# MPEGGroup/mpeg-pcc-tmc2

Hardware: AMD Instinct MI355X
Metric: encoder patch+image-gen frames/sec, longdress_vox10 32-frame GOF (higher is better)
Workload: dtype int32/f64

## Files before the change

include/tmc2hip.h:

```cpp
#ifndef TMC2HIP_H
#define TMC2HIP_H
#include <stddef.h>
#include <stdint.h>

#ifdef __cplusplus
extern "C" {
#endif

#define TMC2_OK 0
#define TMC2_E_NO_DEVICE -1
#define TMC2_E_HIP -2
#define TMC2_E_INVALID -3
#define TMC2_E_UNSUPPORTED -4
#define TMC2_E_STATE -5

typedef struct tmc2_ctx   tmc2_ctx;
typedef struct tmc2_frame tmc2_frame;

typedef struct tmc2_segmenter_params {
  int32_t nnNormalEstimation;
  int32_t normalOrientation;
  int32_t gridBasedRefineSegmentation;
  int32_t maxNNCountRefineSegmentation;
  int32_t iterationCountRefineSegmentation;
  int32_t voxelDimensionRefineSegmentation;
  int32_t searchRadiusRefineSegmentation;
  int32_t occupancyResolution;
  int32_t enablePatchSplitting;
  int32_t maxPatchSize;
  int32_t quantizerSizeX;
  int32_t quantizerSizeY;
  int32_t minPointCountPerCCPatchSegmentation;
  int32_t maxNNCountPatchSegmentation;
  int32_t surfaceThickness;
  int32_t mapCountMinus1;
  int32_t minLevel;
  int32_t maxAllowedDepth;
  int32_t geometryBitDepth2D;
  int32_t geometryBitDepth3D;
  double  maxAllowedDist2RawPointsDetection;
  double  maxAllowedDist2RawPointsSelection;
  double  lambdaRefineSegmentation;
  double  weightNormal[3];
} tmc2_segmenter_params;

typedef struct tmc2_patch {
  int32_t index, viewId;
  int32_t normalAxis, tangentAxis, bitangentAxis, projectionMode;
  int32_t u1, v1, d1;
  int32_t sizeU, sizeV, sizeD, sizeDPixel;
  int32_t sizeU0, sizeV0;
  int32_t size2DXInPixel, size2DYInPixel;
  int32_t d0Count, eomAndD1Count;
  int32_t u0, v0, patchOrientation;
  int64_t depthOffset;
  int64_t occOffset;
} tmc2_patch;

int         tmc2_ctx_create( int device, tmc2_ctx** out );
void        tmc2_ctx_destroy( tmc2_ctx* ctx );
const char* tmc2_last_error( void );
int         tmc2_ctx_synchronize( tmc2_ctx* ctx );
int         tmc2_host_alloc( size_t bytes, void** out );
void        tmc2_host_free( void* p );
int         tmc2_host_register( void* p, size_t bytes );
int         tmc2_host_unregister( void* p );
typedef struct tmc2_host_gate tmc2_host_gate;
int         tmc2_host_gate_create( int maxConcurrentHostSteps, tmc2_host_gate** out );
void        tmc2_host_gate_destroy( tmc2_host_gate* gate );
int         tmc2_ctx_set_host_gate( tmc2_ctx* ctx, tmc2_host_gate* gate );
void        tmc2_set_host_parallelism( int maxConcurrentHostSteps );
int         tmc2_ctx_set_option( tmc2_ctx* ctx, const char* key, const char* value );
const char* tmc2_ctx_get_option( tmc2_ctx* ctx, const char* key );
int         tmc2_ctx_reserve( tmc2_ctx* ctx, uint64_t maxPoints, int voxelDimRefine, int bits3d, int maxCanvasWidth, int maxCanvasHeight );
int         tmc2_ctx_pool_stats( tmc2_ctx* ctx, uint64_t* bytesHeld, uint64_t* mallocCalls, double* mallocMs, uint64_t* carvedBlocks );
int         tmc2_ctx_device_alloc( tmc2_ctx* ctx, size_t bytes, void** out );
int         tmc2_ctx_device_free( tmc2_ctx* ctx, void* p );
int         tmc2_ctx_upload( tmc2_ctx* ctx, void* deviceDst, const void* hostSrc, size_t bytes );
int         tmc2_ctx_download( tmc2_ctx* ctx, void* hostDst, const void* deviceSrc, size_t bytes );
void*       tmc2_ctx_stream( tmc2_ctx* ctx );
int         tmc2_ctx_device( tmc2_ctx* ctx );
int         tmc2_ctx_make_current( tmc2_ctx* ctx );
int         tmc2_ctx_stage_count( tmc2_ctx* ctx );
const char* tmc2_ctx_stage_name( tmc2_ctx* ctx, int i );
double      tmc2_ctx_stage_ms( tmc2_ctx* ctx, int i );
long        tmc2_ctx_stage_calls( tmc2_ctx* ctx, int i );
void        tmc2_ctx_stage_reset( tmc2_ctx* ctx );
void        tmc2_ctx_set_timing( tmc2_ctx* ctx, int enabled );

int  tmc2_frame_create( tmc2_ctx* ctx, const int16_t* xyz, const uint8_t* rgb, uint64_t n, tmc2_frame** out );
void tmc2_frame_destroy( tmc2_frame* f );
int  tmc2_kdtree_build( tmc2_frame* f );
void tmc2_set_kdtree_placement( int mode );
void tmc2_set_refine_overlap( int on );
int  tmc2_frame_get_kdtree_order( tmc2_frame* f, uint32_t* perm, int32_t* depth );
uint64_t tmc2_frame_point_count( const tmc2_frame* f );
int  tmc2_frame_reset( tmc2_frame* f );

int tmc2_kdtree_search( tmc2_frame* f, const int16_t* queries, uint64_t nq, int k, uint32_t* idx, uint32_t* dist2 );
int tmc2_kdtree_search_wide( tmc2_frame* f, const int16_t* queries, uint64_t nq, int k, uint32_t* idx );

int tmc2_normals_compute_normals( tmc2_frame* f, int k );
int tmc2_normals_orient( tmc2_frame* f );
int tmc2_normals_compute( tmc2_frame* f, int k, int orientation );
int tmc2_frame_get_normals( tmc2_frame* f, double* normals  );
int tmc2_frame_set_normals( tmc2_frame* f, const double* normals );
int tmc2_frame_get_adjacency( tmc2_frame* f, uint32_t* adj  );

int tmc2_weight_normal( tmc2_frame* f, int geometryBitDepth3D, double minWeightEPP, double weight[3] );

int tmc2_segmenter_initial_segmentation( tmc2_frame* f, const double weight[3] );
int tmc2_segmenter_refine_grid_based( tmc2_frame* f, int maxNNCount, double lambda, int iterationCount,
                                      int voxDim, int searchRadius );
int tmc2_segmenter_refine( tmc2_frame* f, int maxNNCount, double lambda, int iterationCount );
int tmc2_frame_get_partition( tmc2_frame* f, uint32_t* partition  );
int tmc2_frame_set_partition( tmc2_frame* f, const uint32_t* partition );
int tmc2_segmenter_segment_patches( tmc2_frame* f, const tmc2_segmenter_params* p );
int tmc2_segmenter_compute( tmc2_frame* f, const tmc2_segmenter_params* p );
int tmc2_segmenter_params_check( const tmc2_segmenter_params* p );
int tmc2_segmenter_compute_grid_based( tmc2_frame* f, const tmc2_segmenter_params* p, int voxelDimensionGridBasedSegmentation );
int tmc2_segmenter_compute_knn_refine( tmc2_frame* f, const tmc2_segmenter_params* p, int voxelDimensionGridBasedSegmentation );
int tmc2_segmenter_convert_points_to_voxels( tmc2_ctx* ctx, const int16_t* xyz, uint64_t n, int voxDim, int bits, int16_t* voxelXyz,
                                             uint64_t* voxelCount, uint32_t* voxelOfPoint );

int tmc2_frame_patch_count( tmc2_frame* f );
int tmc2_frame_patch_pool_sizes( tmc2_frame* f, int64_t* depthCount, int64_t* occCount );
int tmc2_frame_get_patches( tmc2_frame* f, tmc2_patch* patches, int16_t* depth0, int16_t* depth1, uint8_t* occupancy );

int tmc2_encoder_pack_flexible( tmc2_frame* f, int presetWidth, int numTilesHor, double tileHeightToWidthRatio,
                                int32_t* height );
int tmc2_encoder_pack_spatial_consistency( tmc2_frame* f, tmc2_frame* previous, int presetWidth, int numTilesHor,
                                           double tileHeightToWidthRatio, int32_t* height );
int tmc2_frame_get_packed_size( tmc2_frame* f, int32_t* width, int32_t* height );
int tmc2_frame_get_patch_matches( tmc2_frame* f, int32_t* matches );
int tmc2_encoder_global_patch_allocation( tmc2_frame** frames, int count, int minimumImageWidth, int minimumImageHeight,
                                          int32_t* widths, int32_t* heights );
int tmc2_frame_set_packing( tmc2_frame* f, const tmc2_patch* list, int count, const int32_t* matches, const uint8_t* occupancy,
                            int64_t occupancyBytes, int packedWidth, int packedHeight );
int tmc2_frame_get_patch_order( tmc2_frame* f, int32_t* order );
int tmc2_encoder_canvas_size( const int32_t* frameHeights, int frames, int tileWidth, int minimumImageWidth,
                              int minimumImageHeight, int32_t* width, int32_t* height );
int tmc2_encoder_generate_geometry_images( tmc2_frame* f, int width, int height, int occupancyPrecision );
int tmc2_frame_get_geometry_images( tmc2_frame* f, uint8_t* occupancy, uint8_t* occVideo, uint32_t* blockToPatch,
                                    uint16_t* geometryD0, uint16_t* geometryD1 );
int     tmc2_encoder_generate_attribute_images( tmc2_frame* f );
int     tmc2_transfer_colors( tmc2_ctx* ctx, const int16_t* srcXyz, const uint8_t* srcRgb, uint64_t n, const int16_t* tgtXyz,
                              uint64_t m, uint8_t* tgtRgb );
int64_t tmc2_frame_recon_count( tmc2_frame* f );
int     tmc2_frame_get_reconstruction( tmc2_frame* f, int16_t* xyz, uint8_t* rgb, uint32_t* pointToPixel );
int     tmc2_frame_get_attribute_images( tmc2_frame* f, uint8_t* attribute );
int     tmc2_frame_set_decoded_geometry( tmc2_frame* f, const uint8_t* occVideo, const uint16_t* geometry );

int tmc2_frame_device_images( tmc2_frame* f, void** occupancy, void** occVideo, void** blockToPatch, void** geometry );
int tmc2_frame_device_attribute( tmc2_frame* f, void** attribute );

int tmc2_color_convert_rgb444_to_yuv420( tmc2_ctx* ctx, const uint8_t* rgb, int width, int height, int downsamplingFilter,
                                         uint8_t* yuv420 );
int tmc2_color_convert_yuv420_to_yuv444( tmc2_ctx* ctx, const uint8_t* yuv420, int width, int height, int upsamplingFilter,
                                         uint16_t* yuv444 );
int tmc2_encoder_attribute_to_yuv420( tmc2_frame* f, int downsamplingFilter, uint8_t* yuv420 );
int tmc2_codec_set_decoded_attribute_yuv420( tmc2_frame* f, const uint8_t* yuv420, int upsamplingFilter );
int tmc2_frame_get_decoded_attribute( tmc2_frame* f, uint16_t* planes );

int tmc2_decoder_frame_create( tmc2_ctx* ctx, const tmc2_patch* patches, int count, int width, int height, int occupancyPrecision,
                               const uint8_t* occVideo, const uint16_t* geometry, tmc2_frame** out );
int tmc2_codec_generate_point_cloud( tmc2_frame* f );
int tmc2_codec_generate_point_cloud_pbf( tmc2_frame* f, int thresholdLossyOM, int passesCount, int filterSize, int log2Threshold );
int tmc2_frame_patch_border_filtering_size( tmc2_frame* f, int64_t* pixels );
int tmc2_frame_get_patch_border_filtering( tmc2_frame* f, uint8_t* occupancy, uint8_t* border );

int tmc2_codec_identify_boundary_points( tmc2_frame* f );
int tmc2_codec_color_point_cloud( tmc2_frame* f, const uint16_t* attribute );
int tmc2_codec_smooth_point_cloud_postprocess( tmc2_frame* f, int gridSize, double thresholdSmoothing );
int tmc2_codec_transfer_colors_16bit_bp( tmc2_frame* f );
int tmc2_codec_color_smoothing( tmc2_frame* f, int gridSize, double thresholdColorSmoothing, double thresholdColorDifference,
                                double thresholdColorVariation );
int tmc2_frame_set_geometry_bit_depth_3d( tmc2_frame* f, int geometryBitDepth3D );
int tmc2_color_smoothing( tmc2_ctx* ctx, const int16_t* xyz, uint16_t* colors16, const uint16_t* boundaryType, const uint32_t* patchIndex,
                          uint64_t M, int gridSize, int geometryBitDepth3D, double thresholdColorSmoothing,
                          double thresholdColorDifference, double thresholdColorVariation );
int tmc2_codec_convert_yuv16_to_rgb8( tmc2_frame* f );
int tmc2_frame_get_post_reconstruction( tmc2_frame* f, int16_t* xyz, uint16_t* colors16, uint8_t* rgb, uint16_t* boundaryType );

int tmc2_metrics_compute( tmc2_ctx* ctx, const int16_t* srcXyz, const uint8_t* srcRgb, uint64_t n, const int16_t* recXyz,
                          const uint8_t* recRgb, uint64_t m, const double* srcNormals, double resolution, double* out,
                          int64_t* counts );

int tmc2_metrics_compute_frame( tmc2_frame* frame, int which, int useNormals, double resolution, double* out, int64_t* counts );
int tmc2_metrics_compute_frame_source( tmc2_frame* frame, int which, const int16_t* srcXyz, const uint8_t* srcRgb, uint64_t n,
                                       const double* srcNormals, double resolution, double* out, int64_t* counts );

int tmc2_metrics_ordered_sums( tmc2_ctx* ctx, const double* termsA, uint64_t nA, const double* termsB, uint64_t nB, double* out );

int tmc2_metrics_display( const double* out, uint64_t sourcePoints, uint64_t reconstructPoints, const int64_t* counts,
                          uint64_t resolution, int withC2p, int precision, char* text, uint64_t capacity, uint64_t* needed );

int tmc2_ply_info( const char* path, int readNormals, uint64_t* pointCount, int* hasColors, int* hasNormals );
int tmc2_ply_read( const char* path, int16_t* xyz, uint8_t* rgb, double* normals, uint64_t capacity, int threads,
                   uint64_t* pointCount );
int tmc2_ply_write( const char* path, const int16_t* xyz, const uint8_t* rgb, const double* normals, uint64_t n, int asAscii );
int tmc2_point_set_checksum( const int16_t* xyz, const uint8_t* rgb, uint64_t n, int reorderPoints, uint8_t digest[16] );

int tmc2_checksum_file_write( const char* path, const uint8_t* digests, uint64_t frames );
int tmc2_checksum_file_read( const char* path, uint8_t* digests, uint64_t capacity, uint64_t* frames );

int tmc2_host_kdtree_build( const int16_t* xyz, uint64_t n, uint32_t* perm, uint64_t* nodeCount, int32_t* depth );
int tmc2_host_pack_flexible( tmc2_patch* patches, int count, const uint8_t* occupancy, int presetWidth, int numTilesHor,
                             double tileHeightToWidthRatio, int32_t* order, int32_t* height );
int tmc2_host_global_patch_allocation( int frames, int32_t* counts, tmc2_patch* patches, const uint8_t* occupancy,
                                       const int64_t* occupancyBase, int32_t* matches, int tileWidth, int tileHeight,
                                       int minimumImageWidth, int minimumImageHeight, uint8_t* occupancyOut,
                                       int64_t occupancyOutCapacity, int64_t* occupancyOutBase, int32_t* widths,
                                       int32_t* heights );
int tmc2_host_pack_spatial_consistency( tmc2_patch* patches, int count, const uint8_t* occupancy, const tmc2_patch* previous,
                                        int previousCount, int presetWidth, int numTilesHor, double tileHeightToWidthRatio,
                                        int32_t* order, int32_t* matches, int32_t* height );
int tmc2_host_place_segments( int frames, const int32_t* counts, tmc2_patch* patches, const uint8_t* occupancy,
                              const int64_t* occupancyBase, int mode, int minimumImageWidth, int minimumImageHeight, int numTilesHor,
                              double tileHeightToWidthRatio, int32_t* matches, uint8_t* occupancyOut, int64_t occupancyOutCapacity,
                              int64_t* occupancyOutBase, int32_t* widths, int32_t* heights );
int tmc2_host_orient_normals( const int16_t* xyz, uint64_t n, const uint32_t* knn, int k, double* normals );
int tmc2_host_color_smoothing( const int16_t* xyz, uint16_t* colors16, const uint16_t* boundaryType, const uint32_t* patchIndex,
                               uint64_t M, int gridSize, int geometryBitDepth3D, double thresholdColorSmoothing,
                               double thresholdColorDifference, double thresholdColorVariation );
int tmc2_host_patch_border_filtering( const tmc2_patch* patches, int count, int width, int height, int occupancyPrecision,
                                      const uint8_t* occVideo, const uint16_t* geometryD0, const uint32_t* blockToPatch,
                                      int thresholdLossyOM, int passesCount, int filterSize, int log2Threshold, uint8_t* occupancy,
                                      uint8_t* border );
int tmc2_host_convert_points_to_voxels( const int16_t* xyz, uint64_t n, int voxDim, int bits, int16_t* voxelXyz, uint64_t* voxelCount,
                                        uint32_t* voxelOfPoint );
int tmc2_host_refine_segmentation( const int16_t* xyz, uint64_t n, const double* normals, uint32_t* partition, int maxNNCount,
                                   double lambda, int iterationCount, uint32_t* adjacency  );

int tmc2_selftest_scan( tmc2_ctx* ctx, const uint32_t* d_in, uint32_t* d_out, uint64_t n, uint32_t* d_total, uint32_t* hostAnswer,
                        const uint32_t* d_carry, int carryWords, uint64_t epoch );
int tmc2_selftest_fill( tmc2_ctx* ctx, const uint64_t* regions, int count );
int tmc2_selftest_work_map( tmc2_ctx* ctx, uint64_t gridBlocks, int blockThreads, uint64_t n, uint64_t liveBlocks, uint32_t* d_hits,
                            uint32_t* d_logical );
int tmc2_selftest_components( tmc2_ctx* ctx, const uint32_t* d_knn, const uint8_t* d_partition, const uint8_t* d_raw,
                              const uint32_t* d_perm, uint64_t n, uint32_t* d_root, uint32_t* d_bad );
int tmc2_selftest_union_find( tmc2_ctx* ctx, int parity, uint32_t* d_word, uint64_t n, const uint32_t* d_edges, uint64_t m, int precheck,
                              int agent, uint32_t* d_root, uint32_t* d_rootParity, uint32_t* d_bad );
int tmc2_selftest_cand_sort( tmc2_ctx* ctx, uint32_t* d_lists, const uint32_t* d_offsets, uint64_t lists, uint32_t* d_ok );
int tmc2_selftest_std_sort( uint32_t* lists, const uint32_t* offsets, uint64_t count );
int tmc2_selftest_marked_cells( tmc2_ctx* ctx, const int16_t* d_xyz4, const uint8_t* d_boundaryType, uint64_t M, int gridSize, int bits,
                                int maxCoord, uint32_t* cells, uint32_t* d_bits, uint32_t* d_rank, const uint32_t* d_keys, uint64_t keys,
                                uint32_t* d_slots );

#ifdef __cplusplus
}
#endif
#endif
```

mpeg-pcc-tmc2_amd/csrc/attributes.hip:

```cpp
#include <algorithm>
#include <cmath>

#include "color_transfer.h"
#include "internal.h"
#include "patch_border_filter.h"

namespace tmc2 {
namespace {

__device__ __forceinline__ void toCanvasB( const PlaceDev& p, int u, int v, int& x, int& y ) {
  if ( p.orient == 0 ) {
    x = u + p.u0 * 16;
    y = v + p.v0 * 16;
  } else {
    x = v + p.u0 * 16;
    y = u + p.v0 * 16;
  }
}

__device__ __forceinline__ int normalCoord( const PlaceDev& p, int depth ) {
  return p.mode == 0 ? depth + p.d1 : max( 0, p.d1 - depth );
}

struct PbfMapsDev {
  const int64_t* offset;
  const uint8_t *occ, *flag;
  int            border;
  uint8_t*       btype;
};

template <bool EMIT, bool PBF = false>
__global__ __launch_bounds__( 256 ) void reconTileKernel( const PlaceDev* __restrict__ place,
                                                           const uint32_t* __restrict__ tilePatch,
                                                           const uint8_t* __restrict__ occVideo,
                                                           const uint32_t* __restrict__ blockToPatch,
                                                           const uint16_t* __restrict__ geo, int W, int H, int prec,
                                                           uint32_t* __restrict__ tileCount,
                                                           const uint32_t* __restrict__ tileOffset, Pt* __restrict__ recon,
                                                           uint32_t* __restrict__ pointToPixel, PbfMapsDev pbf = PbfMapsDev() ) {
  __shared__ uint32_t waveTotal[4];
  const uint32_t      tile  = blockIdx.x;
  const uint32_t      k     = tilePatch[tile];
  const PlaceDev      p     = place[k];
  const int           local = int( tile ) - p.tileBase;
  const int           ub = local % p.sizeU0, vb = local / p.sizeU0;
  const int           bx = p.orient == 0 ? ub + p.u0 : vb + p.u0, by = p.orient == 0 ? vb + p.v0 : ub + p.v0;
  const bool          owned = blockToPatch[size_t( by ) * ( W / 16 ) + bx] == k + 1;
  const int           u = ub * 16 + int( threadIdx.x & 15 ), v = vb * 16 + int( threadIdx.x >> 4 );
  int                 x, y;
  toCanvasB( p, u, v, x, y );
  uint32_t cnt = 0;
  int      c0 = 0, c1 = 0;
  bool    occupied = owned && x < W && y < H;
  uint8_t flag     = 0;
  if constexpr ( PBF ) {
    if ( occupied ) {
      const int64_t c = pbf.offset[k] + int64_t( v + pbf.border ) * ( p.sizeU0 * 16 + 2 * pbf.border ) + u + pbf.border;
      occupied        = pbf.occ[c] != 0;
      flag            = pbf.flag[c];
    }
  } else {
    occupied = occupied && occVideo[size_t( y / prec ) * ( W / prec ) + x / prec];
  }
  if ( occupied ) {
    c0  = normalCoord( p, geo[size_t( y ) * W + x] );
    c1  = normalCoord( p, geo[size_t( W ) * H + size_t( y ) * W + x] );
    cnt = c1 != c0 ? 2u : 1u;
  }
  const int lane = threadIdx.x & 63, wave = threadIdx.x >> 6;
  uint32_t  inc  = cnt;
#pragma unroll
  for ( int off = 1; off < 64; off <<= 1 ) {
    const uint32_t t = __shfl_up( inc, off, 64 );
    if ( lane >= off ) inc += t;
  }
  if ( lane == 63 ) waveTotal[wave] = inc;
  __syncthreads();
  if ( !EMIT ) {
    if ( threadIdx.x == 0 ) tileCount[tile] = waveTotal[0] + waveTotal[1] + waveTotal[2] + waveTotal[3];
    return;
  }
  if ( cnt == 0 ) return;
  uint32_t off = tileOffset[tile] + inc - cnt;
  for ( int w = 0; w < wave; ++w ) off += waveTotal[w];
  int c[3];
  c[p.axT] = u + p.u1;
  c[p.axB] = v + p.v1;
  c[p.axN] = c0;
  recon[off]        = Pt{int16_t( c[0] ), int16_t( c[1] ), int16_t( c[2] ), 0};
  pointToPixel[off] = packPixel( x, y, 0, cnt == 2 );
  if constexpr ( PBF ) {
    pbf.btype[off] = flag;
    if ( cnt == 2 ) pbf.btype[off + 1] = flag;
  }
  if ( cnt == 2 ) {
    c[p.axN]              = c1;
    recon[off + 1]        = Pt{int16_t( c[0] ), int16_t( c[1] ), int16_t( c[2] ), 0};
    pointToPixel[off + 1] = packPixel( x, y, 1, false );
  }
}

__global__ __launch_bounds__( 256 ) void forwardColorKernel( const uint32_t* __restrict__ idx8, const uint32_t* __restrict__ dist8,
                                                              const uint32_t* __restrict__ easy,
                                                              const uint8_t* __restrict__ srcRgb4, uint32_t m,
                                                              uint8_t* __restrict__ fwdRgb4 ) {
  const uint32_t t = blockIdx.x * blockDim.x + threadIdx.x;
  if ( t >= m ) return;
  if ( easy[t] != 0xFFFFFFFFu ) {
    reinterpret_cast<uchar4*>( fwdRgb4 )[t] = reinterpret_cast<const uchar4*>( srcRgb4 )[easy[t]];
    return;
  }
  const uint4* ir = reinterpret_cast<const uint4*>( idx8 + size_t( t ) * 8 );
  const uint4* dr = reinterpret_cast<const uint4*>( dist8 + size_t( t ) * 8 );
  const uint4  i0 = ir[0], i1 = ir[1], d0 = dr[0], d1 = dr[1];
  const uint32_t id[8] = {i0.x, i0.y, i0.z, i0.w, i1.x, i1.y, i1.z, i1.w};
  const uint32_t ds[8] = {d0.x, d0.y, d0.z, d0.w, d1.x, d1.y, d1.z, d1.w};
  reinterpret_cast<uchar4*>( fwdRgb4 )[t] = forwardColor( id, ds, reinterpret_cast<const uchar4*>( srcRgb4 ) );
}

template <bool FILL>
__global__ __launch_bounds__( 256 ) void backwardVoteKernel( const uint32_t* __restrict__ idx1, const uint32_t* __restrict__ dist1, uint32_t n,
                                                              uint32_t* __restrict__ count, const uint32_t* __restrict__ offset,
                                                              uint2* __restrict__ entries ) {
  const uint32_t s = blockIdx.x * blockDim.x + threadIdx.x;
  if ( s >= n ) return;
  const uint32_t t = idx1[s], slot = atomicAdd( &count[t], 1u );
  if ( FILL ) entries[offset[t] + slot] = make_uint2( dist1[s], s );
}

__global__ __launch_bounds__( 256 ) void combineColorKernel( const uint32_t* __restrict__ count, const uint32_t* __restrict__ offset,
                                                              uint2* __restrict__ entries, const uint8_t* __restrict__ srcRgb4,
                                                              const uint8_t* __restrict__ fwdRgb4, uint32_t m,
                                                              uint8_t* __restrict__ outRgb4, uint32_t* __restrict__ error ) {
  const uint32_t t = blockIdx.x * blockDim.x + threadIdx.x;
  if ( t >= m ) return;
  const int n = int( count[t] );
  if ( n == 0 ) {
    reinterpret_cast<uchar4*>( outRgb4 )[t] = reinterpret_cast<const uchar4*>( fwdRgb4 )[t];
    return;
  }
  uint2* e = entries + offset[t];
  if ( !orderCandidates( e, n ) ) *error = 1;
  const ColorSum c = backwardColor( e, e[0].x == 0 ? 1 : n, reinterpret_cast<const uchar4*>( srcRgb4 ), []( uint32_t source ) { return source; } );
  reinterpret_cast<uchar4*>( outRgb4 )[t] = combinedColor( reinterpret_cast<const uchar4*>( fwdRgb4 )[t], c );
}

__global__ __launch_bounds__( 256 ) void attributeScatterKernel( const uint8_t* __restrict__ rgb4,
                                                                  const uint32_t* __restrict__ pointToPixel, uint32_t m,
                                                                  int W, int H, uint8_t* __restrict__ attr ) {
  const uint32_t i = blockIdx.x * blockDim.x + threadIdx.x;
  if ( i >= m ) return;
  const uint32_t pp = pointToPixel[i];
  const size_t   px = size_t( pixelY( pp ) ) * W + pixelX( pp ), plane = size_t( W ) * H;
  const uchar4   c  = reinterpret_cast<const uchar4*>( rgb4 )[i];
  const bool     layer1 = pixelLayer( pp ), hasD1 = pixelHasD1( pp );
  if ( !layer1 ) {
    attr[px] = c.x, attr[plane + px] = c.y, attr[2 * plane + px] = c.z;
    if ( !hasD1 ) attr[3 * plane + px] = c.x, attr[4 * plane + px] = c.y, attr[5 * plane + px] = c.z;
  } else {
    attr[3 * plane + px] = c.x, attr[4 * plane + px] = c.y, attr[5 * plane + px] = c.z;
  }
}

__global__ __launch_bounds__( 256 ) void upsampleOccupancyKernel( const uint8_t* __restrict__ occVideo, int W, int H, int prec,
                                                                   uint8_t* __restrict__ occ ) {
  const size_t c = size_t( blockIdx.x ) * blockDim.x + threadIdx.x;
  if ( c >= size_t( W ) * H ) return;
  occ[c] = occVideo[size_t( ( c / W ) / prec ) * ( W / prec ) + ( c % W ) / prec];
}

__device__ __forceinline__ int mean4w( int p1, int w1, int p2, int w2, int p3, int w3, int p4, int w4 ) {
  return ( p1 * w1 + p2 * w2 + p3 * w3 + p4 * w4 ) / ( w1 + w2 + w3 + w4 );
}

__device__ __forceinline__ void pushPullMipPixel( int i, const uint8_t* img, const uint8_t* occ, int W, int H, uint8_t* mip,
                                                  uint8_t* mipOcc, int w, int h, int p0 = 0, int p1 = 6 ) {
  const int  x = i % w, y = i / w, X = 2 * x, Y = 2 * y;
  const bool i2 = X + 1 < W, i3 = Y + 1 < H;
  const int  w1 = occ[size_t( Y ) * W + X] ? 255 : 0;
  const int  w2 = ( i2 && occ[size_t( Y ) * W + X + 1] ) ? 255 : 0;
  const int  w3 = ( i3 && occ[size_t( Y + 1 ) * W + X] ) ? 255 : 0;
  const int  w4 = ( i2 && i3 && occ[size_t( Y + 1 ) * W + X + 1] ) ? 255 : 0;
  const bool any = ( w1 + w2 + w3 + w4 ) > 0;
  mipOcc[i]      = any ? 1 : 0;
  for ( int p = p0; p < p1; ++p ) {
    const uint8_t* s = img + size_t( p ) * W * H;
    uint8_t        v = 0;
    if ( any ) {
      const int v1 = s[size_t( Y ) * W + X], v2 = i2 ? s[size_t( Y ) * W + X + 1] : 0;
      const int v3 = i3 ? s[size_t( Y + 1 ) * W + X] : 0, v4 = ( i2 && i3 ) ? s[size_t( Y + 1 ) * W + X + 1] : 0;
      v            = uint8_t( mean4w( v1, w1, v2, w2, v3, w3, v4, w4 ) );
    }
    mip[size_t( p ) * w * h + i] = v;
  }
}
__global__ __launch_bounds__( 256 ) void pushPullMipKernel( const uint8_t* __restrict__ img, const uint8_t* __restrict__ occ, int W,
                                                             int H, uint8_t* __restrict__ mip, uint8_t* __restrict__ mipOcc, int w,
                                                             int h ) {
  const int i = blockIdx.x * blockDim.x + threadIdx.x;
  if ( i < w * h ) pushPullMipPixel( i, img, occ, W, H, mip, mipOcc, w, h );
}

__device__ __forceinline__ void pushPullFillPixel( int i, uint8_t* img, const uint8_t* occ, int W, int H, const uint8_t* mip, int w,
                                                   int h, int p0 = 0, int p1 = 6 ) {
  if ( occ[i] ) return;
  const int  X = i % W, Y = i / W, x = X >> 1, y = Y >> 1;
  const int  dx = ( X & 1 ) ? 1 : -1, dy = ( Y & 1 ) ? 1 : -1;
  const bool hx = dx < 0 ? x > 0 : x < w - 1, hy = dy < 0 ? y > 0 : y < h - 1;
  for ( int p = p0; p < p1; ++p ) {
    const uint8_t* m  = mip + size_t( p ) * w * h;
    const int      v  = m[size_t( y ) * w + x];
    const int      vx = hx ? m[size_t( y ) * w + x + dx] : 0;
    const int      vy = hy ? m[size_t( y + dy ) * w + x] : 0;
    const int      vd = ( hx && hy ) ? m[size_t( y + dy ) * w + x + dx] : 0;
    img[size_t( p ) * W * H + i] = uint8_t( mean4w( v, 144, vx, hx ? 48 : 0, vy, hy ? 48 : 0, vd, ( hx && hy ) ? 16 : 0 ) );
  }
}
__global__ __launch_bounds__( 256 ) void pushPullFillKernel( uint8_t* __restrict__ img, const uint8_t* __restrict__ occ, int W, int H,
                                                              const uint8_t* __restrict__ mip, int w, int h ) {
  const int i = blockIdx.x * blockDim.x + threadIdx.x;
  if ( i < W * H ) pushPullFillPixel( i, img, occ, W, H, mip, w, h );
}

__device__ __forceinline__ void pushPullBlurPixel( int i, const uint8_t* src, uint8_t* dst, const uint8_t* occ, int W, int H, int p0 = 0,
                                                   int p1 = 6 ) {
  if ( occ[i] ) return;
  const int x = i % W, y = i / W;
  const int x1 = x > 0 ? x - 1 : x, y1 = y > 0 ? y - 1 : y, x2 = x < W - 1 ? x + 1 : x, y2 = y < H - 1 ? y + 1 : y;
  for ( int p = p0; p < p1; ++p ) {
    const uint8_t* s   = src + size_t( p ) * W * H;
    const int      sum = s[size_t( y1 ) * W + x1] + s[size_t( y1 ) * W + x2] + s[size_t( y2 ) * W + x1] + s[size_t( y2 ) * W + x2] +
                    s[size_t( y ) * W + x1] + s[size_t( y ) * W + x2] + s[size_t( y1 ) * W + x] + s[size_t( y2 ) * W + x];
    dst[size_t( p ) * W * H + i] = uint8_t( ( sum + 4 ) >> 3 );
  }
}
__global__ __launch_bounds__( 256 ) void pushPullBlurKernel( const uint8_t* __restrict__ src, uint8_t* __restrict__ dst,
                                                              const uint8_t* __restrict__ occ, int W, int H ) {
  const int i = blockIdx.x * blockDim.x + threadIdx.x;
  if ( i < W * H ) pushPullBlurPixel( i, src, dst, occ, W, H );
}

constexpr int kPushPullTile = 96, kPushPullSpan = 128, kPushPullMaxIters = ( kPushPullSpan - kPushPullTile ) / 2;
__global__ __launch_bounds__( 1024 ) void pushPullFillBlurKernel( uint8_t* __restrict__ img, const uint8_t* __restrict__ occ, int W,
                                                                   int H, const uint8_t* __restrict__ mip, int w, int h, int iters,
                                                                   int tilesX ) {
  __shared__ uint8_t sOcc[kPushPullSpan * kPushPullSpan];
  __shared__ uint8_t sBuf[2][kPushPullSpan * kPushPullSpan];
  const int      X0 = ( blockIdx.x % tilesX ) * kPushPullTile, Y0 = ( blockIdx.x / tilesX ) * kPushPullTile;
  const int      RX0 = max( X0 - iters, 0 ), RY0 = max( Y0 - iters, 0 );
  const int      RW = min( X0 + kPushPullTile + iters, W ) - RX0, RH = min( Y0 + kPushPullTile + iters, H ) - RY0;
  uint8_t*       plane = img + size_t( blockIdx.y ) * W * H;
  const uint8_t* m     = mip + size_t( blockIdx.y ) * w * h;
  for ( int i = threadIdx.x; i < kPushPullSpan * RH; i += 1024 ) {
    const int rx = i & ( kPushPullSpan - 1 ), ry = i >> 7;
    if ( rx >= RW ) continue;
    const int     X = RX0 + rx, Y = RY0 + ry;
    const size_t  g = size_t( Y ) * W + X;
    const uint8_t o = occ[g];
    uint8_t       v;
    if ( o ) {
      v = plane[g];
    } else {
      const int  x = X >> 1, y = Y >> 1, dx = ( X & 1 ) ? 1 : -1, dy = ( Y & 1 ) ? 1 : -1;
      const bool hx = dx < 0 ? x > 0 : x < w - 1, hy = dy < 0 ? y > 0 : y < h - 1;
      const int  c  = m[size_t( y ) * w + x];
      const int  vx = hx ? m[size_t( y ) * w + x + dx] : 0;
      const int  vy = hy ? m[size_t( y + dy ) * w + x] : 0;
      const int  vd = ( hx && hy ) ? m[size_t( y + dy ) * w + x + dx] : 0;
      v             = uint8_t( mean4w( c, 144, vx, hx ? 48 : 0, vy, hy ? 48 : 0, vd, ( hx && hy ) ? 16 : 0 ) );
    }
    sOcc[i]    = o;
    sBuf[0][i] = v;
    sBuf[1][i] = v;
  }
  __syncthreads();
  int cur = 0;
  for ( int it = 0; it < iters; ++it ) {
    const uint8_t* src = sBuf[cur];
    uint8_t*       dst = sBuf[cur ^ 1];
    for ( int i = threadIdx.x; i < kPushPullSpan * RH; i += 1024 ) {
      const int rx = i & ( kPushPullSpan - 1 ), ry = i >> 7;
      if ( rx >= RW || sOcc[i] ) continue;
      const int l = rx > 0 ? -1 : 0, r = rx < RW - 1 ? 1 : 0;
      const int u = ry > 0 ? -kPushPullSpan : 0, d = ry < RH - 1 ? kPushPullSpan : 0;
      const int sum = src[i + u + l] + src[i + u + r] + src[i + d + l] + src[i + d + r] + src[i + l] + src[i + r] + src[i + u] +
                      src[i + d];
      dst[i] = uint8_t( ( sum + 4 ) >> 3 );
    }
    __syncthreads();
    cur ^= 1;
  }
  const uint8_t* res = sBuf[cur];
  for ( int i = threadIdx.x; i < kPushPullSpan * RH; i += 1024 ) {
    const int rx = i & ( kPushPullSpan - 1 ), ry = i >> 7;
    const int X = RX0 + rx, Y = RY0 + ry;
    if ( rx >= RW || sOcc[i] || X < X0 || X >= X0 + kPushPullTile || Y < Y0 || Y >= Y0 + kPushPullTile ) continue;
    plane[size_t( Y ) * W + X] = res[i];
  }
}

constexpr int kPushPullSmall  = 160 * 160;
constexpr int kPushPullLevels = 16;
struct PushPullLevels {
  int      count;
  int      first;
  int      w[kPushPullLevels], h[kPushPullLevels];
  uint8_t *img[kPushPullLevels], *tmp[kPushPullLevels], *occ[kPushPullLevels];
};
__global__ __launch_bounds__( 1024 ) void pushPullCoarseLevelsKernel( PushPullLevels L ) {
  const int p0 = int( blockIdx.x ), p1 = p0 + 1;
  for ( int l = L.first + 1; l < L.count; ++l ) {
    const int cnt = L.w[l] * L.h[l];
    for ( int i = threadIdx.x; i < cnt; i += blockDim.x )
      pushPullMipPixel( i, L.img[l - 1], L.occ[l - 1], L.w[l - 1], L.h[l - 1], L.img[l], L.occ[l], L.w[l], L.h[l], p0, p1 );
    __syncthreads();
  }
  int iters = 4;
  for ( int l = L.count - 1; l > L.first; --l ) {
    const int fw = L.w[l - 1], fh = L.h[l - 1], cnt = fw * fh;
    uint8_t * img = L.img[l - 1], *tmp = L.tmp[l - 1];
    const uint8_t* occ = L.occ[l - 1];
    for ( int i = threadIdx.x; i < cnt; i += blockDim.x ) pushPullFillPixel( i, img, occ, fw, fh, L.img[l], L.w[l], L.h[l], p0, p1 );
    __syncthreads();
    for ( int i = threadIdx.x; i < cnt; i += blockDim.x ) tmp[size_t( p0 ) * cnt + i] = img[size_t( p0 ) * cnt + i];
    __syncthreads();
    uint8_t *src = img, *dst = tmp;
    for ( int it = 0; it < iters; ++it ) {
      for ( int i = threadIdx.x; i < cnt; i += blockDim.x ) pushPullBlurPixel( i, src, dst, occ, fw, fh, p0, p1 );
      __syncthreads();
      uint8_t* t = src;
      src        = dst;
      dst        = t;
    }
    if ( src != img ) {
      L.img[l - 1] = src;
      L.tmp[l - 1] = img;
    }
    iters = min( iters + 1, 16 );
  }
}

__global__ __launch_bounds__( 256 ) void attributeGroupDilateKernel( const uint8_t* __restrict__ occ, int W, int H,
                                                                      uint8_t* __restrict__ attr ) {
  const size_t c = size_t( blockIdx.x ) * blockDim.x + threadIdx.x, plane = size_t( W ) * H;
  if ( c >= plane || occ[c] ) return;
#pragma unroll
  for ( int k = 0; k < 3; ++k ) {
    const uint32_t a = attr[k * plane + c], b = attr[( 3 + k ) * plane + c];
    const uint8_t  v = uint8_t( ( a + b + 1 ) >> 1 );
    attr[k * plane + c] = attr[( 3 + k ) * plane + c] = v;
  }
}

}

int transferColorsDevice( tmc2_ctx* ctx, const TreeDev& srcTree, const Pt* d_srcPts, const uint8_t* d_srcRgb4, uint32_t n,
                          const TreeDev& tgtTree, const Pt* d_tgtPts, uint32_t M, uint8_t* d_outRgb4, uint32_t* d_error ) {
  hipStream_t      s = ctx->stream;
  const dim3       blk( 256 );
  DevBuf<uint32_t> d_idx8, d_dist8, d_idx1, d_dist1, d_count, d_offset, d_cursor;
  DevBuf<uint2>    d_entries;
  DevBuf<uint8_t>  d_fwd;
  TMC2_TRY( d_idx8.alloc( size_t( M ) * 8 ) );
  TMC2_TRY( d_dist8.alloc( size_t( M ) * 8 ) );
  TMC2_TRY( d_idx1.alloc( n ) );
  TMC2_TRY( d_dist1.alloc( n ) );
  TMC2_TRY( d_count.alloc( M ) );
  TMC2_TRY( d_offset.alloc( M ) );
  TMC2_TRY( d_cursor.alloc( M ) );
  TMC2_TRY( d_entries.alloc( n ) );
  TMC2_TRY( d_fwd.alloc( size_t( M ) * 4 ) );
  DevBuf<uint32_t> d_easy8;
  TMC2_TRY( d_easy8.alloc( M ) );
  TMC2_TRY( launchKnnSplit( ctx, srcTree, d_tgtPts, M, 8, d_easy8.p, d_idx8.p, d_dist8.p, "knn8_recon_in_source" ) );
  TMC2_TRY( launchKnnSplit( ctx, tgtTree, d_srcPts, n, 1, d_idx1.p, d_idx1.p, d_dist1.p, "knn1_source_in_recon" ) );
  StageScope stage( ctx, "transfer_colors" );
  TMC2_TRY( fillRegions( ctx, {{d_count.p, size_t( M ) * 4, 0}, {d_cursor.p, size_t( M ) * 4, 0}, {d_error, 4, 0}} ) );
  const dim3 grdM( ( M + 255 ) / 256 ), grdN( ( n + 255 ) / 256 );
  hipLaunchKernelGGL( forwardColorKernel, grdM, blk, 0, s, d_idx8.p, d_dist8.p, d_easy8.p, d_srcRgb4, M, d_fwd.p );
  hipLaunchKernelGGL( backwardVoteKernel<false>, grdN, blk, 0, s, d_idx1.p, d_dist1.p, n, d_count.p, d_offset.p, d_entries.p );
  TMC2_TRY( exclusiveScanU32( ctx, d_count.p, d_offset.p, M, nullptr ) );
  hipLaunchKernelGGL( backwardVoteKernel<true>, grdN, blk, 0, s, d_idx1.p, d_dist1.p, n, d_cursor.p, d_offset.p, d_entries.p );
  hipLaunchKernelGGL( combineColorKernel, grdM, blk, 0, s, d_count.p, d_offset.p, d_entries.p, d_srcRgb4, d_fwd.p, M,
                      d_outRgb4, d_error );
  TMC2_HIP( hipGetLastError() );
  return TMC2_OK;
}

int reconstructPointCloud( tmc2_frame* f, const PbfParams* pbfParams ) {
  if ( !f->haveGeometryImages ) {
    setError( "generatePointCloud: geometry images missing" );
    return TMC2_E_STATE;
  }
  if ( pbfParams ) {
    if ( const char* what = pbfRefusal( f->occPrecision, *pbfParams, long( f->patches.size() ) ) ) {
      setError( "generatePointCloud (patch border filtering): unsupported %s", what );
      return TMC2_E_UNSUPPORTED;
    }
  }
  const bool keepAttributeImages = f->haveAttributeImages && ( pbfParams || f->havePbf );
  f->canvasesChanged();
  f->haveAttributeImages = keepAttributeImages;
  if ( pbfParams ) TMC2_TRY( patchBorderFilterDevice( f, *pbfParams ) );
  PbfMapsDev pbf;
  if ( pbfParams ) pbf = PbfMapsDev{f->d_pbfOffset.p, f->pbfOcc, f->pbfFlag, f->pbfBorderWidth, nullptr};
  tmc2_ctx*    ctx = f->ctx;
  hipStream_t  s   = ctx->stream;
  const int    W = f->canvasW, H = f->canvasH, prec = f->occPrecision;
  const dim3   blk( 256 );
  const uint32_t tiles = f->tileCount;
  StageScope       stage( ctx, "reconstruct" );
  DevBuf<uint32_t> d_tileCount, d_tileOffset, d_small;
  TMC2_TRY( d_tileCount.alloc( std::max( tiles, 1u ) ) );
  TMC2_TRY( d_tileOffset.alloc( std::max( tiles, 1u ) ) );
  TMC2_TRY( d_small.alloc( 8 ) );
  uint32_t M = 0;
  if ( tiles ) {
    if ( pbfParams )
      hipLaunchKernelGGL( ( reconTileKernel<false, true> ), dim3( tiles ), blk, 0, s, f->d_place.p, f->d_tilePatch.p, f->d_occVideo.p,
                          f->d_blockToPatch.p, f->d_geo.p, W, H, prec, d_tileCount.p, (const uint32_t*)nullptr, (Pt*)nullptr,
                          (uint32_t*)nullptr, pbf );
    else
      hipLaunchKernelGGL( reconTileKernel<false>, dim3( tiles ), blk, 0, s, f->d_place.p, f->d_tilePatch.p, f->d_occVideo.p,
                          f->d_blockToPatch.p, f->d_geo.p, W, H, prec, d_tileCount.p, (const uint32_t*)nullptr, (Pt*)nullptr,
                          (uint32_t*)nullptr, PbfMapsDev() );
    volatile uint32_t* answer = ctx->answerLine( tmc2_ctx::kAnswerRecon );
    TMC2_TRY( exclusiveScanU32( ctx, d_tileCount.p, d_tileOffset.p, tiles, d_small.p, ScanAnswer{answer, nullptr, 0} ) );
    TMC2_HIP( hipStreamSynchronize( s ) );
    M = answer[0];
  }
  if ( M == 0 && pbfParams ) {
    stage.end();
    f->reconCount         = 0;
    f->haveReconstruction = true;
    f->haveBoundaryTypes  = true;
    return TMC2_OK;
  }
  if ( M == 0 ) {
    setError( "generatePointCloud: empty reconstruction" );
    return TMC2_E_STATE;
  }
  TMC2_TRY( f->d_recon.alloc( M ) );
  TMC2_TRY( f->d_pointToPixel.alloc( M ) );
  if ( pbfParams ) {
    TMC2_TRY( f->d_boundaryType.alloc( M ) );
    TMC2_TRY( f->d_pbfBoundary.alloc( M ) );
    pbf.btype = f->d_boundaryType.p;
    hipLaunchKernelGGL( ( reconTileKernel<true, true> ), dim3( tiles ), blk, 0, s, f->d_place.p, f->d_tilePatch.p, f->d_occVideo.p,
                        f->d_blockToPatch.p, f->d_geo.p, W, H, prec, d_tileCount.p, d_tileOffset.p, f->d_recon.p, f->d_pointToPixel.p,
                        pbf );
    TMC2_HIP( hipMemcpyAsync( f->d_pbfBoundary.p, f->d_boundaryType.p, M, hipMemcpyDeviceToDevice, s ) );
  } else {
    hipLaunchKernelGGL( reconTileKernel<true>, dim3( tiles ), blk, 0, s, f->d_place.p, f->d_tilePatch.p, f->d_occVideo.p,
                        f->d_blockToPatch.p, f->d_geo.p, W, H, prec, d_tileCount.p, d_tileOffset.p, f->d_recon.p,
                        f->d_pointToPixel.p, PbfMapsDev() );
  }
  stage.end();
  f->reconCount = M;
  TMC2_TRY( buildKdTreePlaced( ctx, f->d_recon.p, M, nullptr, "kdtree_build_recon", f->reconTree ) );
  f->haveReconstruction = true;
  f->haveBoundaryTypes  = pbfParams != nullptr;
  return TMC2_OK;
}

int generateAttributeImages( tmc2_frame* f ) {
  if ( !f->haveGeometryImages ) {
    setError( "generateAttributeImages: geometry images missing" );
    return TMC2_E_STATE;
  }
  if ( f->d_rgb.count == 0 ) {
    setError( "generateAttributeImages: the frame has no colours" );
    return TMC2_E_STATE;
  }
  TMC2_TRY( f->ensureTree() );
  TMC2_TRY( reconstructPointCloud( f ) );
  tmc2_ctx*    ctx = f->ctx;
  hipStream_t  s   = ctx->stream;
  const int    W = f->canvasW, H = f->canvasH, prec = f->occPrecision;
  const size_t area = size_t( W ) * H;
  const dim3   blk( 256 );
  const uint32_t n = uint32_t( f->n ), M = uint32_t( f->reconCount );
  DevBuf<uint32_t> d_small;
  TMC2_TRY( d_small.alloc( 8 ) );
  TMC2_TRY( f->d_reconRgb.alloc( size_t( M ) * 4 ) );
  const dim3 grdM( ( M + 255 ) / 256 );
  volatile uint32_t* h_err = ctx->answerLine( tmc2_ctx::kAnswerAttrError );
  TMC2_TRY( transferColorsDevice( ctx, f->tree.view( QueryBox::Tight ), f->d_pts.p, f->d_rgb.p, n, f->reconTree.view( QueryBox::Tight ),
                                  f->d_recon.p, M, f->d_reconRgb.p, const_cast<uint32_t*>( h_err ) ) );
  StageScope      stage( ctx, "attribute_images" );
  DevBuf<uint8_t> d_occ;
  TMC2_TRY( d_occ.alloc( area ) );
  TMC2_TRY( f->d_attr.alloc( 6 * area ) );
  TMC2_HIP( hipMemsetAsync( f->d_attr.p, 0, 6 * area, s ) );
  hipLaunchKernelGGL( upsampleOccupancyKernel, dim3( uint32_t( ( area + 255 ) / 256 ) ), blk, 0, s, f->d_occVideo.p, W, H, prec,
                      d_occ.p );
  hipLaunchKernelGGL( attributeScatterKernel, grdM, blk, 0, s, f->d_reconRgb.p, f->d_pointToPixel.p, M, W, H, f->d_attr.p );
  struct Level {
    int      w, h;
    uint8_t *img, *tmp, *occ;
  };
  std::vector<Level> lv;
  lv.push_back( Level{W, H, f->d_attr.p, nullptr, d_occ.p} );
  size_t pyramidBytes = 6 * area;
  {
    int w = W, h = H;
    for ( ;; ) {
      w = ( w + 1 ) >> 1;
      h = ( h + 1 ) >> 1;
      lv.push_back( Level{w, h, nullptr, nullptr, nullptr} );
      pyramidBytes += size_t( w ) * h * ( 6 + 6 + 1 );
      if ( w <= 4 || h <= 4 ) break;
    }
  }
  DevBuf<uint8_t> d_pyr;
  TMC2_TRY( d_pyr.alloc( pyramidBytes + 64 * lv.size() ) );
  {
    uint8_t* p = d_pyr.p;
    lv[0].tmp  = p;
    p += 6 * area;
    for ( size_t l = 1; l < lv.size(); ++l ) {
      const size_t a = size_t( lv[l].w ) * lv[l].h;
      lv[l].img = p, p += 6 * a;
      lv[l].tmp = p, p += 6 * a;
      lv[l].occ = p, p += ( a + 15 ) & ~size_t( 15 );
    }
  }
  size_t firstSmall = lv.size();
  if ( lv.size() <= size_t( kPushPullLevels ) )
    for ( size_t l = 1; l < lv.size(); ++l )
      if ( lv[l].w * lv[l].h <= kPushPullSmall ) {
        firstSmall = l;
        break;
      }
  for ( size_t l = 1; l < lv.size() && l <= firstSmall; ++l ) {
    const int cnt = lv[l].w * lv[l].h;
    hipLaunchKernelGGL( pushPullMipKernel, dim3( ( cnt + 255 ) / 256 ), blk, 0, s, lv[l - 1].img, lv[l - 1].occ, lv[l - 1].w,
                        lv[l - 1].h, lv[l].img, lv[l].occ, lv[l].w, lv[l].h );
  }
  int iters = 4;
  if ( firstSmall + 1 < lv.size() ) {
    PushPullLevels L;
    L.count = int( lv.size() ), L.first = int( firstSmall );
    for ( size_t l = 0; l < lv.size(); ++l ) L.w[l] = lv[l].w, L.h[l] = lv[l].h, L.img[l] = lv[l].img, L.tmp[l] = lv[l].tmp, L.occ[l] = lv[l].occ;
    hipLaunchKernelGGL( pushPullCoarseLevelsKernel, dim3( 6 ), dim3( 1024 ), 0, s, L );
    for ( size_t l = lv.size() - 1; l > firstSmall; --l ) {
      if ( iters & 1 ) std::swap( lv[l - 1].img, lv[l - 1].tmp );
      iters = std::min( iters + 1, 16 );
    }
  }
  for ( size_t l = std::min( firstSmall, lv.size() - 1 ); l >= 1; --l ) {
    Level&    fine = lv[l - 1];
    const int cnt  = fine.w * fine.h;
    const dim3 grd( ( cnt + 255 ) / 256 );
    if ( iters <= kPushPullMaxIters ) {
      const int tilesX = ( fine.w + kPushPullTile - 1 ) / kPushPullTile, tilesY = ( fine.h + kPushPullTile - 1 ) / kPushPullTile;
      hipLaunchKernelGGL( pushPullFillBlurKernel, dim3( tilesX * tilesY, 6 ), dim3( 1024 ), 0, s, fine.img, fine.occ, fine.w, fine.h,
                          lv[l].img, lv[l].w, lv[l].h, iters, tilesX );
      iters = std::min( iters + 1, 16 );
      continue;
    }
    hipLaunchKernelGGL( pushPullFillKernel, grd, blk, 0, s, fine.img, fine.occ, fine.w, fine.h, lv[l].img, lv[l].w, lv[l].h );
    TMC2_HIP( hipMemcpyAsync( fine.tmp, fine.img, size_t( 6 ) * cnt, hipMemcpyDeviceToDevice, s ) );
    uint8_t *src = fine.img, *dst = fine.tmp;
    for ( int it = 0; it < iters; ++it ) {
      hipLaunchKernelGGL( pushPullBlurKernel, grd, blk, 0, s, src, dst, fine.occ, fine.w, fine.h );
      std::swap( src, dst );
    }
    if ( src != fine.img ) {
      if ( l - 1 == 0 )
        TMC2_HIP( hipMemcpyAsync( fine.img, src, size_t( 6 ) * cnt, hipMemcpyDeviceToDevice, s ) );
      else
        std::swap( fine.img, fine.tmp );
    }
    iters = std::min( iters + 1, 16 );
  }
  hipLaunchKernelGGL( attributeGroupDilateKernel, dim3( uint32_t( ( area + 255 ) / 256 ) ), blk, 0, s, d_occ.p, W, H, f->d_attr.p );
  stage.end();
  TMC2_HIP( hipStreamSynchronize( s ) );
  TMC2_HIP( hipGetLastError() );
  const uint32_t err = *h_err;
  if ( err ) {
    setError( "transferColors: a backward candidate list hit std::sort's depth limit (heapsort fallback of libstdc++ "
              "introsort is not reproduced)" );
    return TMC2_E_UNSUPPORTED;
  }
  f->haveAttributeImages = true;
  return TMC2_OK;
}

}

extern "C" {

int tmc2_transfer_colors( tmc2_ctx* ctx, const int16_t* srcXyz, const uint8_t* srcRgb, uint64_t n, const int16_t* tgtXyz,
                          uint64_t m, uint8_t* tgtRgb ) {
  using namespace tmc2;
  if ( !ctx || !srcXyz || !srcRgb || !tgtXyz || !tgtRgb || n < 8 || m < 1 ) {
    setError( "transfer_colors: invalid argument (the source needs at least 8 points)" );
    return TMC2_E_INVALID;
  }
  ApiScope    scope( ctx );
  hipStream_t s = ctx->stream;
  struct Side {
    DevBuf<Pt> pts;
    DeviceTree tree;
  } S, T;
  auto upload = [&]( Side& sd, const int16_t* xyz, uint64_t cnt ) -> int {
    std::vector<Pt> pts( cnt );
    for ( uint64_t i = 0; i < cnt; ++i ) pts[i] = Pt{xyz[3 * i], xyz[3 * i + 1], xyz[3 * i + 2], 0};
    TMC2_TRY( sd.pts.alloc( cnt ) );
    TMC2_HIP( hipMemcpyAsync( sd.pts.p, pts.data(), cnt * sizeof( Pt ), hipMemcpyHostToDevice, s ) );
    TMC2_HIP( hipStreamSynchronize( s ) );
    return buildKdTreeDevice( ctx, sd.pts.p, cnt, sd.tree );
  };
  TMC2_TRY( upload( S, srcXyz, n ) );
  TMC2_TRY( upload( T, tgtXyz, m ) );
  std::vector<uint8_t> c4( 4 * n );
  for ( uint64_t i = 0; i < n; ++i ) c4[4 * i] = srcRgb[3 * i], c4[4 * i + 1] = srcRgb[3 * i + 1], c4[4 * i + 2] = srcRgb[3 * i + 2], c4[4 * i + 3] = 0;
  DevBuf<uint8_t>  d_rgb, d_out;
  DevBuf<uint32_t> d_err;
  TMC2_TRY( d_rgb.alloc( 4 * n ) );
  TMC2_TRY( d_out.alloc( 4 * m ) );
  TMC2_TRY( d_err.alloc( 1 ) );
  TMC2_HIP( hipMemcpyAsync( d_rgb.p, c4.data(), 4 * n, hipMemcpyHostToDevice, s ) );
  TMC2_TRY( transferColorsDevice( ctx, S.tree.view( QueryBox::Any ), S.pts.p, d_rgb.p, uint32_t( n ), T.tree.view( QueryBox::Any ), T.pts.p,
                                  uint32_t( m ), d_out.p, d_err.p ) );
  std::vector<uint8_t> o4( 4 * m );
  uint32_t             err = 0;
  TMC2_HIP( hipMemcpyAsync( o4.data(), d_out.p, 4 * m, hipMemcpyDeviceToHost, s ) );
  TMC2_HIP( hipMemcpyAsync( &err, d_err.p, 4, hipMemcpyDeviceToHost, s ) );
  TMC2_HIP( hipStreamSynchronize( s ) );
  if ( err ) {
    setError( "transferColors: a backward candidate list hit std::sort's depth limit (not reproduced)" );
    return TMC2_E_UNSUPPORTED;
  }
  for ( uint64_t i = 0; i < m; ++i ) tgtRgb[3 * i] = o4[4 * i], tgtRgb[3 * i + 1] = o4[4 * i + 1], tgtRgb[3 * i + 2] = o4[4 * i + 2];
  return TMC2_OK;
}

int tmc2_codec_generate_point_cloud( tmc2_frame* f ) {
  if ( !f ) return TMC2_E_INVALID;
  tmc2::ApiScope scope( f->ctx );
  return tmc2::reconstructPointCloud( f );
}

int tmc2_encoder_generate_attribute_images( tmc2_frame* f ) {
  if ( !f ) return TMC2_E_INVALID;
  tmc2::ApiScope scope( f->ctx );
  return tmc2::generateAttributeImages( f );
}

int64_t tmc2_frame_recon_count( tmc2_frame* f ) { return ( f && f->haveReconstruction ) ? int64_t( f->reconCount ) : 0; }

int tmc2_frame_get_reconstruction( tmc2_frame* f, int16_t* xyz, uint8_t* rgb, uint32_t* pointToPixel ) {
  if ( !f || !f->haveReconstruction ) {
    tmc2::setError( "get_reconstruction: not generated" );
    return TMC2_E_STATE;
  }
  if ( rgb && ( !f->haveAttributeImages || f->havePbf ) ) {
    tmc2::setError( "get_reconstruction: no transferred colours (tmc2_encoder_generate_attribute_images produces them)" );
    return TMC2_E_STATE;
  }
  tmc2::ApiScope scope( f->ctx );
  hipStream_t    s = f->ctx->stream;
  const size_t   M = f->reconCount;
  if ( M == 0 ) return TMC2_OK;
  std::vector<tmc2::Pt>  pts( M );
  std::vector<uint8_t>   c4( rgb ? 4 * M : 0 );
  std::vector<uint32_t>  pp( M );
  TMC2_HIP( hipMemcpyAsync( pts.data(), f->d_recon.p, M * sizeof( tmc2::Pt ), hipMemcpyDeviceToHost, s ) );
  if ( rgb ) TMC2_HIP( hipMemcpyAsync( c4.data(), f->d_reconRgb.p, 4 * M, hipMemcpyDeviceToHost, s ) );
  TMC2_HIP( hipMemcpyAsync( pp.data(), f->d_pointToPixel.p, 4 * M, hipMemcpyDeviceToHost, s ) );
  TMC2_HIP( hipStreamSynchronize( s ) );
  for ( size_t i = 0; i < M; ++i ) {
    if ( xyz ) xyz[3 * i] = pts[i].x, xyz[3 * i + 1] = pts[i].y, xyz[3 * i + 2] = pts[i].z;
    if ( rgb ) rgb[3 * i] = c4[4 * i], rgb[3 * i + 1] = c4[4 * i + 1], rgb[3 * i + 2] = c4[4 * i + 2];
    if ( pointToPixel )
      pointToPixel[3 * i] = tmc2::pixelX( pp[i] ), pointToPixel[3 * i + 1] = tmc2::pixelY( pp[i] ), pointToPixel[3 * i + 2] = tmc2::pixelLayer( pp[i] );
  }
  return TMC2_OK;
}

int tmc2_frame_device_attribute( tmc2_frame* f, void** attribute ) {
  if ( !f || !attribute || !f->haveAttributeImages ) return TMC2_E_STATE;
  *attribute = f->d_attr.p;
  return TMC2_OK;
}

int tmc2_frame_get_attribute_images( tmc2_frame* f, uint8_t* attribute ) {
  if ( !f || !attribute || !f->haveAttributeImages ) {
    tmc2::setError( "get_attribute_images: not generated" );
    return TMC2_E_STATE;
  }
  tmc2::ApiScope scope( f->ctx );
  TMC2_HIP( hipMemcpyAsync( attribute, f->d_attr.p, size_t( 6 ) * f->canvasW * f->canvasH, hipMemcpyDeviceToHost, f->ctx->stream ) );
  TMC2_HIP( hipStreamSynchronize( f->ctx->stream ) );
  return TMC2_OK;
}
}
```

mpeg-pcc-tmc2_amd/csrc/images.hip:

```cpp
#include <memory>

#include "internal.h"

namespace tmc2 {
namespace {

__device__ __forceinline__ void toCanvas( const PlaceDev& p, int u, int v, int& x, int& y ) {
  if ( p.orient == 0 ) {
    x = u + p.u0 * 16;
    y = v + p.v0 * 16;
  } else {
    x = v + p.u0 * 16;
    y = u + p.v0 * 16;
  }
}

__global__ __launch_bounds__( 256 ) void rasterTileKernel( const PlaceDev* __restrict__ place,
                                                            const uint32_t* __restrict__ tilePatch,
                                                            const int16_t* __restrict__ depth0,
                                                            const int16_t* __restrict__ depth1, int W, int H,
                                                            uint8_t* __restrict__ occMap, uint16_t* __restrict__ geo0,
                                                            uint16_t* __restrict__ geo1, uint32_t* __restrict__ error ) {
  const uint32_t tile  = blockIdx.x;
  const PlaceDev p     = place[tilePatch[tile]];
  const int      local = int( tile ) - p.tileBase;
  const int      u = ( local % p.sizeU0 ) * 16 + int( threadIdx.x & 15 ), v = ( local / p.sizeU0 ) * 16 + int( threadIdx.x >> 4 );
  if ( u >= p.sizeU || v >= p.sizeV ) return;
  const size_t  q = size_t( p.depthOff ) + size_t( v ) * p.sizeU + u;
  const int16_t d = depth0[q];
  if ( d == 32767 ) return;
  int x, y;
  toCanvas( p, u, v, x, y );
  if ( x >= W || y >= H ) {
    *error = 1;
    return;
  }
  const size_t c = size_t( y ) * W + x;
  occMap[c]      = 1;
  geo0[c]        = uint16_t( d );
  geo1[c]        = uint16_t( depth1[q] );
}

__global__ __launch_bounds__( 256 ) void occVideoKernel( const uint8_t* __restrict__ occMap, int W, int Wv, int Hv, int p,
                                                          uint8_t* __restrict__ occVideo ) {
  const int i = blockIdx.x * blockDim.x + threadIdx.x;
  if ( i >= Wv * Hv ) return;
  const int xv = i % Wv, yv = i / Wv;
  uint32_t  any = 0;
  for ( int j = 0; j < p; ++j )
    for ( int k = 0; k < p; ++k ) any |= occMap[size_t( yv * p + j ) * W + xv * p + k];
  occVideo[i] = any ? 1 : 0;
}

__global__ __launch_bounds__( 256 ) void blockToPatchKernel( const PlaceDev* __restrict__ place, int P,
                                                              const uint8_t* __restrict__ occVideo, int Wb, int Hb,
                                                              int Wv, int p, uint32_t* __restrict__ blockToPatch ) {
  const int b = blockIdx.x * blockDim.x + threadIdx.x;
  if ( b >= Wb * Hb ) return;
  const int bx = b % Wb, by = b / Wb;
  const int cells = 16 / p;
  bool      any = false;
  for ( int j = 0; j < cells && !any; ++j )
    for ( int i = 0; i < cells; ++i ) any |= occVideo[size_t( by * cells + j ) * Wv + bx * cells + i] != 0;
  uint32_t owner = 0;
  if ( any ) {
    for ( int k = 0; k < P; ++k ) {
      const PlaceDev q = place[k];
      const int      w = q.orient == 0 ? q.sizeU0 : q.sizeV0, h = q.orient == 0 ? q.sizeV0 : q.sizeU0;
      if ( bx >= q.u0 && bx < q.u0 + w && by >= q.v0 && by < q.v0 + h ) owner = uint32_t( k + 1 );
    }
  }
  blockToPatch[b] = owner;
}

__global__ __launch_bounds__( 256 ) void dilateBlockKernel( const uint8_t* __restrict__ occMap, int W, int H,
                                                             uint16_t* __restrict__ geo ,
                                                             uint8_t* __restrict__ emptyBlock ) {
  __shared__ uint32_t lvl[18][18];
  __shared__ uint32_t val[18][18];
  __shared__ int      counters[2];
  const int Wb = W / 16;
  const int bx = blockIdx.x % Wb, by = blockIdx.x / Wb;
  const int i = threadIdx.x & 15, j = threadIdx.x >> 4;
  uint16_t* img = geo + size_t( blockIdx.y ) * W * H;
  const size_t c = size_t( by * 16 + j ) * W + bx * 16 + i;
  for ( int t = threadIdx.x; t < 18 * 18; t += 256 ) ( &lvl[0][0] )[t] = 0xFFFFFFFFu;
  if ( threadIdx.x == 0 ) counters[0] = 0;
  __syncthreads();
  uint32_t myLevel = occMap[c] ? 1u : 0u;
  uint32_t myVal   = img[c];
  lvl[j + 1][i + 1] = myLevel;
  val[j + 1][i + 1] = myVal;
  if ( myLevel ) atomicAdd( &counters[0], 1 );
  __syncthreads();
  int filled = counters[0];
  if ( filled == 0 ) {
    if ( threadIdx.x == 0 && blockIdx.y == 0 ) emptyBlock[blockIdx.x] = 1;
    return;
  }
  if ( threadIdx.x == 0 && blockIdx.y == 0 ) emptyBlock[blockIdx.x] = 0;
  for ( uint32_t it = 1; filled < 256; ++it ) {
    uint32_t sum = 0, cnt = 0;
    if ( myLevel == 0 ) {
      if ( lvl[j][i + 1] == it ) { sum += val[j][i + 1]; ++cnt; }
      if ( lvl[j + 1][i] == it ) { sum += val[j + 1][i]; ++cnt; }
      if ( lvl[j + 1][i + 2] == it ) { sum += val[j + 1][i + 2]; ++cnt; }
      if ( lvl[j + 2][i + 1] == it ) { sum += val[j + 2][i + 1]; ++cnt; }
    }
    __syncthreads();
    if ( threadIdx.x == 0 ) counters[1] = 0;
    __syncthreads();
    if ( cnt ) {
      myLevel           = it + 1;
      myVal             = ( sum + cnt / 2 ) / cnt;
      lvl[j + 1][i + 1] = myLevel;
      val[j + 1][i + 1] = myVal;
      atomicAdd( &counters[1], 1 );
    }
    __syncthreads();
    filled += counters[1];
    __syncthreads();
  }
  img[c] = uint16_t( myVal );
}

__global__ void carryFirstColumnKernel( const uint8_t* __restrict__ emptyBlock, int W, int H, uint16_t* __restrict__ geo,
                                        uint8_t* __restrict__ resolved ) {
  const int x = threadIdx.x;
  uint16_t* img = geo + size_t( blockIdx.x ) * W * H;
  const int Wb = W / 16, Hb = H / 16;
  uint16_t  carry = 0;
  for ( int by = 0; by < Hb; ++by ) {
    if ( emptyBlock[size_t( by ) * Wb] ) {
      if ( by > 0 )
        for ( int j = 0; j < 16; ++j ) img[size_t( by * 16 + j ) * W + x] = carry;
      if ( by == 0 ) carry = img[size_t( 15 ) * W + x];
    } else {
      carry = img[size_t( by * 16 + 15 ) * W + x];
    }
  }
  (void)resolved;
}

__global__ __launch_bounds__( 64 ) void carryRowsKernel( const uint8_t* __restrict__ emptyBlock, int W, int H,
                                                          uint16_t* __restrict__ geo ) {
  const int y = blockIdx.x * blockDim.x + threadIdx.x;
  if ( y >= H ) return;
  uint16_t* row = geo + size_t( blockIdx.y ) * W * H + size_t( y ) * W;
  const int Wb  = W / 16;
  const uint8_t* e = emptyBlock + size_t( y / 16 ) * Wb;
  uint16_t carry = row[15];
  for ( int bx = 1; bx < Wb; ++bx ) {
    if ( e[bx] ) {
#pragma unroll
      for ( int i = 0; i < 16; ++i ) row[bx * 16 + i] = carry;
    } else {
      carry = row[bx * 16 + 15];
    }
  }
}

__global__ __launch_bounds__( 256 ) void groupDilateKernel( const uint8_t* __restrict__ occVideo, int W, int H, int Wv,
                                                             int p, uint16_t* __restrict__ geo ) {
  const size_t c = size_t( blockIdx.x ) * blockDim.x + threadIdx.x;
  if ( c >= size_t( W ) * H ) return;
  const int x = int( c % W ), y = int( c / W );
  if ( occVideo[size_t( y / p ) * Wv + x / p ] ) return;
  const uint32_t a = geo[c], b = geo[size_t( W ) * H + c];
  const uint16_t avg = uint16_t( ( a + b + 1 ) >> 1 );
  geo[c]                   = avg;
  geo[size_t( W ) * H + c] = avg;
}

}

int uploadPlacement( tmc2_frame* f ) {
  const int P = int( f->patches.size() );
  size_t    tiles = 0;
  for ( int k = 0; k < P; ++k ) {
    const tmc2_patch& t = f->patches[size_t( f->packOrder[size_t( k )] )];
    if ( t.patchOrientation != 0 && t.patchOrientation != 1 ) {
      setError( "patch orientation %d unsupported", t.patchOrientation );
      return TMC2_E_UNSUPPORTED;
    }
    if ( t.sizeU0 < 0 || t.sizeV0 < 0 || t.u0 < 0 || t.v0 < 0 ) {
      setError( "patch %d: negative block size or position", k );
      return TMC2_E_INVALID;
    }
    tiles += size_t( t.sizeU0 ) * size_t( t.sizeV0 );
  }
  const size_t placeBytes = ( size_t( P ) * sizeof( PlaceDev ) + 15 ) & ~size_t( 15 );
  uint8_t*     staging    = f->ctx->hostTables.get<uint8_t>( std::max<size_t>( placeBytes + tiles * 4, size_t( 1 ) << 20 ) );
  if ( !staging ) {
    setError( "uploadPlacement: hipHostMalloc failed" );
    return TMC2_E_HIP;
  }
  PlaceDev* place     = reinterpret_cast<PlaceDev*>( staging );
  uint32_t* tilePatch = reinterpret_cast<uint32_t*>( staging + placeBytes );
  size_t    at        = 0;
  for ( int k = 0; k < P; ++k ) {
    const tmc2_patch& t = f->patches[size_t( f->packOrder[size_t( k )] )];
    PlaceDev&         d = place[size_t( k )];
    d.u0 = t.u0, d.v0 = t.v0, d.orient = t.patchOrientation;
    d.sizeU = t.sizeU, d.sizeV = t.sizeV, d.sizeU0 = t.sizeU0, d.sizeV0 = t.sizeV0;
    d.tileBase = int32_t( at );
    d.depthOff = t.depthOffset;
    d.u1 = t.u1, d.v1 = t.v1, d.d1 = t.d1;
    d.axN = t.normalAxis, d.axT = t.tangentAxis, d.axB = t.bitangentAxis, d.mode = t.projectionMode;
    d.pad = 0;
    for ( size_t b = size_t( t.sizeU0 ) * size_t( t.sizeV0 ); b > 0; --b ) tilePatch[at++] = uint32_t( k );
  }
  hipStream_t s = f->ctx->stream;
  TMC2_TRY( f->d_place.alloc( size_t( std::max( P, 1 ) ) ) );
  TMC2_TRY( f->d_tilePatch.alloc( std::max<size_t>( tiles, 1 ) ) );
  if ( P ) {
    TMC2_HIP( hipMemcpyAsync( f->d_place.p, place, size_t( P ) * sizeof( PlaceDev ), hipMemcpyHostToDevice, s ) );
    if ( tiles ) TMC2_HIP( hipMemcpyAsync( f->d_tilePatch.p, tilePatch, tiles * 4, hipMemcpyHostToDevice, s ) );
  }
  f->tileCount = uint32_t( tiles );
  return TMC2_OK;
}

int createDecoderFrame( tmc2_ctx* ctx, const tmc2_patch* patches, int count, int W, int H, int occPrecision, const uint8_t* occVideo,
                        const uint16_t* geometry, tmc2_frame** out ) {
  if ( W <= 0 || H <= 0 || W % 16 || H % 16 || W > kMaxCanvasDim || H > kMaxCanvasDim || occPrecision < 1 || 16 % occPrecision ) {
    setError( "decoder_frame_create: unsupported geometry %dx%d (at most %d a side), precision %d", W, H, kMaxCanvasDim, occPrecision );
    return TMC2_E_UNSUPPORTED;
  }
  std::unique_ptr<tmc2_frame> f( new tmc2_frame() );
  f->ticket.bind( ctx );
  f->ctx = ctx;
  f->n   = 0;
  f->patches.assign( patches, patches + count );
  f->packOrder.resize( size_t( count ) );
  for ( int k = 0; k < count; ++k ) {
    f->packOrder[size_t( k )] = k;
    const tmc2_patch& t = f->patches[size_t( k )];
    const int axes = ( 1 << t.normalAxis ) | ( 1 << t.tangentAxis ) | ( 1 << t.bitangentAxis );
    if ( t.normalAxis < 0 || t.normalAxis > 2 || t.tangentAxis < 0 || t.tangentAxis > 2 || t.bitangentAxis < 0 ||
         t.bitangentAxis > 2 || axes != 7 || t.projectionMode < 0 || t.projectionMode > 1 || t.patchOrientation < 0 ||
         t.patchOrientation > 1 || t.sizeU0 <= 0 || t.sizeV0 <= 0 ) {
      setError( "decoder_frame_create: patch %d: axes (%d, %d, %d) / projection mode %d / orientation %d / block size %dx%d invalid",
                k, t.normalAxis, t.tangentAxis, t.bitangentAxis, t.projectionMode, t.patchOrientation, t.sizeU0, t.sizeV0 );
      return TMC2_E_INVALID;
    }
    const int64_t bw = t.patchOrientation == 0 ? t.sizeU0 : t.sizeV0, bh = t.patchOrientation == 0 ? t.sizeV0 : t.sizeU0;
    if ( t.u0 < 0 || t.v0 < 0 || ( int64_t( t.u0 ) + bw ) * 16 > W || ( int64_t( t.v0 ) + bh ) * 16 > H ) {
      setError( "decoder_frame_create: patch %d lies outside the %dx%d canvas", k, W, H );
      return TMC2_E_INVALID;
    }
  }
  f->packMatch.assign( size_t( count ), -1 );
  f->havePatches = f->havePacking = true;
  hipStream_t  s    = ctx->stream;
  const size_t area = size_t( W ) * H;
  const int    Wv = W / occPrecision, Hv = H / occPrecision, Wb = W / 16, Hb = H / 16;
  TMC2_TRY( f->d_occVideo.alloc( size_t( Wv ) * Hv ) );
  TMC2_TRY( f->d_blockToPatch.alloc( size_t( Wb ) * Hb ) );
  TMC2_TRY( f->d_geo.alloc( 2 * area ) );
  TMC2_TRY( f->d_occMap.alloc( area ) );
  TMC2_TRY( uploadPlacement( f.get() ) );
  TMC2_HIP( hipMemcpyAsync( f->d_occVideo.p, occVideo, size_t( Wv ) * Hv, hipMemcpyHostToDevice, s ) );
  TMC2_HIP( hipMemcpyAsync( f->d_geo.p, geometry, 2 * area * sizeof( uint16_t ), hipMemcpyHostToDevice, s ) );
  TMC2_HIP( hipMemsetAsync( f->d_occMap.p, 0, area, s ) );
  {
    StageScope stage( ctx, "block_to_patch" );
    hipLaunchKernelGGL( blockToPatchKernel, dim3( ( Wb * Hb + 255 ) / 256 ), dim3( 256 ), 0, s, f->d_place.p, count, f->d_occVideo.p, Wb,
                        Hb, Wv, occPrecision, f->d_blockToPatch.p );
  }
  TMC2_HIP( hipStreamSynchronize( s ) );
  TMC2_HIP( hipGetLastError() );
  f->canvasW = W, f->canvasH = H, f->occPrecision = occPrecision;
  f->haveGeometryImages = true;
  *out                  = f.release();
  return TMC2_OK;
}

int generateGeometryImages( tmc2_frame* f, int W, int H, int occRes, int occPrecision ) {
  if ( !f->havePacking ) {
    setError( "generateGeometryImages: frame not packed" );
    return TMC2_E_STATE;
  }
  if ( occRes != 16 || W <= 0 || H <= 0 || W % 16 || H % 16 || W > kMaxCanvasDim || H > kMaxCanvasDim || occPrecision < 1 ||
       16 % occPrecision ) {
    setError( "generateGeometryImages: unsupported geometry %dx%d (at most %d a side), occupancyResolution %d, precision %d", W, H,
              kMaxCanvasDim, occRes, occPrecision );
    return TMC2_E_UNSUPPORTED;
  }
  f->packingChanged();
  tmc2_ctx*   ctx = f->ctx;
  hipStream_t s   = ctx->stream;
  const int   P   = int( f->patches.size() );
  const size_t area = size_t( W ) * H;
  const int    Wv = W / occPrecision, Hv = H / occPrecision, Wb = W / 16, Hb = H / 16;
  volatile uint32_t* h_err = ctx->answerLine( tmc2_ctx::kAnswerGeoError );
  *h_err                   = 0;
  DevBuf<uint8_t>  d_empty;
  TMC2_TRY( d_empty.alloc( size_t( Wb ) * Hb ) );
  TMC2_TRY( f->d_occMap.alloc( area ) );
  TMC2_TRY( f->d_occVideo.alloc( size_t( Wv ) * Hv ) );
  TMC2_TRY( f->d_blockToPatch.alloc( size_t( Wb ) * Hb ) );
  TMC2_TRY( f->d_geo.alloc( 2 * area ) );
  TMC2_TRY( uploadPlacement( f ) );
  DevBuf<PlaceDev>& d_place     = f->d_place;
  DevBuf<uint32_t>& d_tilePatch = f->d_tilePatch;
  StageScope        stage( ctx, "geometry_images" );
  TMC2_TRY( fillRegions( ctx, {{f->d_occMap.p, area, 0}, {f->d_geo.p, 2 * area * sizeof( uint16_t ), 0}} ) );
  const dim3 blk( 256 );
  if ( f->tileCount )
    hipLaunchKernelGGL( rasterTileKernel, dim3( f->tileCount ), blk, 0, s, d_place.p, d_tilePatch.p,
                        f->d_depth0.p, f->d_depth1.p, W, H, f->d_occMap.p, f->d_geo.p, f->d_geo.p + area, const_cast<uint32_t*>( h_err ) );
  hipLaunchKernelGGL( occVideoKernel, dim3( ( Wv * Hv + 255 ) / 256 ), blk, 0, s, f->d_occMap.p, W, Wv, Hv, occPrecision,
                      f->d_occVideo.p );
  hipLaunchKernelGGL( blockToPatchKernel, dim3( ( Wb * Hb + 255 ) / 256 ), blk, 0, s, d_place.p, P, f->d_occVideo.p, Wb,
                      Hb, Wv, occPrecision, f->d_blockToPatch.p );
  hipLaunchKernelGGL( dilateBlockKernel, dim3( Wb * Hb, 2 ), blk, 0, s, f->d_occMap.p, W, H, f->d_geo.p, d_empty.p );
  hipLaunchKernelGGL( carryFirstColumnKernel, dim3( 2 ), dim3( 16 ), 0, s, d_empty.p, W, H, f->d_geo.p, (uint8_t*)nullptr );
  hipLaunchKernelGGL( carryRowsKernel, dim3( ( H + 63 ) / 64, 2 ), dim3( 64 ), 0, s, d_empty.p, W, H, f->d_geo.p );
  hipLaunchKernelGGL( groupDilateKernel, dim3( uint32_t( ( area + 255 ) / 256 ) ), blk, 0, s, f->d_occVideo.p, W, H, Wv,
                      occPrecision, f->d_geo.p );
  stage.end();
  TMC2_HIP( hipStreamSynchronize( s ) );
  TMC2_HIP( hipGetLastError() );
  const uint32_t err = *h_err;
  if ( err ) {
    setError( "generateGeometryImages: a patch falls outside the %dx%d canvas (the reference exits with code 180)", W, H );
    return TMC2_E_INVALID;
  }
  f->canvasW            = W;
  f->canvasH            = H;
  f->occPrecision       = occPrecision;
  f->haveGeometryImages = true;
  return TMC2_OK;
}

}

extern "C" {

int tmc2_encoder_generate_geometry_images( tmc2_frame* f, int width, int height, int occupancyPrecision ) {
  if ( !f ) return TMC2_E_INVALID;
  tmc2::ApiScope scope( f->ctx );
  return tmc2::generateGeometryImages( f, width, height, 16, occupancyPrecision );
}

int tmc2_decoder_frame_create( tmc2_ctx* ctx, const tmc2_patch* patches, int count, int width, int height, int occupancyPrecision,
                               const uint8_t* occVideo, const uint16_t* geometry, tmc2_frame** out ) {
  if ( !ctx || !out || count < 0 || ( count && !patches ) || !occVideo || !geometry ) return TMC2_E_INVALID;
  *out = nullptr;
  tmc2::ApiScope scope( ctx );
  return tmc2::createDecoderFrame( ctx, patches, count, width, height, occupancyPrecision, occVideo, geometry, out );
}

int tmc2_frame_set_decoded_geometry( tmc2_frame* f, const uint8_t* occVideo, const uint16_t* geometry ) {
  if ( !f || !f->haveGeometryImages ) {
    tmc2::setError( "set_decoded_geometry: canvases not generated" );
    return TMC2_E_STATE;
  }
  tmc2::ApiScope scope( f->ctx );
  hipStream_t    s    = f->ctx->stream;
  const size_t   area = size_t( f->canvasW ) * f->canvasH;
  if ( occVideo )
    TMC2_HIP( hipMemcpyAsync( f->d_occVideo.p, occVideo, area / ( size_t( f->occPrecision ) * f->occPrecision ),
                              hipMemcpyHostToDevice, s ) );
  if ( geometry ) TMC2_HIP( hipMemcpyAsync( f->d_geo.p, geometry, 2 * area * sizeof( uint16_t ), hipMemcpyHostToDevice, s ) );
  if ( occVideo ) {
    const int Wb = f->canvasW / 16, Hb = f->canvasH / 16;
    hipLaunchKernelGGL( tmc2::blockToPatchKernel, dim3( ( Wb * Hb + 255 ) / 256 ), dim3( 256 ), 0, s, f->d_place.p,
                        int( f->patches.size() ), f->d_occVideo.p, Wb, Hb, f->canvasW / f->occPrecision, f->occPrecision,
                        f->d_blockToPatch.p );
  }
  f->canvasesChanged();
  TMC2_HIP( hipStreamSynchronize( s ) );
  TMC2_HIP( hipGetLastError() );
  return TMC2_OK;
}

int tmc2_frame_device_images( tmc2_frame* f, void** occupancy, void** occVideo, void** blockToPatch, void** geometry ) {
  if ( !f || !f->haveGeometryImages ) {
    tmc2::setError( "device_images: not generated" );
    return TMC2_E_STATE;
  }
  if ( occupancy ) *occupancy = f->d_occMap.p;
  if ( occVideo ) *occVideo = f->d_occVideo.p;
  if ( blockToPatch ) *blockToPatch = f->d_blockToPatch.p;
  if ( geometry ) *geometry = f->d_geo.p;
  return TMC2_OK;
}

int tmc2_frame_get_geometry_images( tmc2_frame* f, uint8_t* occupancy, uint8_t* occVideo, uint32_t* blockToPatch,
                                    uint16_t* geometryD0, uint16_t* geometryD1 ) {
  if ( !f || !f->haveGeometryImages ) {
    tmc2::setError( "get_geometry_images: not generated" );
    return TMC2_E_STATE;
  }
  tmc2::ApiScope scope( f->ctx );
  hipStream_t  s    = f->ctx->stream;
  const size_t area = size_t( f->canvasW ) * f->canvasH;
  const size_t av   = area / ( size_t( f->occPrecision ) * f->occPrecision );
  if ( occupancy ) TMC2_HIP( hipMemcpyAsync( occupancy, f->d_occMap.p, area, hipMemcpyDeviceToHost, s ) );
  if ( occVideo ) TMC2_HIP( hipMemcpyAsync( occVideo, f->d_occVideo.p, av, hipMemcpyDeviceToHost, s ) );
  if ( blockToPatch ) TMC2_HIP( hipMemcpyAsync( blockToPatch, f->d_blockToPatch.p, area / 256 * 4, hipMemcpyDeviceToHost, s ) );
  if ( geometryD0 ) TMC2_HIP( hipMemcpyAsync( geometryD0, f->d_geo.p, area * 2, hipMemcpyDeviceToHost, s ) );
  if ( geometryD1 ) TMC2_HIP( hipMemcpyAsync( geometryD1, f->d_geo.p + area, area * 2, hipMemcpyDeviceToHost, s ) );
  TMC2_HIP( hipStreamSynchronize( s ) );
  return TMC2_OK;
}
}
```

mpeg-pcc-tmc2_amd/tmc2_amd/lib.py:

```python
import ctypes as C
import os as _os

_os.environ.setdefault("GPU_MAX_HW_QUEUES", "16")
import os
import re
import threading
import numpy as np

_HERE = os.path.dirname(os.path.abspath(__file__))
_LIB = None


def library_path():
    return os.path.normpath(os.path.join(_HERE, "..", "libtmc2hip.so"))


class Tmc2Error(RuntimeError):
    pass


class SegmenterParams(C.Structure):
    _fields_ = [(n, C.c_int32) for n in (
        "nnNormalEstimation", "normalOrientation", "gridBasedRefineSegmentation", "maxNNCountRefineSegmentation",
        "iterationCountRefineSegmentation", "voxelDimensionRefineSegmentation", "searchRadiusRefineSegmentation",
        "occupancyResolution", "enablePatchSplitting", "maxPatchSize", "quantizerSizeX", "quantizerSizeY",
        "minPointCountPerCCPatchSegmentation", "maxNNCountPatchSegmentation", "surfaceThickness", "mapCountMinus1",
        "minLevel", "maxAllowedDepth", "geometryBitDepth2D", "geometryBitDepth3D")] + [
        ("maxAllowedDist2RawPointsDetection", C.c_double), ("maxAllowedDist2RawPointsSelection", C.c_double),
        ("lambdaRefineSegmentation", C.c_double), ("weightNormal", C.c_double * 3)]


class Patch(C.Structure):
    _fields_ = [(n, C.c_int32) for n in (
        "index", "viewId", "normalAxis", "tangentAxis", "bitangentAxis", "projectionMode", "u1", "v1", "d1", "sizeU",
        "sizeV", "sizeD", "sizeDPixel", "sizeU0", "sizeV0", "size2DXInPixel", "size2DYInPixel", "d0Count",
        "eomAndD1Count", "u0", "v0", "patchOrientation")] + [("depthOffset", C.c_int64), ("occOffset", C.c_int64)]


PATCH_DTYPE = np.dtype(Patch._fields_)


def ctc_params(iterations=10, bits3d=11, weight=(1.0, 1.0, 1.0), vox_dim=4):
    p = SegmenterParams()
    p.nnNormalEstimation = 16
    p.normalOrientation = 1
    p.gridBasedRefineSegmentation = 1
    p.maxNNCountRefineSegmentation = 1024
    p.iterationCountRefineSegmentation = iterations
    p.voxelDimensionRefineSegmentation = vox_dim
    p.searchRadiusRefineSegmentation = 192
    p.occupancyResolution = 16
    p.enablePatchSplitting = 1
    p.maxPatchSize = 1024
    p.quantizerSizeX = 16
    p.quantizerSizeY = 16
    p.minPointCountPerCCPatchSegmentation = 16
    p.maxNNCountPatchSegmentation = 16
    p.surfaceThickness = 4
    p.mapCountMinus1 = 1
    p.minLevel = 64
    p.maxAllowedDepth = 255
    p.geometryBitDepth2D = 8
    p.geometryBitDepth3D = bits3d
    p.maxAllowedDist2RawPointsDetection = 9.0
    p.maxAllowedDist2RawPointsSelection = 1.0
    p.lambdaRefineSegmentation = 3.0
    p.weightNormal[0], p.weightNormal[1], p.weightNormal[2] = weight
    return p


def fast_params(iterations=5, bits3d=11, weight=(1.0, 1.0, 1.0)):
    p = ctc_params(iterations, bits3d, weight, vox_dim=2)
    p.maxNNCountRefineSegmentation = 384
    p.searchRadiusRefineSegmentation = 128
    return p


def knn_refine_params(iterations=100, bits3d=11, weight=(1.0, 1.0, 1.0)):
    p = ctc_params(iterations, bits3d, weight)
    p.gridBasedRefineSegmentation = 0
    p.maxNNCountRefineSegmentation = 256
    return p


_GUARD = 4096
_guard_on = os.environ.get("TMC2_GUARD", "0") == "1"
_guard_tls = threading.local()


def set_guard(on):
    global _guard_on
    _guard_on = bool(on)


def _ptr(a):
    if not _guard_on or a.nbytes == 0:
        return a.ctypes.data_as(C.c_void_p)
    if not a.flags["C_CONTIGUOUS"]:
        raise Tmc2Error("guard mode: array handed to the C-ABI is not contiguous")
    g = np.full(a.nbytes + 2 * _GUARD, 0xA5, np.uint8)
    g[_GUARD:_GUARD + a.nbytes] = a.reshape(-1).view(np.uint8)
    if not hasattr(_guard_tls, "pending"):
        _guard_tls.pending = []
    _guard_tls.pending.append((a, g))
    return C.c_void_p(g.ctypes.data + _GUARD)


def _guard_finish():
    pending, _guard_tls.pending = getattr(_guard_tls, "pending", []), []
    for a, g in pending:
        n = a.nbytes
        lo, hi = g[:_GUARD], g[_GUARD + n:]
        if (lo != 0xA5).any() or (hi != 0xA5).any():
            before, after = int((lo != 0xA5).sum()), int((hi != 0xA5).sum())
            first = int(np.argmax(hi != 0xA5)) if after else -1
            raise Tmc2Error("guard mode: the library wrote outside a caller's buffer (%s %s, %d bytes): %d bytes changed before it, "
                            "%d after it (first at +%d)" % (a.dtype, a.shape, n, before, after, first))
        if a.flags["WRITEABLE"]:
            a.reshape(-1).view(np.uint8)[:] = g[_GUARD:_GUARD + n]


_SCALARS = {"void": None, "int": C.c_int, "int32_t": C.c_int32, "int64_t": C.c_int64, "uint64_t": C.c_uint64, "size_t": C.c_size_t,
            "long": C.c_long, "double": C.c_double}


def _ctype(c_type):
    if c_type == "const char*":
        return C.c_char_p
    return C.c_void_p if c_type[-1] in "*]" else _SCALARS[c_type]


def declare(handle, rows):
    for row in rows:
        ret, name, params = re.fullmatch(r"(.+?) (tmc2_\w+)\((.*)\)", row).groups()
        fn = getattr(handle, name)
        fn.restype = _ctype(ret)
        fn.argtypes = [] if params == "void" else [_ctype(t) for t in params.split(", ")]
    return handle


def load_library():
    global _LIB
    if _LIB is not None:
        return _LIB
    path = library_path()
    if not os.path.exists(path):
        raise Tmc2Error("libtmc2hip.so not built: run `python __graft_entry__.py build` (hipcc, gfx950)")
    _LIB = declare(C.CDLL(path), TMC2HIP)
    return _LIB


def _check(rc):
    if _guard_on:
        _guard_finish()
    if rc != 0:
        raise Tmc2Error("tmc2hip error %d: %s" % (rc, load_library().tmc2_last_error().decode()))


class HostGate:

    def __init__(self, limit):
        self.L = load_library()
        self.h = C.c_void_p()
        _check(self.L.tmc2_host_gate_create(int(limit), C.byref(self.h)))

    def close(self):
        if self.h:
            self.L.tmc2_host_gate_destroy(self.h)
            self.h = C.c_void_p()

    def __del__(self):
        try:
            self.close()
        except Exception:
            pass


class Context:
    def __init__(self, device=0):
        self.L = load_library()
        self.h = C.c_void_p()
        _check(self.L.tmc2_ctx_create(int(device), C.byref(self.h)))

    def close(self):
        if self.h:
            self.L.tmc2_ctx_destroy(self.h)
            self.h = C.c_void_p()

    def __del__(self):
        try:
            self.close()
        except Exception:
            pass

    def synchronize(self):
        _check(self.L.tmc2_ctx_synchronize(self.h))

    def set_option(self, key, value):
        _check(self.L.tmc2_ctx_set_option(self.h, key.encode(), None if value is None else str(value).encode()))

    def get_option(self, key):
        v = self.L.tmc2_ctx_get_option(self.h, key.encode())
        return None if v is None else v.decode()

    def set_host_gate(self, gate):
        _check(self.L.tmc2_ctx_set_host_gate(self.h, None if gate is None else gate.h))

    def reserve(self, max_points, vox_dim, bits3d, max_w, max_h):
        _check(self.L.tmc2_ctx_reserve(self.h, int(max_points), int(vox_dim), int(bits3d), int(max_w), int(max_h)))

    def device_alloc(self, nbytes):
        p = C.c_void_p()
        _check(self.L.tmc2_ctx_device_alloc(self.h, int(nbytes), C.byref(p)))
        return p

    def device_free(self, p):
        _check(self.L.tmc2_ctx_device_free(self.h, p))

    def upload(self, device_ptr, array):
        a = np.ascontiguousarray(array)
        _check(self.L.tmc2_ctx_upload(self.h, device_ptr, _ptr(a), a.nbytes))

    def download(self, array, device_ptr):
        _check(self.L.tmc2_ctx_download(self.h, _ptr(array), device_ptr, array.nbytes))
        return array


    def selftest_scan(self, d_in, d_out, n, d_total=None, host_answer=None, d_carry=None, carry_words=0, epoch=0):
        _check(self.L.tmc2_selftest_scan(self.h, d_in, d_out, int(n), d_total, host_answer, d_carry, int(carry_words), int(epoch)))

    def selftest_fill(self, regions):
        r = np.ascontiguousarray([[int(getattr(p, "value", p) or 0), int(b), int(v)] for p, b, v in regions], dtype=np.uint64).reshape(-1, 3)
        _check(self.L.tmc2_selftest_fill(self.h, _ptr(r) if len(r) else None, len(r)))

    def selftest_work_map(self, grid_blocks, block_threads, n, live_blocks, d_hits, d_logical):
        _check(self.L.tmc2_selftest_work_map(self.h, int(grid_blocks), int(block_threads), int(n), int(live_blocks), d_hits, d_logical))

    def selftest_components(self, d_knn, d_partition, d_raw, d_perm, n, d_root, d_bad):
        _check(self.L.tmc2_selftest_components(self.h, d_knn, d_partition, d_raw, d_perm, int(n), d_root, d_bad))

    def selftest_union_find(self, parity, d_word, n, d_edges, m, precheck, agent, d_root, d_root_parity, d_bad):
        _check(self.L.tmc2_selftest_union_find(self.h, int(parity), d_word, int(n), d_edges, int(m), int(precheck), int(agent), d_root,
                                               d_root_parity, d_bad))

    def selftest_cand_sort(self, d_lists, d_offsets, lists, d_ok):
        _check(self.L.tmc2_selftest_cand_sort(self.h, d_lists, d_offsets, int(lists), d_ok))

    def selftest_marked_cells(self, d_xyz4, d_boundary_type, m, grid_size, bits=0, max_coord=0, d_bits=None, d_rank=None, d_keys=None,
                              keys=0, d_slots=None):
        cells = C.c_uint32(0)
        _check(self.L.tmc2_selftest_marked_cells(self.h, d_xyz4, d_boundary_type, int(m), int(grid_size), int(bits), int(max_coord),
                                                 C.byref(cells), d_bits, d_rank, d_keys, int(keys), d_slots))
        return cells.value

    def stream(self):
        return self.L.tmc2_ctx_stream(self.h)

    def device(self):
        return int(self.L.tmc2_ctx_device(self.h))

    def make_current(self):
        _check(self.L.tmc2_ctx_make_current(self.h))

    def pool_stats(self):
        held, calls, carved, ms = C.c_uint64(), C.c_uint64(), C.c_uint64(), C.c_double()
        _check(self.L.tmc2_ctx_pool_stats(self.h, C.byref(held), C.byref(calls), C.byref(ms), C.byref(carved)))
        return {"bytes_held": held.value, "hipmalloc_calls": calls.value, "hipmalloc_ms": ms.value, "carved_blocks": carved.value}

    def stage_ms(self):
        return {self.L.tmc2_ctx_stage_name(self.h, i).decode(): self.L.tmc2_ctx_stage_ms(self.h, i)
                for i in range(self.L.tmc2_ctx_stage_count(self.h))}

    def stage_calls(self):
        return {self.L.tmc2_ctx_stage_name(self.h, i).decode(): self.L.tmc2_ctx_stage_calls(self.h, i)
                for i in range(self.L.tmc2_ctx_stage_count(self.h))}

    def stage_reset(self):
        self.L.tmc2_ctx_stage_reset(self.h)

    def set_timing(self, enabled):
        self.L.tmc2_ctx_set_timing(self.h, 1 if enabled else 0)

    def frame(self, xyz, rgb=None):
        return Frame(self, xyz, rgb)

    def transfer_colors(self, src_xyz, src_rgb, tgt_xyz):
        a = np.ascontiguousarray(src_xyz, np.int16)
        b = np.ascontiguousarray(src_rgb, np.uint8)
        c = np.ascontiguousarray(tgt_xyz, np.int16)
        if a.shape != b.shape:
            raise Tmc2Error("transfer_colors: %d source points, %d source colours" % (len(a), len(b)))
        out = np.zeros((len(c), 3), np.uint8)
        _check(self.L.tmc2_transfer_colors(self.h, _ptr(a), _ptr(b), len(a), _ptr(c), len(c), _ptr(out)))
        return out

    def convert_points_to_voxels(self, xyz, vox_dim, bits3d):
        a = np.ascontiguousarray(xyz, np.int16).reshape(-1, 3)
        vox, rank, count = np.zeros((len(a), 3), np.int16), np.zeros(len(a), np.uint32), C.c_uint64()
        _check(self.L.tmc2_segmenter_convert_points_to_voxels(self.h, _ptr(a), len(a), int(vox_dim), int(bits3d), _ptr(vox), C.byref(count),
                                                              _ptr(rank)))
        return vox[:count.value].copy(), rank

    def color_smoothing(self, xyz, colors16, boundary, patch_index, grid_size, bits3d, thr_smoothing=10.0, thr_difference=10.0,
                        thr_variation=6.0):
        a = _color_smoothing_arrays(xyz, colors16, boundary, patch_index)
        _check(self.L.tmc2_color_smoothing(self.h, _ptr(a[0]), _ptr(a[1]), _ptr(a[2]), _ptr(a[3]), len(a[0]), int(grid_size),
                                          int(bits3d), thr_smoothing, thr_difference, thr_variation))
        return a[1]

    def decoder_frame(self, patches, width, height, occ_precision, occ_video, geometry):
        pt = np.ascontiguousarray(patches, dtype=PATCH_DTYPE)
        ov = np.ascontiguousarray(occ_video, dtype=np.uint8)
        geo = np.ascontiguousarray(geometry, dtype=np.uint16)
        if ov.shape != (height // occ_precision, width // occ_precision) or geo.shape != (2, height, width):
            raise ValueError("decoded canvases do not match %dx%d at precision %d" % (width, height, occ_precision))
        fr = Frame.__new__(Frame)
        fr.L, fr.ctx, fr.h = self.L, self, C.c_void_p()
        fr._xyz, fr._rgb, fr.n = None, None, 0
        _check(self.L.tmc2_decoder_frame_create(self.h, _ptr(pt), len(pt), int(width), int(height), int(occ_precision), _ptr(ov),
                                               _ptr(geo), C.byref(fr.h)))
        fr._canvas = (int(width), int(height), int(occ_precision))
        return fr

    def color_convert_rgb444_to_yuv420(self, rgb, downsampling_filter=4):
        rgb = np.ascontiguousarray(rgb, dtype=np.uint8)
        _, H, W = rgb.shape
        out = np.zeros(W * H * 3 // 2, np.uint8)
        _check(self.L.tmc2_color_convert_rgb444_to_yuv420(self.h, _ptr(rgb), int(W), int(H), int(downsampling_filter), _ptr(out)))
        a = W * H
        return out[:a].reshape(H, W), out[a:a + a // 4].reshape(H // 2, W // 2), out[a + a // 4:].reshape(H // 2, W // 2)

    def color_convert_yuv420_to_yuv444(self, y, u, v, upsampling_filter=0):
        H, W = y.shape
        src = np.concatenate([np.ascontiguousarray(a, dtype=np.uint8).reshape(-1) for a in (y, u, v)])
        out = np.zeros((3, H, W), np.uint16)
        _check(self.L.tmc2_color_convert_yuv420_to_yuv444(self.h, _ptr(src), int(W), int(H), int(upsampling_filter), _ptr(out)))
        return out

    def metrics_compute(self, src_xyz, src_rgb, rec_xyz, rec_rgb, normals=None, resolution=1023.0):
        a = np.ascontiguousarray(src_xyz, np.int16)
        b = np.ascontiguousarray(src_rgb, np.uint8)
        c = np.ascontiguousarray(rec_xyz, np.int16)
        d = np.ascontiguousarray(rec_rgb, np.uint8)
        nm = None if normals is None else np.ascontiguousarray(normals, np.float64)
        out = np.zeros((3, 8), np.float64)
        counts = np.zeros(2, np.int64)
        _check(self.L.tmc2_metrics_compute(self.h, _ptr(a), _ptr(b), len(a), _ptr(c), _ptr(d), len(c),
                                           None if nm is None else _ptr(nm), resolution, _ptr(out), _ptr(counts)))
        return out, counts

    def metrics_ordered_sums(self, terms_a, terms_b):
        a = np.ascontiguousarray(terms_a, np.float64).reshape(-1, 5)
        b = np.ascontiguousarray(terms_b, np.float64).reshape(-1, 5)
        out = np.zeros(10, np.float64)
        _check(self.L.tmc2_metrics_ordered_sums(self.h, _ptr(a) if len(a) else None, len(a), _ptr(b) if len(b) else None, len(b), _ptr(out)))
        return out


class Frame:

    def __init__(self, ctx, xyz, rgb=None):
        self.ctx, self.L = ctx, ctx.L
        xyz = np.ascontiguousarray(xyz, dtype=np.int16)
        assert xyz.ndim == 2 and xyz.shape[1] == 3
        self.n = len(xyz)
        self._xyz = xyz
        self._rgb = None if rgb is None else np.ascontiguousarray(rgb, dtype=np.uint8)
        self.h = C.c_void_p()
        _check(self.L.tmc2_frame_create(ctx.h, _ptr(xyz), None if rgb is None else _ptr(self._rgb), self.n, C.byref(self.h)))

    def close(self):
        if self.h:
            self.L.tmc2_frame_destroy(self.h)
            self.h = C.c_void_p()

    def __del__(self):
        try:
            self.close()
        except Exception:
            pass

    def reset(self):
        _check(self.L.tmc2_frame_reset(self.h))

    def metrics_compute(self, which=0, use_normals=True, resolution=1023.0):
        out = np.zeros((3, 8), np.float64)
        counts = np.zeros(2, np.int64)
        _check(self.L.tmc2_metrics_compute_frame(self.h, which, 1 if use_normals else 0, resolution, _ptr(out), _ptr(counts)))
        return out, counts

    def metrics_compute_source(self, src_xyz, src_rgb, normals=None, which=1, resolution=1023.0):
        a = np.ascontiguousarray(src_xyz, np.int16)
        b = np.ascontiguousarray(src_rgb, np.uint8)
        nm = None if normals is None else np.ascontiguousarray(normals, np.float64)
        out = np.zeros((3, 8), np.float64)
        counts = np.zeros(2, np.int64)
        _check(self.L.tmc2_metrics_compute_frame_source(self.h, which, _ptr(a), _ptr(b), len(a),
                                                        None if nm is None else _ptr(nm), resolution, _ptr(out), _ptr(counts)))
        return out, counts

    def kdtree_build(self):
        _check(self.L.tmc2_kdtree_build(self.h))

    def kdtree_order(self):
        perm = np.empty(self.n, np.uint32)
        depth = C.c_int32()
        _check(self.L.tmc2_frame_get_kdtree_order(self.h, _ptr(perm), C.byref(depth)))
        return perm, depth.value

    def device_images(self):
        W, H, p = self._canvas
        ptrs = [C.c_void_p() for _ in range(4)]
        _check(self.L.tmc2_frame_device_images(self.h, *[C.byref(x) for x in ptrs]))
        out = dict(occupancy=(ptrs[0].value, (H, W), "|u1"), occ_video=(ptrs[1].value, (H // p, W // p), "|u1"),
                   block_to_patch=(ptrs[2].value, (H // 16, W // 16), "<u4"), geometry=(ptrs[3].value, (2, H, W), "<u2"))
        a = C.c_void_p()
        if self.L.tmc2_frame_device_attribute(self.h, C.byref(a)) == 0:
            out["attribute"] = (a.value, (2, 3, H, W), "|u1")
        return out

    def kdtree_search(self, queries, k, with_dist=False):
        q = np.ascontiguousarray(queries, dtype=np.int16)
        idx = np.empty((len(q), k), np.uint32)
        d = np.empty((len(q), k), np.uint32) if with_dist else None
        _check(self.L.tmc2_kdtree_search(self.h, _ptr(q), len(q), int(k), _ptr(idx), None if d is None else _ptr(d)))
        return (idx, d) if with_dist else idx

    def kdtree_search_wide(self, k, queries=None):
        q = None if queries is None else np.ascontiguousarray(queries, dtype=np.int16).reshape(-1, 3)
        nq = self.n if q is None else len(q)
        idx = np.empty((nq, max(int(k), 0) if int(k) <= 1024 else 0), np.uint32)
        _check(self.L.tmc2_kdtree_search_wide(self.h, None if q is None else _ptr(q), nq, int(k), _ptr(idx)))
        return idx

    def normals_compute_normals(self, k=16):
        _check(self.L.tmc2_normals_compute_normals(self.h, int(k)))

    def normals_orient(self):
        _check(self.L.tmc2_normals_orient(self.h))

    def normals_compute(self, k=16, orientation=1):
        _check(self.L.tmc2_normals_compute(self.h, int(k), int(orientation)))

    def get_normals(self):
        out = np.empty((self.n, 3), np.float64)
        _check(self.L.tmc2_frame_get_normals(self.h, _ptr(out)))
        return out

    def set_normals(self, normals):
        a = np.ascontiguousarray(normals, dtype=np.float64)
        _check(self.L.tmc2_frame_set_normals(self.h, _ptr(a)))

    def get_adjacency(self, k=16):
        out = np.empty((self.n, k), np.uint32)
        _check(self.L.tmc2_frame_get_adjacency(self.h, _ptr(out)))
        return out

    def weight_normal(self, bits3d=11, min_weight_epp=0.6):
        w = (C.c_double * 3)()
        _check(self.L.tmc2_weight_normal(self.h, int(bits3d), min_weight_epp, w))
        return np.array([w[0], w[1], w[2]])

    def segmenter_initial_segmentation(self, weight):
        w = (C.c_double * 3)(*[float(x) for x in weight])
        _check(self.L.tmc2_segmenter_initial_segmentation(self.h, w))

    def segmenter_refine_grid_based(self, max_nn=1024, lam=3.0, iterations=10, vox_dim=4, radius=192):
        _check(self.L.tmc2_segmenter_refine_grid_based(self.h, int(max_nn), lam, int(iterations), int(vox_dim), int(radius)))

    def segmenter_refine(self, max_nn=256, lam=3.0, iterations=100):
        _check(self.L.tmc2_segmenter_refine(self.h, int(max_nn), lam, int(iterations)))

    def get_partition(self):
        out = np.empty(self.n, np.uint32)
        _check(self.L.tmc2_frame_get_partition(self.h, _ptr(out)))
        return out

    def set_partition(self, partition):
        a = np.ascontiguousarray(partition, dtype=np.uint32)
        _check(self.L.tmc2_frame_set_partition(self.h, _ptr(a)))

    def segmenter_segment_patches(self, params):
        _check(self.L.tmc2_segmenter_segment_patches(self.h, C.byref(params)))

    def segmenter_compute(self, params, grid_based=None):
        if not params.gridBasedRefineSegmentation:
            _check(self.L.tmc2_segmenter_compute_knn_refine(self.h, C.byref(params), 0 if grid_based is None else int(grid_based)))
        elif grid_based is None:
            _check(self.L.tmc2_segmenter_compute(self.h, C.byref(params)))
        else:
            _check(self.L.tmc2_segmenter_compute_grid_based(self.h, C.byref(params), int(grid_based)))

    def get_patches(self):
        cnt = self.L.tmc2_frame_patch_count(self.h)
        dc, oc = C.c_int64(), C.c_int64()
        _check(self.L.tmc2_frame_patch_pool_sizes(self.h, C.byref(dc), C.byref(oc)))
        patches = np.zeros(cnt, PATCH_DTYPE)
        d0 = np.zeros(dc.value, np.int16)
        d1 = np.zeros(dc.value, np.int16)
        occ = np.zeros(oc.value, np.uint8)
        _check(self.L.tmc2_frame_get_patches(self.h, _ptr(patches), _ptr(d0), _ptr(d1), _ptr(occ)))
        return patches, d0, d1, occ


    def get_patch_records(self):
        cnt = self.L.tmc2_frame_patch_count(self.h)
        dc, oc = C.c_int64(), C.c_int64()
        _check(self.L.tmc2_frame_patch_pool_sizes(self.h, C.byref(dc), C.byref(oc)))
        patches, occ = np.zeros(cnt, PATCH_DTYPE), np.zeros(oc.value, np.uint8)
        _check(self.L.tmc2_frame_get_patches(self.h, _ptr(patches), None, None, _ptr(occ)))
        return patches, occ

    def set_packing(self, patch_list, matches, occupancy, packed_width, packed_height):
        p = np.ascontiguousarray(patch_list, dtype=PATCH_DTYPE)
        occ = np.ascontiguousarray(occupancy, dtype=np.uint8)
        m = None if matches is None else np.ascontiguousarray(matches, dtype=np.int32)
        _check(self.L.tmc2_frame_set_packing(self.h, _ptr(p), len(p), None if m is None else _ptr(m), _ptr(occ), len(occ),
                                             int(packed_width), int(packed_height)))

    def encoder_pack_flexible(self, preset_width=1280, tiles_hor=2, ratio=1.0):
        h = C.c_int32()
        _check(self.L.tmc2_encoder_pack_flexible(self.h, int(preset_width), int(tiles_hor), ratio, C.byref(h)))
        return h.value

    def encoder_pack_spatial_consistency(self, previous, preset_width=1280, tiles_hor=2, ratio=1.0):
        h = C.c_int32()
        _check(self.L.tmc2_encoder_pack_spatial_consistency(self.h, previous.h, int(preset_width), int(tiles_hor), ratio, C.byref(h)))
        return h.value

    def get_packed_size(self):
        w, h = C.c_int32(), C.c_int32()
        _check(self.L.tmc2_frame_get_packed_size(self.h, C.byref(w), C.byref(h)))
        return w.value, h.value

    def get_patch_matches(self):
        m = np.zeros(self.L.tmc2_frame_patch_count(self.h), np.int32)
        _check(self.L.tmc2_frame_get_patch_matches(self.h, _ptr(m)))
        return m

    def get_patch_order(self):
        order = np.zeros(self.L.tmc2_frame_patch_count(self.h), np.int32)
        _check(self.L.tmc2_frame_get_patch_order(self.h, _ptr(order)))
        return order

    def encoder_generate_geometry_images(self, width, height, occ_precision=4):
        _check(self.L.tmc2_encoder_generate_geometry_images(self.h, int(width), int(height), int(occ_precision)))
        self._canvas = (int(width), int(height), int(occ_precision))

    def get_geometry_images(self, out=None):
        W, H, p = self._canvas
        if out is None:
            out = dict(occupancy=np.zeros((H, W), np.uint8), occ_video=np.zeros((H // p, W // p), np.uint8),
                       block_to_patch=np.zeros((H // 16, W // 16), np.uint32), geo0=np.zeros((H, W), np.uint16),
                       geo1=np.zeros((H, W), np.uint16))
        _check(self.L.tmc2_frame_get_geometry_images(self.h, _ptr(out["occupancy"]), _ptr(out["occ_video"]),
                                                     _ptr(out["block_to_patch"]), _ptr(out["geo0"]), _ptr(out["geo1"])))
        return out


    def encoder_generate_attribute_images(self):
        self._pbf = False
        _check(self.L.tmc2_encoder_generate_attribute_images(self.h))

    def recon_count(self):
        return self.L.tmc2_frame_recon_count(self.h)

    def get_reconstruction(self, colors=True):
        M = self.L.tmc2_frame_recon_count(self.h)
        xyz, rgb, p2p = np.zeros((M, 3), np.int16), (np.zeros((M, 3), np.uint8) if colors else None), np.zeros((M, 3), np.uint32)
        _check(self.L.tmc2_frame_get_reconstruction(self.h, _ptr(xyz), None if rgb is None else _ptr(rgb), _ptr(p2p)))
        return xyz, rgb, p2p

    def codec_generate_point_cloud(self, pbf=None):
        self._pbf = pbf is not None
        if pbf is None:
            _check(self.L.tmc2_codec_generate_point_cloud(self.h))
            return
        passes, filter_size, log2_threshold, threshold_om = (tuple(pbf) + (0,))[:4]
        _check(self.L.tmc2_codec_generate_point_cloud_pbf(self.h, int(threshold_om), int(passes), int(filter_size), int(log2_threshold)))

    def get_patch_border_filtering(self):
        n = C.c_int64()
        _check(self.L.tmc2_frame_patch_border_filtering_size(self.h, C.byref(n)))
        occ, border = np.zeros(n.value, np.uint8), np.zeros(n.value, np.uint8)
        _check(self.L.tmc2_frame_get_patch_border_filtering(self.h, _ptr(occ), _ptr(border)))
        return occ, border

    def codec_identify_boundary_points(self):
        _check(self.L.tmc2_codec_identify_boundary_points(self.h))

    def encoder_attribute_to_yuv420(self, downsampling_filter=4, out=None):
        W, H, _ = self._canvas
        if out is None:
            out = np.zeros((2, W * H * 3 // 2), np.uint8)
        _check(self.L.tmc2_encoder_attribute_to_yuv420(self.h, int(downsampling_filter), _ptr(out)))
        return out

    def codec_set_decoded_attribute_yuv420(self, yuv420, upsampling_filter=0):
        W, H, _ = self._canvas
        src = np.ascontiguousarray(yuv420, dtype=np.uint8)
        if src.size != 2 * (W * H * 3 // 2):
            raise ValueError("decoded I420 frames must hold 2 x %d bytes" % (W * H * 3 // 2))
        _check(self.L.tmc2_codec_set_decoded_attribute_yuv420(self.h, _ptr(src), int(upsampling_filter)))

    def get_decoded_attribute(self):
        W, H, _ = self._canvas
        out = np.zeros((2, 3, H, W), np.uint16)
        _check(self.L.tmc2_frame_get_decoded_attribute(self.h, _ptr(out)))
        return out

    def codec_color_point_cloud(self, attribute16=None):
        if attribute16 is None:
            _check(self.L.tmc2_codec_color_point_cloud(self.h, None))
            return
        W, H, _ = self._canvas
        att = np.ascontiguousarray(attribute16, dtype=np.uint16)
        if att.shape != (2, 3, H, W):
            raise ValueError("decoded attribute frames must be uint16 [2][3][%d][%d]" % (H, W))
        _check(self.L.tmc2_codec_color_point_cloud(self.h, _ptr(att)))

    def codec_smooth_point_cloud_postprocess(self, grid_size=8, threshold=64.0):
        _check(self.L.tmc2_codec_smooth_point_cloud_postprocess(self.h, int(grid_size), threshold))

    def codec_transfer_colors_16bit_bp(self):
        _check(self.L.tmc2_codec_transfer_colors_16bit_bp(self.h))

    def codec_convert_yuv16_to_rgb8(self):
        _check(self.L.tmc2_codec_convert_yuv16_to_rgb8(self.h))

    def set_geometry_bit_depth_3d(self, bits3d):
        _check(self.L.tmc2_frame_set_geometry_bit_depth_3d(self.h, int(bits3d)))

    def codec_color_smoothing(self, grid_size, thr_smoothing=10.0, thr_difference=10.0, thr_variation=6.0):
        _check(self.L.tmc2_codec_color_smoothing(self.h, int(grid_size), thr_smoothing, thr_difference, thr_variation))

    def codec_post_reconstruct(self, attribute16=None, grid_size=8, threshold=64.0, color_smoothing=None, pbf=None):
        if pbf is not None:
            self.codec_generate_point_cloud(pbf)
        else:
            if getattr(self, "_pbf", False):
                self.codec_generate_point_cloud()
            self.codec_identify_boundary_points()
        self.codec_color_point_cloud(attribute16)
        self.codec_smooth_point_cloud_postprocess(grid_size, threshold)
        if pbf is None:
            self.codec_transfer_colors_16bit_bp()
        if color_smoothing is not None:
            self.codec_color_smoothing(*color_smoothing)
        self.codec_convert_yuv16_to_rgb8()

    def get_post_reconstruction(self, xyz=True, colors16=True, rgb=True, boundary=True):
        M = self.L.tmc2_frame_recon_count(self.h)
        out = dict(xyz=np.zeros((M, 3), np.int16) if xyz else None, colors16=np.zeros((M, 3), np.uint16) if colors16 else None,
                   rgb=np.zeros((M, 3), np.uint8) if rgb else None, boundary=np.zeros(M, np.uint16) if boundary else None)
        _check(self.L.tmc2_frame_get_post_reconstruction(self.h, *[None if out[k] is None else _ptr(out[k])
                                                                    for k in ("xyz", "colors16", "rgb", "boundary")]))
        return {k: v for k, v in out.items() if v is not None}

    def get_attribute_images(self, out=None):
        W, H, _ = self._canvas
        if out is None:
            out = np.zeros((2, 3, H, W), np.uint8)
        _check(self.L.tmc2_frame_get_attribute_images(self.h, _ptr(out)))
        return out

    def set_decoded_geometry(self, occ_video=None, geometry=None):
        ov = None if occ_video is None else np.ascontiguousarray(occ_video, dtype=np.uint8)
        g = None if geometry is None else np.ascontiguousarray(geometry, dtype=np.uint16)
        _check(self.L.tmc2_frame_set_decoded_geometry(self.h, None if ov is None else _ptr(ov), None if g is None else _ptr(g)))


class _Pinned:

    def __init__(self, nbytes):
        self.L, self.p, self.nbytes = load_library(), C.c_void_p(), int(nbytes)
        _check(self.L.tmc2_host_alloc(self.nbytes, C.byref(self.p)))
        self.__array_interface__ = dict(shape=(self.nbytes,), typestr="|u1", data=(self.p.value, False), version=3)

    def __del__(self):
        try:
            if self.p:
                self.L.tmc2_host_free(self.p)
                self.p = C.c_void_p()
        except Exception:
            pass


class SharedHostArray:

    def __init__(self, name, nbytes, create, register=True):
        import mmap
        self.path, self.nbytes, self.created, self.registered = os.path.join("/dev/shm", name), int(nbytes), bool(create), False
        fd = os.open(self.path, (os.O_CREAT | os.O_RDWR) if create else os.O_RDWR, 0o600)
        try:
            if create:
                os.ftruncate(fd, self.nbytes)
            self.map = mmap.mmap(fd, self.nbytes)
        finally:
            os.close(fd)
        self.array = np.frombuffer(self.map, dtype=np.uint8)
        if register:
            _check(load_library().tmc2_host_register(C.c_void_p(self.array.ctypes.data), self.nbytes))
            self.registered = True

    def close(self):
        if self.registered:
            rc = load_library().tmc2_host_unregister(C.c_void_p(self.array.ctypes.data))
            self.registered = False
            if rc != 0:
                raise Tmc2Error("tmc2_host_unregister(%s) failed: %d" % (self.path, rc))
        if self.created:
            try:
                os.unlink(self.path)
            except OSError:
                pass
            self.created = False


def host_array(shape, dtype=np.uint8):
    dtype = np.dtype(dtype)
    n = int(np.prod(shape)) * dtype.itemsize
    return np.asarray(_Pinned(max(n, 1)))[:n].view(dtype).reshape(shape)


def encoder_canvas_size(heights, tile_width=1280, min_w=1280, min_h=1280):
    L = load_library()
    hs = np.ascontiguousarray(heights, dtype=np.int32)
    W, H = C.c_int32(), C.c_int32()
    _check(L.tmc2_encoder_canvas_size(_ptr(hs), len(hs), int(tile_width), int(min_w), int(min_h), C.byref(W), C.byref(H)))
    return W.value, H.value


def host_kdtree_build(xyz):
    L = load_library()
    xyz = np.ascontiguousarray(xyz, dtype=np.int16)
    perm = np.empty(len(xyz), np.uint32)
    nodes, depth = C.c_uint64(), C.c_int32()
    _check(L.tmc2_host_kdtree_build(_ptr(xyz), len(xyz), _ptr(perm), C.byref(nodes), C.byref(depth)))
    return perm, nodes.value, depth.value


def host_pack_flexible(patches, occupancy, preset_width=1280, tiles_hor=2, ratio=1.0):
    L = load_library()
    p = np.array(patches, dtype=PATCH_DTYPE, order="C", copy=True)
    occ = np.ascontiguousarray(occupancy, dtype=np.uint8)
    order, h = np.zeros(len(p), np.int32), C.c_int32()
    _check(L.tmc2_host_pack_flexible(_ptr(p), len(p), _ptr(occ), int(preset_width), int(tiles_hor), ratio, _ptr(order),
                                     C.byref(h)))
    return p, order, h.value


def host_pack_spatial_consistency(patches, occupancy, previous_list, preset_width=1280, tiles_hor=2, ratio=1.0):
    L = load_library()
    p = np.array(patches, dtype=PATCH_DTYPE, order="C", copy=True)
    prev = np.ascontiguousarray(previous_list, dtype=PATCH_DTYPE)
    occ = np.ascontiguousarray(occupancy, dtype=np.uint8)
    order, match, h = np.zeros(len(p), np.int32), np.zeros(len(p), np.int32), C.c_int32()
    _check(L.tmc2_host_pack_spatial_consistency(_ptr(p), len(p), _ptr(occ), _ptr(prev), len(prev), int(preset_width),
                                                int(tiles_hor), ratio, _ptr(order), _ptr(match), C.byref(h)))
    return p, order, match, h.value


def encoder_global_patch_allocation(frames, min_w=1280, min_h=1280):
    L = load_library()
    n = len(frames)
    handles = (C.c_void_p * n)(*[fr.h for fr in frames])
    w, h = np.zeros(n, np.int32), np.zeros(n, np.int32)
    _check(L.tmc2_encoder_global_patch_allocation(handles, n, int(min_w), int(min_h), _ptr(w), _ptr(h)))
    return w, h


def host_global_patch_allocation(lists, pools, matches, tile_w, tile_h, min_w=1280, min_h=1280):
    L = load_library()
    n = len(lists)
    counts = np.array([len(x) for x in lists], np.int32)
    patches = np.ascontiguousarray(np.concatenate([np.asarray(x, dtype=PATCH_DTYPE) for x in lists]), dtype=PATCH_DTYPE)
    m = np.ascontiguousarray(np.concatenate([np.asarray(x, dtype=np.int32) for x in matches]), dtype=np.int32)
    pools = [np.ascontiguousarray(x, dtype=np.uint8) for x in pools]
    base = np.zeros(n, np.int64)
    base[1:] = np.cumsum([len(x) for x in pools])[:-1]
    occ = np.ascontiguousarray(np.concatenate(pools)) if n else np.zeros(0, np.uint8)
    cap = int(len(patches) * max(1, int(patches["sizeU0"].max(initial=1))) * max(1, int(patches["sizeV0"].max(initial=1))))
    out, out_base = np.zeros(max(cap, 1), np.uint8), np.zeros(n + 1, np.int64)
    w, h = np.zeros(n, np.int32), np.zeros(n, np.int32)
    _check(L.tmc2_host_global_patch_allocation(n, _ptr(counts), _ptr(patches), _ptr(occ), _ptr(base), _ptr(m), int(tile_w),
                                               int(tile_h), int(min_w), int(min_h), _ptr(out), cap, _ptr(out_base),
                                               _ptr(w), _ptr(h)))
    res, at = [], 0
    for f in range(n):
        c = int(counts[f])
        res.append((patches[at:at + c].copy(), out[out_base[f]:out_base[f + 1] if f + 1 < n else out_base[n]].copy(),
                    m[at:at + c].copy(), int(w[f]), int(h[f])))
        at += c
    return res


def host_pack_gof_records(records, mode, min_w=1280, min_h=1280, tiles_hor=2, ratio=1.0):
    L = load_library()
    n = len(records)
    if n == 0:
        return []
    counts = np.array([len(r) for r, _ in records], np.int32)
    patches = np.ascontiguousarray(np.concatenate([np.asarray(r, dtype=PATCH_DTYPE) for r, _ in records]), dtype=PATCH_DTYPE)
    pools = [np.ascontiguousarray(o, dtype=np.uint8) for _, o in records]
    base = np.zeros(n, np.int64)
    base[1:] = np.cumsum([len(x) for x in pools])[:-1]
    occ = np.ascontiguousarray(np.concatenate(pools))
    cap = int(len(patches) * max(1, int(patches["sizeU0"].max(initial=1))) * max(1, int(patches["sizeV0"].max(initial=1)))) if mode == 2 else len(occ)
    out, out_base = np.zeros(max(cap, 1), np.uint8), np.zeros(n + 1, np.int64)
    m = np.zeros(max(len(patches), 1), np.int32)
    w, h = np.zeros(n, np.int32), np.zeros(n, np.int32)
    _check(L.tmc2_host_place_segments(n, _ptr(counts), _ptr(patches), _ptr(occ), _ptr(base), int(mode), int(min_w), int(min_h),
                                      int(tiles_hor), ratio, _ptr(m), _ptr(out), cap, _ptr(out_base), _ptr(w), _ptr(h)))
    res, at = [], 0
    for f in range(n):
        c = int(counts[f])
        res.append((patches[at:at + c].copy(), out[out_base[f]:out_base[f + 1]].copy(), m[at:at + c].copy(), int(w[f]), int(h[f])))
        at += c
    return res


def segmenter_params_check(params):
    _check(load_library().tmc2_segmenter_params_check(C.byref(params)))


def metrics_display(out, source_points, reconstruct_points, counts, resolution=1023, with_c2p=True, precision=9):
    L = load_library()
    q = np.ascontiguousarray(out, dtype=np.float64)
    c = np.ascontiguousarray(counts, dtype=np.int64)
    need = C.c_uint64()
    _check(L.tmc2_metrics_display(_ptr(q), int(source_points), int(reconstruct_points), _ptr(c), int(resolution), int(bool(with_c2p)),
                                  int(precision), None, 0, C.byref(need)))
    buf = C.create_string_buffer(need.value)
    _check(L.tmc2_metrics_display(_ptr(q), int(source_points), int(reconstruct_points), _ptr(c), int(resolution), int(bool(with_c2p)),
                                  int(precision), buf, need.value, None))
    return buf.value.decode()


def checksum_file_write(path, digests):
    L = load_library()
    d = np.frombuffer(b"".join(digests), np.uint8).copy() if len(digests) else np.zeros(0, np.uint8)
    _check(L.tmc2_checksum_file_write(str(path).encode(), _ptr(d) if len(d) else None, len(digests)))


def checksum_file_read(path):
    L = load_library()
    n = C.c_uint64()
    _check(L.tmc2_checksum_file_read(str(path).encode(), None, 0, C.byref(n)))
    d = np.zeros(16 * max(1, n.value), np.uint8)
    _check(L.tmc2_checksum_file_read(str(path).encode(), _ptr(d), n.value, C.byref(n)))
    return [d[16 * f:16 * f + 16].tobytes() for f in range(n.value)]


def ply_info(path, read_normals=False):
    L = load_library()
    n, c, m = C.c_uint64(), C.c_int(), C.c_int()
    _check(L.tmc2_ply_info(str(path).encode(), int(bool(read_normals)), C.byref(n), C.byref(c), C.byref(m)))
    return n.value, bool(c.value), bool(m.value)


def ply_read(path, read_normals=False, threads=0, out=None):
    L = load_library()
    n, has_rgb, has_nrm = ply_info(path, read_normals)
    if out is not None:
        xyz, rgb = out
        if len(xyz) < n or (rgb is not None and len(rgb) < n):
            raise ValueError("buffers too small for %d points" % n)
    else:
        xyz, rgb = np.zeros((n, 3), np.int16), (np.zeros((n, 3), np.uint8) if has_rgb else None)
    nrm = np.zeros((n, 3), np.float64) if has_nrm else None
    cnt = C.c_uint64()
    _check(L.tmc2_ply_read(str(path).encode(), _ptr(xyz), None if rgb is None or not has_rgb else _ptr(rgb),
                           None if nrm is None else _ptr(nrm), len(xyz), int(threads), C.byref(cnt)))
    return xyz[:n], (rgb[:n] if rgb is not None and has_rgb else None), nrm


def ply_write(path, xyz, rgb=None, normals=None, ascii=True):
    L = load_library()
    xyz = np.ascontiguousarray(xyz, dtype=np.int16)
    rgb = None if rgb is None else np.ascontiguousarray(rgb, dtype=np.uint8)
    nrm = None if normals is None else np.ascontiguousarray(normals, dtype=np.float64)
    _check(L.tmc2_ply_write(str(path).encode(), _ptr(xyz), None if rgb is None else _ptr(rgb), None if nrm is None else _ptr(nrm),
                            len(xyz), int(bool(ascii))))


def point_set_checksum(xyz, rgb=None, reorder=False):
    L = load_library()
    xyz = np.ascontiguousarray(xyz, dtype=np.int16)
    rgb = None if rgb is None else np.ascontiguousarray(rgb, dtype=np.uint8)
    d = np.zeros(16, np.uint8)
    _check(L.tmc2_point_set_checksum(_ptr(xyz), None if rgb is None else _ptr(rgb), len(xyz), int(bool(reorder)), _ptr(d)))
    return d.tobytes()


def host_orient_normals(xyz, knn, normals):
    L = load_library()
    xyz = np.ascontiguousarray(xyz, dtype=np.int16)
    knn = np.ascontiguousarray(knn, dtype=np.uint32)
    out = np.array(normals, dtype=np.float64, order="C", copy=True)
    _check(L.tmc2_host_orient_normals(_ptr(xyz), len(xyz), _ptr(knn), int(knn.shape[1]), _ptr(out)))
    return out


def _color_smoothing_arrays(xyz, colors16, boundary, patch_index):
    xyz = np.ascontiguousarray(xyz, dtype=np.int16)
    out = np.array(colors16, dtype=np.uint16, order="C", copy=True)
    bt = np.ascontiguousarray(boundary, dtype=np.uint16)
    patch = np.ascontiguousarray(patch_index, dtype=np.uint32)
    if xyz.shape != (len(xyz), 3) or out.shape != xyz.shape or bt.shape != (len(xyz),) or patch.shape != (len(xyz),):
        raise Tmc2Error("color_smoothing: xyz [M][3], colors16 [M][3], boundary [M] and patch_index [M] of one M expected")
    return xyz, out, bt, patch


def host_color_smoothing(xyz, colors16, boundary, patch_index, grid_size, bits3d, thr_smoothing=10.0, thr_difference=10.0,
                         thr_variation=6.0):
    L = load_library()
    a = _color_smoothing_arrays(xyz, colors16, boundary, patch_index)
    _check(L.tmc2_host_color_smoothing(_ptr(a[0]), _ptr(a[1]), _ptr(a[2]), _ptr(a[3]), len(a[0]), int(grid_size), int(bits3d),
                                       thr_smoothing, thr_difference, thr_variation))
    return a[1]


def host_patch_border_filtering(patches, width, height, occ_precision, occ_video, geometry_d0, block_to_patch, passes, filter_size,
                                log2_threshold, threshold_om=0):
    L = load_library()
    pt = np.ascontiguousarray(patches, dtype=PATCH_DTYPE)
    ov = np.ascontiguousarray(occ_video, dtype=np.uint8)
    geo = np.ascontiguousarray(geometry_d0, dtype=np.uint16)
    b2p = np.ascontiguousarray(block_to_patch, dtype=np.uint32)
    if width <= 0 or height <= 0 or occ_precision <= 0 or ov.size != (height // occ_precision) * (width // occ_precision) or \
            geo.size != height * width or b2p.size != (height // 16) * (width // 16):
        raise Tmc2Error("host_patch_border_filtering: canvases do not match %dx%d at precision %d" % (width, height, occ_precision))
    n = int(sum(int(t["sizeU0"]) * int(t["sizeV0"]) * 256 for t in pt if t["sizeU0"] > 0 and t["sizeV0"] > 0))
    occ, border = np.zeros(n, np.uint8), np.zeros(n, np.uint8)
    _check(L.tmc2_host_patch_border_filtering(_ptr(pt), len(pt), int(width), int(height), int(occ_precision), _ptr(ov), _ptr(geo), _ptr(b2p),
                                              int(threshold_om), int(passes), int(filter_size), int(log2_threshold), _ptr(occ), _ptr(border)))
    return occ, border


def host_convert_points_to_voxels(xyz, vox_dim, bits3d):
    a = np.ascontiguousarray(xyz, np.int16).reshape(-1, 3)
    vox, rank, count = np.zeros((len(a), 3), np.int16), np.zeros(len(a), np.uint32), C.c_uint64()
    _check(load_library().tmc2_host_convert_points_to_voxels(_ptr(a), len(a), int(vox_dim), int(bits3d), _ptr(vox), C.byref(count), _ptr(rank)))
    return vox[:count.value].copy(), rank


def host_refine_segmentation(xyz, normals, partition, max_nn=256, lam=3.0, iterations=100, with_adjacency=False):
    a = np.ascontiguousarray(xyz, np.int16).reshape(-1, 3)
    nrm = np.ascontiguousarray(normals, np.float64).reshape(-1, 3)
    out = np.array(partition, dtype=np.uint32, order="C", copy=True).reshape(-1)
    if len(nrm) != len(a) or len(out) != len(a):
        raise Tmc2Error("host_refine_segmentation: xyz [n][3], normals [n][3] and partition [n] of one n expected")
    adj = np.zeros((len(a), max(int(max_nn), 0) if int(max_nn) <= 1024 else 0), np.uint32) if with_adjacency else None
    _check(load_library().tmc2_host_refine_segmentation(_ptr(a), len(a), _ptr(nrm), _ptr(out), int(max_nn), lam, int(iterations),
                                                        None if adj is None else _ptr(adj)))
    return (out, adj) if with_adjacency else out


def selftest_std_sort(pairs, offsets):
    out = np.ascontiguousarray(pairs, dtype=np.uint32).copy()
    off = np.ascontiguousarray(offsets, dtype=np.uint32)
    if out.ndim != 2 or out.shape[1] != 2 or len(off) < 1 or int(off[-1]) != len(out) or (np.diff(off.astype(np.int64)) < 0).any():
        raise Tmc2Error("selftest_std_sort: pairs [total][2] and rising offsets that end at total expected")
    _check(load_library().tmc2_selftest_std_sort(_ptr(out), _ptr(off), len(off) - 1))
    return out


TMC2HIP = """
int tmc2_ctx_create(int, tmc2_ctx**)
void tmc2_ctx_destroy(tmc2_ctx*)
const char* tmc2_last_error(void)
int tmc2_ctx_synchronize(tmc2_ctx*)
int tmc2_host_alloc(size_t, void**)
void tmc2_host_free(void*)
int tmc2_host_register(void*, size_t)
int tmc2_host_unregister(void*)
int tmc2_host_gate_create(int, tmc2_host_gate**)
void tmc2_host_gate_destroy(tmc2_host_gate*)
int tmc2_ctx_set_host_gate(tmc2_ctx*, tmc2_host_gate*)
void tmc2_set_host_parallelism(int)
int tmc2_ctx_set_option(tmc2_ctx*, const char*, const char*)
const char* tmc2_ctx_get_option(tmc2_ctx*, const char*)
int tmc2_ctx_reserve(tmc2_ctx*, uint64_t, int, int, int, int)
int tmc2_ctx_pool_stats(tmc2_ctx*, uint64_t*, uint64_t*, double*, uint64_t*)
int tmc2_ctx_device_alloc(tmc2_ctx*, size_t, void**)
int tmc2_ctx_device_free(tmc2_ctx*, void*)
int tmc2_ctx_upload(tmc2_ctx*, void*, const void*, size_t)
int tmc2_ctx_download(tmc2_ctx*, void*, const void*, size_t)
void* tmc2_ctx_stream(tmc2_ctx*)
int tmc2_ctx_device(tmc2_ctx*)
int tmc2_ctx_make_current(tmc2_ctx*)
int tmc2_ctx_stage_count(tmc2_ctx*)
const char* tmc2_ctx_stage_name(tmc2_ctx*, int)
double tmc2_ctx_stage_ms(tmc2_ctx*, int)
long tmc2_ctx_stage_calls(tmc2_ctx*, int)
void tmc2_ctx_stage_reset(tmc2_ctx*)
void tmc2_ctx_set_timing(tmc2_ctx*, int)
int tmc2_frame_create(tmc2_ctx*, const int16_t*, const uint8_t*, uint64_t, tmc2_frame**)
void tmc2_frame_destroy(tmc2_frame*)
int tmc2_kdtree_build(tmc2_frame*)
void tmc2_set_kdtree_placement(int)
void tmc2_set_refine_overlap(int)
int tmc2_frame_get_kdtree_order(tmc2_frame*, uint32_t*, int32_t*)
uint64_t tmc2_frame_point_count(const tmc2_frame*)
int tmc2_frame_reset(tmc2_frame*)
int tmc2_kdtree_search(tmc2_frame*, const int16_t*, uint64_t, int, uint32_t*, uint32_t*)
int tmc2_kdtree_search_wide(tmc2_frame*, const int16_t*, uint64_t, int, uint32_t*)
int tmc2_normals_compute_normals(tmc2_frame*, int)
int tmc2_normals_orient(tmc2_frame*)
int tmc2_normals_compute(tmc2_frame*, int, int)
int tmc2_frame_get_normals(tmc2_frame*, double*)
int tmc2_frame_set_normals(tmc2_frame*, const double*)
int tmc2_frame_get_adjacency(tmc2_frame*, uint32_t*)
int tmc2_weight_normal(tmc2_frame*, int, double, double[3])
int tmc2_segmenter_initial_segmentation(tmc2_frame*, const double[3])
int tmc2_segmenter_refine_grid_based(tmc2_frame*, int, double, int, int, int)
int tmc2_segmenter_refine(tmc2_frame*, int, double, int)
int tmc2_frame_get_partition(tmc2_frame*, uint32_t*)
int tmc2_frame_set_partition(tmc2_frame*, const uint32_t*)
int tmc2_segmenter_segment_patches(tmc2_frame*, const tmc2_segmenter_params*)
int tmc2_segmenter_compute(tmc2_frame*, const tmc2_segmenter_params*)
int tmc2_segmenter_params_check(const tmc2_segmenter_params*)
int tmc2_segmenter_compute_grid_based(tmc2_frame*, const tmc2_segmenter_params*, int)
int tmc2_segmenter_compute_knn_refine(tmc2_frame*, const tmc2_segmenter_params*, int)
int tmc2_segmenter_convert_points_to_voxels(tmc2_ctx*, const int16_t*, uint64_t, int, int, int16_t*, uint64_t*, uint32_t*)
int tmc2_frame_patch_count(tmc2_frame*)
int tmc2_frame_patch_pool_sizes(tmc2_frame*, int64_t*, int64_t*)
int tmc2_frame_get_patches(tmc2_frame*, tmc2_patch*, int16_t*, int16_t*, uint8_t*)
int tmc2_encoder_pack_flexible(tmc2_frame*, int, int, double, int32_t*)
int tmc2_encoder_pack_spatial_consistency(tmc2_frame*, tmc2_frame*, int, int, double, int32_t*)
int tmc2_frame_get_packed_size(tmc2_frame*, int32_t*, int32_t*)
int tmc2_frame_get_patch_matches(tmc2_frame*, int32_t*)
int tmc2_encoder_global_patch_allocation(tmc2_frame**, int, int, int, int32_t*, int32_t*)
int tmc2_frame_set_packing(tmc2_frame*, const tmc2_patch*, int, const int32_t*, const uint8_t*, int64_t, int, int)
int tmc2_frame_get_patch_order(tmc2_frame*, int32_t*)
int tmc2_encoder_canvas_size(const int32_t*, int, int, int, int, int32_t*, int32_t*)
int tmc2_encoder_generate_geometry_images(tmc2_frame*, int, int, int)
int tmc2_frame_get_geometry_images(tmc2_frame*, uint8_t*, uint8_t*, uint32_t*, uint16_t*, uint16_t*)
int tmc2_encoder_generate_attribute_images(tmc2_frame*)
int tmc2_transfer_colors(tmc2_ctx*, const int16_t*, const uint8_t*, uint64_t, const int16_t*, uint64_t, uint8_t*)
int64_t tmc2_frame_recon_count(tmc2_frame*)
int tmc2_frame_get_reconstruction(tmc2_frame*, int16_t*, uint8_t*, uint32_t*)
int tmc2_frame_get_attribute_images(tmc2_frame*, uint8_t*)
int tmc2_frame_set_decoded_geometry(tmc2_frame*, const uint8_t*, const uint16_t*)
int tmc2_frame_device_images(tmc2_frame*, void**, void**, void**, void**)
int tmc2_frame_device_attribute(tmc2_frame*, void**)
int tmc2_color_convert_rgb444_to_yuv420(tmc2_ctx*, const uint8_t*, int, int, int, uint8_t*)
int tmc2_color_convert_yuv420_to_yuv444(tmc2_ctx*, const uint8_t*, int, int, int, uint16_t*)
int tmc2_encoder_attribute_to_yuv420(tmc2_frame*, int, uint8_t*)
int tmc2_codec_set_decoded_attribute_yuv420(tmc2_frame*, const uint8_t*, int)
int tmc2_frame_get_decoded_attribute(tmc2_frame*, uint16_t*)
int tmc2_decoder_frame_create(tmc2_ctx*, const tmc2_patch*, int, int, int, int, const uint8_t*, const uint16_t*, tmc2_frame**)
int tmc2_codec_generate_point_cloud(tmc2_frame*)
int tmc2_codec_generate_point_cloud_pbf(tmc2_frame*, int, int, int, int)
int tmc2_frame_patch_border_filtering_size(tmc2_frame*, int64_t*)
int tmc2_frame_get_patch_border_filtering(tmc2_frame*, uint8_t*, uint8_t*)
int tmc2_codec_identify_boundary_points(tmc2_frame*)
int tmc2_codec_color_point_cloud(tmc2_frame*, const uint16_t*)
int tmc2_codec_smooth_point_cloud_postprocess(tmc2_frame*, int, double)
int tmc2_codec_transfer_colors_16bit_bp(tmc2_frame*)
int tmc2_codec_color_smoothing(tmc2_frame*, int, double, double, double)
int tmc2_frame_set_geometry_bit_depth_3d(tmc2_frame*, int)
int tmc2_color_smoothing(tmc2_ctx*, const int16_t*, uint16_t*, const uint16_t*, const uint32_t*, uint64_t, int, int, double, double, double)
int tmc2_codec_convert_yuv16_to_rgb8(tmc2_frame*)
int tmc2_frame_get_post_reconstruction(tmc2_frame*, int16_t*, uint16_t*, uint8_t*, uint16_t*)
int tmc2_metrics_compute(tmc2_ctx*, const int16_t*, const uint8_t*, uint64_t, const int16_t*, const uint8_t*, uint64_t, const double*, double, double*, int64_t*)
int tmc2_metrics_compute_frame(tmc2_frame*, int, int, double, double*, int64_t*)
int tmc2_metrics_compute_frame_source(tmc2_frame*, int, const int16_t*, const uint8_t*, uint64_t, const double*, double, double*, int64_t*)
int tmc2_metrics_ordered_sums(tmc2_ctx*, const double*, uint64_t, const double*, uint64_t, double*)
int tmc2_metrics_display(const double*, uint64_t, uint64_t, const int64_t*, uint64_t, int, int, char*, uint64_t, uint64_t*)
int tmc2_ply_info(const char*, int, uint64_t*, int*, int*)
int tmc2_ply_read(const char*, int16_t*, uint8_t*, double*, uint64_t, int, uint64_t*)
int tmc2_ply_write(const char*, const int16_t*, const uint8_t*, const double*, uint64_t, int)
int tmc2_point_set_checksum(const int16_t*, const uint8_t*, uint64_t, int, uint8_t[16])
int tmc2_checksum_file_write(const char*, const uint8_t*, uint64_t)
int tmc2_checksum_file_read(const char*, uint8_t*, uint64_t, uint64_t*)
int tmc2_host_kdtree_build(const int16_t*, uint64_t, uint32_t*, uint64_t*, int32_t*)
int tmc2_host_pack_flexible(tmc2_patch*, int, const uint8_t*, int, int, double, int32_t*, int32_t*)
int tmc2_host_global_patch_allocation(int, int32_t*, tmc2_patch*, const uint8_t*, const int64_t*, int32_t*, int, int, int, int, uint8_t*, int64_t, int64_t*, int32_t*, int32_t*)
int tmc2_host_pack_spatial_consistency(tmc2_patch*, int, const uint8_t*, const tmc2_patch*, int, int, int, double, int32_t*, int32_t*, int32_t*)
int tmc2_host_place_segments(int, const int32_t*, tmc2_patch*, const uint8_t*, const int64_t*, int, int, int, int, double, int32_t*, uint8_t*, int64_t, int64_t*, int32_t*, int32_t*)
int tmc2_host_orient_normals(const int16_t*, uint64_t, const uint32_t*, int, double*)
int tmc2_host_color_smoothing(const int16_t*, uint16_t*, const uint16_t*, const uint32_t*, uint64_t, int, int, double, double, double)
int tmc2_host_patch_border_filtering(const tmc2_patch*, int, int, int, int, const uint8_t*, const uint16_t*, const uint32_t*, int, int, int, int, uint8_t*, uint8_t*)
int tmc2_host_convert_points_to_voxels(const int16_t*, uint64_t, int, int, int16_t*, uint64_t*, uint32_t*)
int tmc2_host_refine_segmentation(const int16_t*, uint64_t, const double*, uint32_t*, int, double, int, uint32_t*)
int tmc2_selftest_scan(tmc2_ctx*, const uint32_t*, uint32_t*, uint64_t, uint32_t*, uint32_t*, const uint32_t*, int, uint64_t)
int tmc2_selftest_fill(tmc2_ctx*, const uint64_t*, int)
int tmc2_selftest_work_map(tmc2_ctx*, uint64_t, int, uint64_t, uint64_t, uint32_t*, uint32_t*)
int tmc2_selftest_components(tmc2_ctx*, const uint32_t*, const uint8_t*, const uint8_t*, const uint32_t*, uint64_t, uint32_t*, uint32_t*)
int tmc2_selftest_union_find(tmc2_ctx*, int, uint32_t*, uint64_t, const uint32_t*, uint64_t, int, int, uint32_t*, uint32_t*, uint32_t*)
int tmc2_selftest_cand_sort(tmc2_ctx*, uint32_t*, const uint32_t*, uint64_t, uint32_t*)
int tmc2_selftest_std_sort(uint32_t*, const uint32_t*, uint64_t)
int tmc2_selftest_marked_cells(tmc2_ctx*, const int16_t*, const uint8_t*, uint64_t, int, int, int, uint32_t*, uint32_t*, uint32_t*, const uint32_t*, uint64_t, uint32_t*)
""".strip().split("\n")
```

Baseline: 197.8.

## Vectorise push-pull padding and group dilation with packed byte words and pitched levels

Rewrites the attribute push-pull padding to work on 32-bit words of four pixels. It uses pitched per-level buffers, SWAR occupancy masks and reciprocal-multiply averaging in the mip kernel. The tiled fill+blur kernel now runs with 256 threads, keeps a per-word free-pixel mask in shared memory, and exits early for tiles with no empty pixels. Group dilation of the geometry images now processes four 16-bit pixels per thread using a packed average. It also adds a standalone attribute_images API, at the cost of more intricate bit tricks and edge handling.

```diff
diff --git a/include/tmc2hip.h b/include/tmc2hip.h
--- a/include/tmc2hip.h
+++ b/include/tmc2hip.h
@@ -146,6 +146,8 @@
 int     tmc2_encoder_generate_attribute_images( tmc2_frame* f );
 int     tmc2_transfer_colors( tmc2_ctx* ctx, const int16_t* srcXyz, const uint8_t* srcRgb, uint64_t n, const int16_t* tgtXyz,
                               uint64_t m, uint8_t* tgtRgb );
+int     tmc2_attribute_images( tmc2_ctx* ctx, const uint8_t* rgb, const uint32_t* pointToPixel, uint64_t M, const uint8_t* occVideo,
+                               int W, int H, int occPrecision, uint8_t* out );
 int64_t tmc2_frame_recon_count( tmc2_frame* f );
 int     tmc2_frame_get_reconstruction( tmc2_frame* f, int16_t* xyz, uint8_t* rgb, uint32_t* pointToPixel );
 int     tmc2_frame_get_attribute_images( tmc2_frame* f, uint8_t* attribute );
diff --git a/mpeg-pcc-tmc2_amd/csrc/attributes.hip b/mpeg-pcc-tmc2_amd/csrc/attributes.hip
--- a/mpeg-pcc-tmc2_amd/csrc/attributes.hip
+++ b/mpeg-pcc-tmc2_amd/csrc/attributes.hip
@@ -1,5 +1,7 @@
 #include <algorithm>
 #include <cmath>
+#include <cstdlib>
+#include <vector>
 
 #include "color_transfer.h"
 #include "internal.h"
@@ -163,192 +165,284 @@
 }
 
 __global__ __launch_bounds__( 256 ) void upsampleOccupancyKernel( const uint8_t* __restrict__ occVideo, int W, int H, int prec,
-                                                                   uint8_t* __restrict__ occ ) {
+                                                                   uint32_t* __restrict__ occ ) {
   const size_t c = size_t( blockIdx.x ) * blockDim.x + threadIdx.x;
-  if ( c >= size_t( W ) * H ) return;
-  occ[c] = occVideo[size_t( ( c / W ) / prec ) * ( W / prec ) + ( c % W ) / prec];
-}
+  const int    Ww = W >> 2;
+  if ( c >= size_t( Ww ) * H ) return;
+  const int      x   = int( c % Ww ) * 4, y = int( c / Ww );
+  const uint8_t* row = occVideo + size_t( y / prec ) * ( W / prec );
+  uint32_t       o   = 0;
+#pragma unroll
+  for ( int k = 0; k < 4; ++k ) o |= uint32_t( row[( x + k ) / prec] ) << ( 8 * k );
+  occ[c] = o;
+}
+
+struct PushPullLevel {
+  int      w, h, pitch;
+  uint8_t *img, *tmp, *occ;
+};
+__host__ __device__ __forceinline__ size_t planeBytes( const PushPullLevel& l ) { return size_t( l.pitch ) * l.h; }
+
+__device__ __forceinline__ uint32_t nonzeroBytes( uint32_t o ) {
+  const uint32_t t = ( ( ( o & 0x7F7F7F7Fu ) + 0x7F7F7F7Fu ) | o ) & 0x80808080u;
+  return ( t >> 7 ) * 0xFFu;
+}
+__device__ __forceinline__ uint32_t lowBytes( int n ) { return n >= 4 ? 0xFFFFFFFFu : ( 1u << ( 8 * n ) ) - 1u; }
+__device__ __forceinline__ uint32_t pairSums( uint32_t v ) { return ( v & 0x00FF00FFu ) + ( ( v >> 8 ) & 0x00FF00FFu ); }
 
 __device__ __forceinline__ int mean4w( int p1, int w1, int p2, int w2, int p3, int w3, int p4, int w4 ) {
   return ( p1 * w1 + p2 * w2 + p3 * w3 + p4 * w4 ) / ( w1 + w2 + w3 + w4 );
 }
 
-__device__ __forceinline__ void pushPullMipPixel( int i, const uint8_t* img, const uint8_t* occ, int W, int H, uint8_t* mip,
-                                                  uint8_t* mipOcc, int w, int h, int p0 = 0, int p1 = 6 ) {
+__device__ __forceinline__ void pushPullMipPixel( int i, const uint8_t* img, const uint8_t* occ, int W, int H, int P, uint8_t* mip,
+                                                  uint8_t* mipOcc, int w, int p ) {
   const int  x = i % w, y = i / w, X = 2 * x, Y = 2 * y;
   const bool i2 = X + 1 < W, i3 = Y + 1 < H;
-  const int  w1 = occ[size_t( Y ) * W + X] ? 255 : 0;
-  const int  w2 = ( i2 && occ[size_t( Y ) * W + X + 1] ) ? 255 : 0;
-  const int  w3 = ( i3 && occ[size_t( Y + 1 ) * W + X] ) ? 255 : 0;
-  const int  w4 = ( i2 && i3 && occ[size_t( Y + 1 ) * W + X + 1] ) ? 255 : 0;
+  const int  w1 = occ[Y * P + X] ? 255 : 0;
+  const int  w2 = ( i2 && occ[Y * P + X + 1] ) ? 255 : 0;
+  const int  w3 = ( i3 && occ[( Y + 1 ) * P + X] ) ? 255 : 0;
+  const int  w4 = ( i2 && i3 && occ[( Y + 1 ) * P + X + 1] ) ? 255 : 0;
   const bool any = ( w1 + w2 + w3 + w4 ) > 0;
-  mipOcc[i]      = any ? 1 : 0;
-  for ( int p = p0; p < p1; ++p ) {
-    const uint8_t* s = img + size_t( p ) * W * H;
-    uint8_t        v = 0;
-    if ( any ) {
-      const int v1 = s[size_t( Y ) * W + X], v2 = i2 ? s[size_t( Y ) * W + X + 1] : 0;
-      const int v3 = i3 ? s[size_t( Y + 1 ) * W + X] : 0, v4 = ( i2 && i3 ) ? s[size_t( Y + 1 ) * W + X + 1] : 0;
-      v            = uint8_t( mean4w( v1, w1, v2, w2, v3, w3, v4, w4 ) );
-    }
-    mip[size_t( p ) * w * h + i] = v;
-  }
-}
-__global__ __launch_bounds__( 256 ) void pushPullMipKernel( const uint8_t* __restrict__ img, const uint8_t* __restrict__ occ, int W,
-                                                             int H, uint8_t* __restrict__ mip, uint8_t* __restrict__ mipOcc, int w,
-                                                             int h ) {
+  mipOcc[y * p + x] = any ? 1 : 0;
+  uint8_t v         = 0;
+  if ( any ) {
+    const int v1 = img[Y * P + X], v2 = i2 ? img[Y * P + X + 1] : 0;
+    const int v3 = i3 ? img[( Y + 1 ) * P + X] : 0, v4 = ( i2 && i3 ) ? img[( Y + 1 ) * P + X + 1] : 0;
+    v            = uint8_t( mean4w( v1, w1, v2, w2, v3, w3, v4, w4 ) );
+  }
+  mip[y * p + x] = v;
+}
+
+__global__ __launch_bounds__( 256 ) void pushPullMipKernel( PushPullLevel F, PushPullLevel C ) {
+  const int cw = ( C.w + 3 ) >> 2, i = blockIdx.x * blockDim.x + threadIdx.x;
+  if ( i >= cw * C.h ) return;
+  const int      wx = i % cw, y = i / cw, X = 8 * wx, Y = 2 * y;
+  const bool     row1 = Y + 1 < F.h;
+  const uint32_t va = lowBytes( min( F.w - X, 4 ) ), vb = F.w - X > 4 ? lowBytes( min( F.w - X - 4, 4 ) ) : 0u;
+  const size_t   g0 = size_t( Y ) * F.pitch + X, g1 = g0 + F.pitch;
+  auto           word = []( const uint8_t* p, size_t at ) { return *reinterpret_cast<const uint32_t*>( p + at ); };
+  const uint32_t o0a = nonzeroBytes( word( F.occ, g0 ) ) & va, o0b = vb ? nonzeroBytes( word( F.occ, g0 + 4 ) ) & vb : 0u;
+  const uint32_t o1a = row1 ? nonzeroBytes( word( F.occ, g1 ) ) & va : 0u, o1b = ( row1 && vb ) ? nonzeroBytes( word( F.occ, g1 + 4 ) ) & vb : 0u;
+  const uint32_t one = 0x01010101u;
+  const uint32_t cntA = pairSums( o0a & one ) + pairSums( o1a & one ), cntB = pairSums( o0b & one ) + pairSums( o1b & one );
+  const uint32_t cnt[4] = {cntA & 0xFFFFu, cntA >> 16, cntB & 0xFFFFu, cntB >> 16};
+  uint32_t       rcp[4], occOut = 0;
+#pragma unroll
+  for ( int k = 0; k < 4; ++k ) {
+    rcp[k] = cnt[k] == 1 ? 1u << 17 : cnt[k] == 2 ? 1u << 16 : cnt[k] == 3 ? 0xAAABu : 1u << 15;
+    occOut |= ( cnt[k] ? 1u : 0u ) << ( 8 * k );
+  }
+  *reinterpret_cast<uint32_t*>( C.occ + size_t( y ) * C.pitch + 4 * wx ) = occOut;
+  const size_t fp = planeBytes( F ), cp = planeBytes( C );
+  for ( int p = 0; p < 6; ++p ) {
+    const uint8_t* s = F.img + p * fp;
+    const uint32_t sA = pairSums( o0a ? word( s, g0 ) & o0a : 0u ) + pairSums( o1a ? word( s, g1 ) & o1a : 0u );
+    const uint32_t sB = pairSums( o0b ? word( s, g0 + 4 ) & o0b : 0u ) + pairSums( o1b ? word( s, g1 + 4 ) & o1b : 0u );
+    const uint32_t v = ( ( sA & 0xFFFFu ) * rcp[0] >> 17 ) | ( ( sA >> 16 ) * rcp[1] >> 17 ) << 8 | ( ( sB & 0xFFFFu ) * rcp[2] >> 17 ) << 16 |
+                       ( ( sB >> 16 ) * rcp[3] >> 17 ) << 24;
+    *reinterpret_cast<uint32_t*>( C.img + p * cp + size_t( y ) * C.pitch + 4 * wx ) = v;
+  }
+}
+
+__device__ __forceinline__ uint8_t pushPullFillValue( const uint8_t* m, int pitch, int w, int h, int X, int Y ) {
+  const int  x = X >> 1, y = Y >> 1, dx = ( X & 1 ) ? 1 : -1, dy = ( Y & 1 ) ? 1 : -1;
+  const bool hx = dx < 0 ? x > 0 : x < w - 1, hy = dy < 0 ? y > 0 : y < h - 1;
+  const int  v  = m[y * pitch + x];
+  const int  vx = hx ? m[y * pitch + x + dx] : 0;
+  const int  vy = hy ? m[( y + dy ) * pitch + x] : 0;
+  const int  vd = ( hx && hy ) ? m[( y + dy ) * pitch + x + dx] : 0;
+  return uint8_t( mean4w( v, 144, vx, hx ? 48 : 0, vy, hy ? 48 : 0, vd, ( hx && hy ) ? 16 : 0 ) );
+}
+__device__ __forceinline__ void pushPullFillPixel( int i, uint8_t* img, const uint8_t* occ, int W, int P, const uint8_t* mip, int w, int h,
+                                                   int p ) {
+  const int X = i % W, Y = i / W;
+  if ( !occ[Y * P + X] ) img[Y * P + X] = pushPullFillValue( mip, p, w, h, X, Y );
+}
+__device__ __forceinline__ void pushPullBlurPixel( int i, const uint8_t* s, uint8_t* dst, const uint8_t* occ, int W, int H, int P ) {
+  const int x = i % W, y = i / W;
+  if ( occ[y * P + x] ) return;
+  const int x1 = x > 0 ? x - 1 : x, y1 = y > 0 ? y - 1 : y, x2 = x < W - 1 ? x + 1 : x, y2 = y < H - 1 ? y + 1 : y;
+  const int sum = s[y1 * P + x1] + s[y1 * P + x2] + s[y2 * P + x1] + s[y2 * P + x2] + s[y * P + x1] + s[y * P + x2] + s[y1 * P + x] +
+                  s[y2 * P + x];
+  dst[y * P + x] = uint8_t( ( sum + 4 ) >> 3 );
+}
+
+__global__ __launch_bounds__( 256 ) void pushPullFillKernel( PushPullLevel F, PushPullLevel C ) {
   const int i = blockIdx.x * blockDim.x + threadIdx.x;
-  if ( i < w * h ) pushPullMipPixel( i, img, occ, W, H, mip, mipOcc, w, h );
-}
-
-__device__ __forceinline__ void pushPullFillPixel( int i, uint8_t* img, const uint8_t* occ, int W, int H, const uint8_t* mip, int w,
-                                                   int h, int p0 = 0, int p1 = 6 ) {
-  if ( occ[i] ) return;
-  const int  X = i % W, Y = i / W, x = X >> 1, y = Y >> 1;
-  const int  dx = ( X & 1 ) ? 1 : -1, dy = ( Y & 1 ) ? 1 : -1;
-  const bool hx = dx < 0 ? x > 0 : x < w - 1, hy = dy < 0 ? y > 0 : y < h - 1;
-  for ( int p = p0; p < p1; ++p ) {
-    const uint8_t* m  = mip + size_t( p ) * w * h;
-    const int      v  = m[size_t( y ) * w + x];
-    const int      vx = hx ? m[size_t( y ) * w + x + dx] : 0;
-    const int      vy = hy ? m[size_t( y + dy ) * w + x] : 0;
-    const int      vd = ( hx && hy ) ? m[size_t( y + dy ) * w + x + dx] : 0;
-    img[size_t( p ) * W * H + i] = uint8_t( mean4w( v, 144, vx, hx ? 48 : 0, vy, hy ? 48 : 0, vd, ( hx && hy ) ? 16 : 0 ) );
-  }
-}
-__global__ __launch_bounds__( 256 ) void pushPullFillKernel( uint8_t* __restrict__ img, const uint8_t* __restrict__ occ, int W, int H,
-                                                              const uint8_t* __restrict__ mip, int w, int h ) {
+  if ( i < F.w * F.h )
+    pushPullFillPixel( i, F.img + blockIdx.y * planeBytes( F ), F.occ, F.w, F.pitch, C.img + blockIdx.y * planeBytes( C ), C.w, C.h, C.pitch );
+}
+__global__ __launch_bounds__( 256 ) void pushPullBlurKernel( PushPullLevel F, const uint8_t* __restrict__ src, uint8_t* __restrict__ dst ) {
   const int i = blockIdx.x * blockDim.x + threadIdx.x;
-  if ( i < W * H ) pushPullFillPixel( i, img, occ, W, H, mip, w, h );
-}
-
-__device__ __forceinline__ void pushPullBlurPixel( int i, const uint8_t* src, uint8_t* dst, const uint8_t* occ, int W, int H, int p0 = 0,
-                                                   int p1 = 6 ) {
-  if ( occ[i] ) return;
-  const int x = i % W, y = i / W;
-  const int x1 = x > 0 ? x - 1 : x, y1 = y > 0 ? y - 1 : y, x2 = x < W - 1 ? x + 1 : x, y2 = y < H - 1 ? y + 1 : y;
-  for ( int p = p0; p < p1; ++p ) {
-    const uint8_t* s   = src + size_t( p ) * W * H;
-    const int      sum = s[size_t( y1 ) * W + x1] + s[size_t( y1 ) * W + x2] + s[size_t( y2 ) * W + x1] + s[size_t( y2 ) * W + x2] +
-                    s[size_t( y ) * W + x1] + s[size_t( y ) * W + x2] + s[size_t( y1 ) * W + x] + s[size_t( y2 ) * W + x];
-    dst[size_t( p ) * W * H + i] = uint8_t( ( sum + 4 ) >> 3 );
-  }
-}
-__global__ __launch_bounds__( 256 ) void pushPullBlurKernel( const uint8_t* __restrict__ src, uint8_t* __restrict__ dst,
-                                                              const uint8_t* __restrict__ occ, int W, int H ) {
-  const int i = blockIdx.x * blockDim.x + threadIdx.x;
-  if ( i < W * H ) pushPullBlurPixel( i, src, dst, occ, W, H );
+  if ( i < F.w * F.h ) pushPullBlurPixel( i, src + blockIdx.y * planeBytes( F ), dst + blockIdx.y * planeBytes( F ), F.occ, F.w, F.h, F.pitch );
 }
 
 constexpr int kPushPullTile = 96, kPushPullSpan = 128, kPushPullMaxIters = ( kPushPullSpan - kPushPullTile ) / 2;
-__global__ __launch_bounds__( 1024 ) void pushPullFillBlurKernel( uint8_t* __restrict__ img, const uint8_t* __restrict__ occ, int W,
-                                                                   int H, const uint8_t* __restrict__ mip, int w, int h, int iters,
-                                                                   int tilesX ) {
-  __shared__ uint8_t sOcc[kPushPullSpan * kPushPullSpan];
-  __shared__ uint8_t sBuf[2][kPushPullSpan * kPushPullSpan];
-  const int      X0 = ( blockIdx.x % tilesX ) * kPushPullTile, Y0 = ( blockIdx.x / tilesX ) * kPushPullTile;
-  const int      RX0 = max( X0 - iters, 0 ), RY0 = max( Y0 - iters, 0 );
-  const int      RW = min( X0 + kPushPullTile + iters, W ) - RX0, RH = min( Y0 + kPushPullTile + iters, H ) - RY0;
-  uint8_t*       plane = img + size_t( blockIdx.y ) * W * H;
-  const uint8_t* m     = mip + size_t( blockIdx.y ) * w * h;
-  for ( int i = threadIdx.x; i < kPushPullSpan * RH; i += 1024 ) {
-    const int rx = i & ( kPushPullSpan - 1 ), ry = i >> 7;
-    if ( rx >= RW ) continue;
-    const int     X = RX0 + rx, Y = RY0 + ry;
-    const size_t  g = size_t( Y ) * W + X;
-    const uint8_t o = occ[g];
-    uint8_t       v;
-    if ( o ) {
-      v = plane[g];
-    } else {
-      const int  x = X >> 1, y = Y >> 1, dx = ( X & 1 ) ? 1 : -1, dy = ( Y & 1 ) ? 1 : -1;
-      const bool hx = dx < 0 ? x > 0 : x < w - 1, hy = dy < 0 ? y > 0 : y < h - 1;
-      const int  c  = m[size_t( y ) * w + x];
-      const int  vx = hx ? m[size_t( y ) * w + x + dx] : 0;
-      const int  vy = hy ? m[size_t( y + dy ) * w + x] : 0;
-      const int  vd = ( hx && hy ) ? m[size_t( y + dy ) * w + x + dx] : 0;
-      v             = uint8_t( mean4w( c, 144, vx, hx ? 48 : 0, vy, hy ? 48 : 0, vd, ( hx && hy ) ? 16 : 0 ) );
-    }
-    sOcc[i]    = o;
+constexpr int kPushPullSpanW = kPushPullSpan / 4, kPushPullThreads = 256;
+constexpr int kPushPullStripRows = kPushPullSpan / ( kPushPullThreads / kPushPullSpanW );
+static_assert( kPushPullSpanW == 32 && kPushPullTile % 4 == 0 && kPushPullMaxIters % 4 == 0, "word indexing of the fill + blur tile" );
+__global__ __launch_bounds__( kPushPullThreads ) void pushPullFillBlurKernel( PushPullLevel F, PushPullLevel C, int iters, int tilesX ) {
+  __shared__ uint8_t  sFree[kPushPullSpanW * kPushPullSpan];
+  __shared__ uint32_t sBuf[2][kPushPullSpanW * kPushPullSpan];
+  const int tid = threadIdx.x;
+  const int X0 = ( blockIdx.x % tilesX ) * kPushPullTile, Y0 = ( blockIdx.x / tilesX ) * kPushPullTile;
+  const int X1 = min( X0 + kPushPullTile, F.w ), Y1 = min( Y0 + kPushPullTile, F.h );
+  const int mx = ( iters + 3 ) & ~3;
+  const int RX0 = max( X0 - mx, 0 ), RY0 = max( Y0 - iters, 0 );
+  const int RW = min( X0 + kPushPullTile + mx, F.w ) - RX0, RH = min( Y0 + kPushPullTile + iters, F.h ) - RY0, RWw = ( RW + 3 ) >> 2;
+  uint8_t*       plane = F.img + blockIdx.y * planeBytes( F );
+  const uint8_t* m     = C.img + blockIdx.y * planeBytes( C );
+  int            any   = 0;
+  for ( int i = tid; i < kPushPullSpanW * RH; i += kPushPullThreads ) {
+    const int wx = i & ( kPushPullSpanW - 1 ), ry = i >> 5;
+    if ( wx >= RWw ) continue;
+    const int      X = RX0 + 4 * wx, Y = RY0 + ry;
+    const uint32_t o = *reinterpret_cast<const uint32_t*>( F.occ + size_t( Y ) * F.pitch + X );
+    const uint32_t f = ~nonzeroBytes( o ) & lowBytes( min( F.w - X, 4 ) ) & 0x01010101u;
+    const uint32_t bits = ( f | f >> 7 | f >> 14 | f >> 21 ) & 0xFu;
+    sFree[i]            = uint8_t( bits );
+    if ( bits && X >= X0 && X < X1 && Y >= Y0 && Y < Y1 ) any = 1;
+  }
+  if ( !__syncthreads_or( any ) ) return;
+  for ( int i = tid; i < kPushPullSpanW * RH; i += kPushPullThreads ) {
+    const int wx = i & ( kPushPullSpanW - 1 ), ry = i >> 5;
+    if ( wx >= RWw ) continue;
+    const int      X = RX0 + 4 * wx, Y = RY0 + ry, n = min( F.w - X, 4 );
+    const uint32_t bits = sFree[i];
+    uint32_t       v    = bits != 0xFu ? *reinterpret_cast<const uint32_t*>( plane + size_t( Y ) * F.pitch + X ) : 0u;
+    if ( bits ) {
+#pragma unroll
+      for ( int k = 0; k < 4; ++k )
+        if ( bits >> k & 1u ) v = ( v & ~( 0xFFu << ( 8 * k ) ) ) | uint32_t( pushPullFillValue( m, C.pitch, C.w, C.h, X + k, Y ) ) << ( 8 * k );
+    }
+    if ( n < 4 ) v = ( v & lowBytes( n ) ) | ( ( ( v >> ( 8 * ( n - 1 ) ) ) & 0xFFu ) * 0x01010101u & ~lowBytes( n ) );
     sBuf[0][i] = v;
     sBuf[1][i] = v;
   }
   __syncthreads();
-  int cur = 0;
+  const int  wx = tid & ( kPushPullSpanW - 1 ), r0 = ( tid >> 5 ) * kPushPullStripRows, r1 = min( r0 + kPushPullStripRows, RH );
+  const bool first = wx == 0, last = wx == RWw - 1;
+  const int  wl = first ? wx : wx - 1, wr = last ? wx : wx + 1, n = min( RW - 4 * wx, 4 );
+  int        cur = 0;
   for ( int it = 0; it < iters; ++it ) {
-    const uint8_t* src = sBuf[cur];
-    uint8_t*       dst = sBuf[cur ^ 1];
-    for ( int i = threadIdx.x; i < kPushPullSpan * RH; i += 1024 ) {
-      const int rx = i & ( kPushPullSpan - 1 ), ry = i >> 7;
-      if ( rx >= RW || sOcc[i] ) continue;
-      const int l = rx > 0 ? -1 : 0, r = rx < RW - 1 ? 1 : 0;
-      const int u = ry > 0 ? -kPushPullSpan : 0, d = ry < RH - 1 ? kPushPullSpan : 0;
-      const int sum = src[i + u + l] + src[i + u + r] + src[i + d + l] + src[i + d + r] + src[i + l] + src[i + r] + src[i + u] +
-                      src[i + d];
-      dst[i] = uint8_t( ( sum + 4 ) >> 3 );
+    const uint32_t* src = sBuf[cur];
+    uint32_t*       dst = sBuf[cur ^ 1];
+    if ( wx < RWw && r0 < RH ) {
+      auto hsum = [&]( int r, uint32_t& s, uint32_t& he, uint32_t& ho ) {
+        const uint32_t* row = src + r * kPushPullSpanW;
+        s                   = row[wx];
+        const uint32_t lb = first ? s & 0xFFu : row[wl] >> 24, rb = last ? s >> 24 : row[wr] & 0xFFu;
+        const uint32_t e = s & 0x00FF00FFu, o = ( s >> 8 ) & 0x00FF00FFu;
+        he               = e + o + ( ( o << 16 ) | lb );
+        ho               = e + o + ( ( e >> 16 ) | ( rb << 16 ) );
+      };
+      uint32_t c, cn, he0, ho0, he1, ho1, he2, ho2;
+      hsum( max( r0 - 1, 0 ), c, he0, ho0 );
+      hsum( r0, c, he1, ho1 );
+      for ( int r = r0; r < r1; ++r ) {
+        hsum( min( r + 1, RH - 1 ), cn, he2, ho2 );
+        const uint32_t bits = sFree[r * kPushPullSpanW + wx];
+        if ( bits ) {
+          const uint32_t e = ( ( he0 + he1 + he2 - ( c & 0x00FF00FFu ) + 0x00040004u ) >> 3 ) & 0x00FF00FFu;
+          const uint32_t o = ( ( ho0 + ho1 + ho2 - ( ( c >> 8 ) & 0x00FF00FFu ) + 0x00040004u ) >> 3 ) & 0x00FF00FFu;
+          const uint32_t sel = ( ( bits * 0x00204081u ) & 0x01010101u ) * 0xFFu;
+          uint32_t       v   = ( ( e | o << 8 ) & sel ) | ( c & ~sel );
+          if ( n < 4 ) v = ( v & lowBytes( n ) ) | ( ( ( v >> ( 8 * ( n - 1 ) ) ) & 0xFFu ) * 0x01010101u & ~lowBytes( n ) );
+          dst[r * kPushPullSpanW + wx] = v;
+        }
+        he0 = he1, ho0 = ho1, he1 = he2, ho1 = ho2, c = cn;
+      }
     }
     __syncthreads();
     cur ^= 1;
   }
-  const uint8_t* res = sBuf[cur];
-  for ( int i = threadIdx.x; i < kPushPullSpan * RH; i += 1024 ) {
-    const int rx = i & ( kPushPullSpan - 1 ), ry = i >> 7;
-    const int X = RX0 + rx, Y = RY0 + ry;
-    if ( rx >= RW || sOcc[i] || X < X0 || X >= X0 + kPushPullTile || Y < Y0 || Y >= Y0 + kPushPullTile ) continue;
-    plane[size_t( Y ) * W + X] = res[i];
-  }
-}
-
-constexpr int kPushPullSmall  = 160 * 160;
-constexpr int kPushPullLevels = 16;
+  const uint32_t* res = sBuf[cur];
+  for ( int i = tid; i < kPushPullSpanW * RH; i += kPushPullThreads ) {
+    const int wx = i & ( kPushPullSpanW - 1 ), ry = i >> 5, X = RX0 + 4 * wx, Y = RY0 + ry;
+    if ( wx >= RWw || !sFree[i] || X < X0 || X >= X1 || Y < Y0 || Y >= Y1 ) continue;
+    *reinterpret_cast<uint32_t*>( plane + size_t( Y ) * F.pitch + X ) = res[i];
+  }
+}
+
+constexpr int    kPushPullSmall  = 160 * 160;
+constexpr int    kPushPullLevels = 16;
+constexpr size_t kPushPullCoarseLds = 64 << 10;
 struct PushPullLevels {
-  int      count;
-  int      first;
-  int      w[kPushPullLevels], h[kPushPullLevels];
-  uint8_t *img[kPushPullLevels], *tmp[kPushPullLevels], *occ[kPushPullLevels];
+  int            count;
+  int            first;
+  int            w[kPushPullLevels], h[kPushPullLevels], pitch[kPushPullLevels];
+  uint8_t*       img;
+  const uint8_t* occ;
 };
+__host__ __device__ inline size_t pushPullCoarseBytes( const PushPullLevels& L ) {
+  size_t b = size_t( L.pitch[L.first] ) * L.h[L.first];
+  for ( int l = L.first; l < L.count; ++l ) b += 2 * size_t( L.pitch[l] ) * L.h[l];
+  return b;
+}
 __global__ __launch_bounds__( 1024 ) void pushPullCoarseLevelsKernel( PushPullLevels L ) {
-  const int p0 = int( blockIdx.x ), p1 = p0 + 1;
+  extern __shared__ __align__( 16 ) uint8_t sPyr[];
+  const int tid = threadIdx.x, nt = blockDim.x;
+  {
+    const int       a   = L.pitch[L.first] * L.h[L.first];
+    const uint32_t *gi = reinterpret_cast<const uint32_t*>( L.img + size_t( blockIdx.x ) * a ), *go = reinterpret_cast<const uint32_t*>( L.occ );
+    uint32_t*       s   = reinterpret_cast<uint32_t*>( sPyr );
+    for ( int i = tid; i < a / 4; i += nt ) s[i] = gi[i], s[a / 4 + i] = go[i];
+  }
+  __syncthreads();
+  int base = 0;
   for ( int l = L.first + 1; l < L.count; ++l ) {
-    const int cnt = L.w[l] * L.h[l];
-    for ( int i = threadIdx.x; i < cnt; i += blockDim.x )
-      pushPullMipPixel( i, L.img[l - 1], L.occ[l - 1], L.w[l - 1], L.h[l - 1], L.img[l], L.occ[l], L.w[l], L.h[l], p0, p1 );
+    const int a = L.pitch[l - 1] * L.h[l - 1], b = L.pitch[l] * L.h[l], cnt = L.w[l] * L.h[l];
+    for ( int i = tid; i < cnt; i += nt )
+      pushPullMipPixel( i, sPyr + base, sPyr + base + a, L.w[l - 1], L.h[l - 1], L.pitch[l - 1], sPyr + base + 2 * a, sPyr + base + 2 * a + b,
+                        L.w[l], L.pitch[l] );
     __syncthreads();
-  }
-  int iters = 4;
+    base += 2 * a;
+  }
+  uint8_t* const partner = sPyr + base + 2 * L.pitch[L.count - 1] * L.h[L.count - 1];
+  uint8_t*       coarse  = sPyr + base;
+  int            iters   = 4;
   for ( int l = L.count - 1; l > L.first; --l ) {
-    const int fw = L.w[l - 1], fh = L.h[l - 1], cnt = fw * fh;
-    uint8_t * img = L.img[l - 1], *tmp = L.tmp[l - 1];
-    const uint8_t* occ = L.occ[l - 1];
-    for ( int i = threadIdx.x; i < cnt; i += blockDim.x ) pushPullFillPixel( i, img, occ, fw, fh, L.img[l], L.w[l], L.h[l], p0, p1 );
+    const int fw = L.w[l - 1], fh = L.h[l - 1], fp = L.pitch[l - 1], a = fp * fh, cnt = fw * fh;
+    base -= 2 * a;
+    uint8_t*       img = sPyr + base;
+    const uint8_t* occ = img + a;
+    for ( int i = tid; i < cnt; i += nt ) pushPullFillPixel( i, img, occ, fw, fp, coarse, L.w[l], L.h[l], L.pitch[l] );
     __syncthreads();
-    for ( int i = threadIdx.x; i < cnt; i += blockDim.x ) tmp[size_t( p0 ) * cnt + i] = img[size_t( p0 ) * cnt + i];
+    for ( int i = tid; i < a / 4; i += nt ) reinterpret_cast<uint32_t*>( partner )[i] = reinterpret_cast<const uint32_t*>( img )[i];
     __syncthreads();
-    uint8_t *src = img, *dst = tmp;
+    uint8_t *src = img, *dst = partner;
     for ( int it = 0; it < iters; ++it ) {
-      for ( int i = threadIdx.x; i < cnt; i += blockDim.x ) pushPullBlurPixel( i, src, dst, occ, fw, fh, p0, p1 );
+      for ( int i = tid; i < cnt; i += nt ) pushPullBlurPixel( i, src, dst, occ, fw, fh, fp );
       __syncthreads();
       uint8_t* t = src;
       src        = dst;
       dst        = t;
     }
-    if ( src != img ) {
-      L.img[l - 1] = src;
-      L.tmp[l - 1] = img;
-    }
-    iters = min( iters + 1, 16 );
-  }
-}
-
-__global__ __launch_bounds__( 256 ) void attributeGroupDilateKernel( const uint8_t* __restrict__ occ, int W, int H,
-                                                                      uint8_t* __restrict__ attr ) {
-  const size_t c = size_t( blockIdx.x ) * blockDim.x + threadIdx.x, plane = size_t( W ) * H;
-  if ( c >= plane || occ[c] ) return;
+    coarse = src;
+    iters  = min( iters + 1, 16 );
+  }
+  {
+    const int a  = L.pitch[L.first] * L.h[L.first];
+    uint32_t* gi = reinterpret_cast<uint32_t*>( L.img + size_t( blockIdx.x ) * a );
+    for ( int i = tid; i < a / 4; i += nt ) gi[i] = reinterpret_cast<const uint32_t*>( coarse )[i];
+  }
+}
+
+__device__ __forceinline__ void groupAverage( uint32_t occ, uint32_t& a, uint32_t& b ) {
+  const uint32_t keep = nonzeroBytes( occ ), avg = ( a | b ) - ( ( ( a ^ b ) >> 1 ) & 0x7F7F7F7Fu );
+  a                   = ( a & keep ) | ( avg & ~keep );
+  b                   = ( b & keep ) | ( avg & ~keep );
+}
+__global__ __launch_bounds__( 256 ) void attributeGroupDilateKernel( const uint4* __restrict__ occ, size_t plane16, uint4* __restrict__ attr ) {
+  const size_t c = size_t( blockIdx.x ) * blockDim.x + threadIdx.x;
+  if ( c >= plane16 ) return;
+  const uint4 o = occ[c];
+  if ( ( nonzeroBytes( o.x ) & nonzeroBytes( o.y ) & nonzeroBytes( o.z ) & nonzeroBytes( o.w ) ) == 0xFFFFFFFFu ) return;
 #pragma unroll
   for ( int k = 0; k < 3; ++k ) {
-    const uint32_t a = attr[k * plane + c], b = attr[( 3 + k ) * plane + c];
-    const uint8_t  v = uint8_t( ( a + b + 1 ) >> 1 );
-    attr[k * plane + c] = attr[( 3 + k ) * plane + c] = v;
+    uint4 a = attr[k * plane16 + c], b = attr[( 3 + k ) * plane16 + c];
+    groupAverage( o.x, a.x, b.x ), groupAverage( o.y, a.y, b.y ), groupAverage( o.z, a.z, b.z ), groupAverage( o.w, a.w, b.w );
+    attr[k * plane16 + c] = a, attr[( 3 + k ) * plane16 + c] = b;
   }
 }
 
@@ -463,121 +557,131 @@
   return TMC2_OK;
 }
 
-int generateAttributeImages( tmc2_frame* f ) {
-  if ( !f->haveGeometryImages ) {
-    setError( "generateAttributeImages: geometry images missing" );
-    return TMC2_E_STATE;
-  }
-  if ( f->d_rgb.count == 0 ) {
-    setError( "generateAttributeImages: the frame has no colours" );
-    return TMC2_E_STATE;
-  }
-  TMC2_TRY( f->ensureTree() );
-  TMC2_TRY( reconstructPointCloud( f ) );
-  tmc2_ctx*    ctx = f->ctx;
-  hipStream_t  s   = ctx->stream;
-  const int    W = f->canvasW, H = f->canvasH, prec = f->occPrecision;
+int attributeImagesDevice( tmc2_ctx* ctx, const uint8_t* d_rgb4, const uint32_t* d_pointToPixel, uint32_t M, const uint8_t* d_occVideo,
+                           int W, int H, int prec, uint8_t* d_attr ) {
+  hipStream_t  s    = ctx->stream;
   const size_t area = size_t( W ) * H;
   const dim3   blk( 256 );
-  const uint32_t n = uint32_t( f->n ), M = uint32_t( f->reconCount );
-  DevBuf<uint32_t> d_small;
-  TMC2_TRY( d_small.alloc( 8 ) );
-  TMC2_TRY( f->d_reconRgb.alloc( size_t( M ) * 4 ) );
-  const dim3 grdM( ( M + 255 ) / 256 );
-  volatile uint32_t* h_err = ctx->answerLine( tmc2_ctx::kAnswerAttrError );
-  TMC2_TRY( transferColorsDevice( ctx, f->tree.view( QueryBox::Tight ), f->d_pts.p, f->d_rgb.p, n, f->reconTree.view( QueryBox::Tight ),
-                                  f->d_recon.p, M, f->d_reconRgb.p, const_cast<uint32_t*>( h_err ) ) );
+  bool pixelForm = false;
+  long small     = kPushPullSmall;
+  if ( const auto e = ctxOption( ctx, "PUSHPULL_FORM" ) ) pixelForm = *e == "pixel";
+  if ( const auto e = ctxOption( ctx, "PUSHPULL_SMALL" ) ) {
+    char*      end = nullptr;
+    const long v   = strtol( e->c_str(), &end, 10 );
+    if ( end != e->c_str() && *end == 0 && v >= 0 ) small = v;
+  }
   StageScope      stage( ctx, "attribute_images" );
   DevBuf<uint8_t> d_occ;
   TMC2_TRY( d_occ.alloc( area ) );
-  TMC2_TRY( f->d_attr.alloc( 6 * area ) );
-  TMC2_HIP( hipMemsetAsync( f->d_attr.p, 0, 6 * area, s ) );
-  hipLaunchKernelGGL( upsampleOccupancyKernel, dim3( uint32_t( ( area + 255 ) / 256 ) ), blk, 0, s, f->d_occVideo.p, W, H, prec,
-                      d_occ.p );
-  hipLaunchKernelGGL( attributeScatterKernel, grdM, blk, 0, s, f->d_reconRgb.p, f->d_pointToPixel.p, M, W, H, f->d_attr.p );
-  struct Level {
-    int      w, h;
-    uint8_t *img, *tmp, *occ;
-  };
-  std::vector<Level> lv;
-  lv.push_back( Level{W, H, f->d_attr.p, nullptr, d_occ.p} );
+  TMC2_HIP( hipMemsetAsync( d_attr, 0, 6 * area, s ) );
+  hipLaunchKernelGGL( upsampleOccupancyKernel, dim3( uint32_t( ( area / 4 + 255 ) / 256 ) ), blk, 0, s, d_occVideo, W, H, prec,
+                      reinterpret_cast<uint32_t*>( d_occ.p ) );
+  if ( M ) hipLaunchKernelGGL( attributeScatterKernel, dim3( ( M + 255 ) / 256 ), blk, 0, s, d_rgb4, d_pointToPixel, M, W, H, d_attr );
+  std::vector<PushPullLevel> lv;
+  lv.push_back( PushPullLevel{W, H, W, d_attr, nullptr, d_occ.p} );
   size_t pyramidBytes = 6 * area;
   {
     int w = W, h = H;
     for ( ;; ) {
       w = ( w + 1 ) >> 1;
       h = ( h + 1 ) >> 1;
-      lv.push_back( Level{w, h, nullptr, nullptr, nullptr} );
-      pyramidBytes += size_t( w ) * h * ( 6 + 6 + 1 );
+      lv.push_back( PushPullLevel{w, h, ( w + 7 ) & ~7, nullptr, nullptr, nullptr} );
+      pyramidBytes += planeBytes( lv.back() ) * ( 6 + 6 + 1 ) + 3 * 16;
       if ( w <= 4 || h <= 4 ) break;
     }
   }
   DevBuf<uint8_t> d_pyr;
-  TMC2_TRY( d_pyr.alloc( pyramidBytes + 64 * lv.size() ) );
+  TMC2_TRY( d_pyr.alloc( pyramidBytes ) );
   {
-    uint8_t* p = d_pyr.p;
-    lv[0].tmp  = p;
-    p += 6 * area;
+    uint8_t*   p     = d_pyr.p;
+    const auto piece = [&p]( size_t bytes ) {
+      uint8_t* at = p;
+      p += ( bytes + 15 ) & ~size_t( 15 );
+      return at;
+    };
+    lv[0].tmp = piece( 6 * area );
     for ( size_t l = 1; l < lv.size(); ++l ) {
-      const size_t a = size_t( lv[l].w ) * lv[l].h;
-      lv[l].img = p, p += 6 * a;
-      lv[l].tmp = p, p += 6 * a;
-      lv[l].occ = p, p += ( a + 15 ) & ~size_t( 15 );
-    }
-  }
-  size_t firstSmall = lv.size();
-  if ( lv.size() <= size_t( kPushPullLevels ) )
-    for ( size_t l = 1; l < lv.size(); ++l )
-      if ( lv[l].w * lv[l].h <= kPushPullSmall ) {
+      lv[l].img = piece( 6 * planeBytes( lv[l] ) );
+      lv[l].tmp = piece( 6 * planeBytes( lv[l] ) );
+      lv[l].occ = piece( planeBytes( lv[l] ) );
+    }
+  }
+  size_t         firstSmall = lv.size();
+  PushPullLevels L{};
+  L.count = int( lv.size() );
+  if ( lv.size() <= size_t( kPushPullLevels ) ) {
+    for ( size_t l = 0; l < lv.size(); ++l ) L.w[l] = lv[l].w, L.h[l] = lv[l].h, L.pitch[l] = lv[l].pitch;
+    for ( size_t l = 1; l < lv.size(); ++l ) {
+      L.first = int( l );
+      if ( long( lv[l].w ) * lv[l].h <= small && pushPullCoarseBytes( L ) <= kPushPullCoarseLds ) {
         firstSmall = l;
         break;
       }
+    }
+  }
   for ( size_t l = 1; l < lv.size() && l <= firstSmall; ++l ) {
-    const int cnt = lv[l].w * lv[l].h;
-    hipLaunchKernelGGL( pushPullMipKernel, dim3( ( cnt + 255 ) / 256 ), blk, 0, s, lv[l - 1].img, lv[l - 1].occ, lv[l - 1].w,
-                        lv[l - 1].h, lv[l].img, lv[l].occ, lv[l].w, lv[l].h );
+    const int cnt = ( ( lv[l].w + 3 ) >> 2 ) * lv[l].h;
+    hipLaunchKernelGGL( pushPullMipKernel, dim3( ( cnt + 255 ) / 256 ), blk, 0, s, lv[l - 1], lv[l] );
   }
   int iters = 4;
   if ( firstSmall + 1 < lv.size() ) {
-    PushPullLevels L;
-    L.count = int( lv.size() ), L.first = int( firstSmall );
-    for ( size_t l = 0; l < lv.size(); ++l ) L.w[l] = lv[l].w, L.h[l] = lv[l].h, L.img[l] = lv[l].img, L.tmp[l] = lv[l].tmp, L.occ[l] = lv[l].occ;
-    hipLaunchKernelGGL( pushPullCoarseLevelsKernel, dim3( 6 ), dim3( 1024 ), 0, s, L );
-    for ( size_t l = lv.size() - 1; l > firstSmall; --l ) {
-      if ( iters & 1 ) std::swap( lv[l - 1].img, lv[l - 1].tmp );
-      iters = std::min( iters + 1, 16 );
-    }
+    L.first = int( firstSmall ), L.img = lv[firstSmall].img, L.occ = lv[firstSmall].occ;
+    hipLaunchKernelGGL( pushPullCoarseLevelsKernel, dim3( 6 ), dim3( 1024 ), pushPullCoarseBytes( L ), s, L );
+    iters = std::min( iters + int( lv.size() - 1 - firstSmall ), 16 );
   }
   for ( size_t l = std::min( firstSmall, lv.size() - 1 ); l >= 1; --l ) {
-    Level&    fine = lv[l - 1];
-    const int cnt  = fine.w * fine.h;
-    const dim3 grd( ( cnt + 255 ) / 256 );
-    if ( iters <= kPushPullMaxIters ) {
+    PushPullLevel& fine = lv[l - 1];
+    if ( !pixelForm && iters <= kPushPullMaxIters ) {
       const int tilesX = ( fine.w + kPushPullTile - 1 ) / kPushPullTile, tilesY = ( fine.h + kPushPullTile - 1 ) / kPushPullTile;
-      hipLaunchKernelGGL( pushPullFillBlurKernel, dim3( tilesX * tilesY, 6 ), dim3( 1024 ), 0, s, fine.img, fine.occ, fine.w, fine.h,
-                          lv[l].img, lv[l].w, lv[l].h, iters, tilesX );
+      hipLaunchKernelGGL( pushPullFillBlurKernel, dim3( tilesX * tilesY, 6 ), dim3( kPushPullThreads ), 0, s, fine, lv[l], iters, tilesX );
       iters = std::min( iters + 1, 16 );
       continue;
     }
-    hipLaunchKernelGGL( pushPullFillKernel, grd, blk, 0, s, fine.img, fine.occ, fine.w, fine.h, lv[l].img, lv[l].w, lv[l].h );
-    TMC2_HIP( hipMemcpyAsync( fine.tmp, fine.img, size_t( 6 ) * cnt, hipMemcpyDeviceToDevice, s ) );
+    const dim3   grd( ( fine.w * fine.h + 255 ) / 256, 6 );
+    const size_t bytes = 6 * planeBytes( fine );
+    hipLaunchKernelGGL( pushPullFillKernel, grd, blk, 0, s, fine, lv[l] );
+    TMC2_HIP( hipMemcpyAsync( fine.tmp, fine.img, bytes, hipMemcpyDeviceToDevice, s ) );
     uint8_t *src = fine.img, *dst = fine.tmp;
     for ( int it = 0; it < iters; ++it ) {
-      hipLaunchKernelGGL( pushPullBlurKernel, grd, blk, 0, s, src, dst, fine.occ, fine.w, fine.h );
+      hipLaunchKernelGGL( pushPullBlurKernel, grd, blk, 0, s, fine, src, dst );
       std::swap( src, dst );
     }
     if ( src != fine.img ) {
       if ( l - 1 == 0 )
-        TMC2_HIP( hipMemcpyAsync( fine.img, src, size_t( 6 ) * cnt, hipMemcpyDeviceToDevice, s ) );
+        TMC2_HIP( hipMemcpyAsync( fine.img, src, bytes, hipMemcpyDeviceToDevice, s ) );
       else
         std::swap( fine.img, fine.tmp );
     }
     iters = std::min( iters + 1, 16 );
   }
-  hipLaunchKernelGGL( attributeGroupDilateKernel, dim3( uint32_t( ( area + 255 ) / 256 ) ), blk, 0, s, d_occ.p, W, H, f->d_attr.p );
+  hipLaunchKernelGGL( attributeGroupDilateKernel, dim3( uint32_t( ( area / 16 + 255 ) / 256 ) ), blk, 0, s,
+                      reinterpret_cast<const uint4*>( d_occ.p ), area / 16, reinterpret_cast<uint4*>( d_attr ) );
   stage.end();
   TMC2_HIP( hipStreamSynchronize( s ) );
   TMC2_HIP( hipGetLastError() );
+  return TMC2_OK;
+}
+
+int generateAttributeImages( tmc2_frame* f ) {
+  if ( !f->haveGeometryImages ) {
+    setError( "generateAttributeImages: geometry images missing" );
+    return TMC2_E_STATE;
+  }
+  if ( f->d_rgb.count == 0 ) {
+    setError( "generateAttributeImages: the frame has no colours" );
+    return TMC2_E_STATE;
+  }
+  TMC2_TRY( f->ensureTree() );
+  TMC2_TRY( reconstructPointCloud( f ) );
+  tmc2_ctx*      ctx = f->ctx;
+  const int      W = f->canvasW, H = f->canvasH;
+  const uint32_t n = uint32_t( f->n ), M = uint32_t( f->reconCount );
+  TMC2_TRY( f->d_reconRgb.alloc( size_t( M ) * 4 ) );
+  volatile uint32_t* h_err = ctx->answerLine( tmc2_ctx::kAnswerAttrError );
+  TMC2_TRY( transferColorsDevice( ctx, f->tree.view( QueryBox::Tight ), f->d_pts.p, f->d_rgb.p, n, f->reconTree.view( QueryBox::Tight ),
+                                  f->d_recon.p, M, f->d_reconRgb.p, const_cast<uint32_t*>( h_err ) ) );
+  TMC2_TRY( f->d_attr.alloc( 6 * size_t( W ) * H ) );
+  TMC2_TRY( attributeImagesDevice( ctx, f->d_reconRgb.p, f->d_pointToPixel.p, M, f->d_occVideo.p, W, H, f->occPrecision, f->d_attr.p ) );
   const uint32_t err = *h_err;
   if ( err ) {
     setError( "transferColors: a backward candidate list hit std::sort's depth limit (heapsort fallback of libstdc++ "
@@ -591,6 +695,50 @@
 }
 
 extern "C" {
+
+int tmc2_attribute_images( tmc2_ctx* ctx, const uint8_t* rgb, const uint32_t* pointToPixel, uint64_t M, const uint8_t* occVideo, int W,
+                           int H, int occPrecision, uint8_t* out ) {
+  using namespace tmc2;
+  if ( !ctx || !occVideo || !out || ( M && ( !rgb || !pointToPixel ) ) || M > ( uint64_t( 1 ) << 31 ) || W <= 0 || H <= 0 || W % 16 || H % 16 ||
+       W > 0x7FFF || H > 0x7FFF || occPrecision < 1 || 16 % occPrecision ) {
+    setError( "attribute_images: invalid argument (the canvas is a multiple of 16 x 16 of at most 32767, the occupancy precision divides 16)" );
+    return TMC2_E_INVALID;
+  }
+  const size_t area = size_t( W ) * H, video = area / size_t( occPrecision * occPrecision );
+  std::vector<uint8_t> hasD1( area, 0 );
+  for ( uint64_t i = 0; i < M; ++i ) {
+    const uint32_t x = pointToPixel[3 * i], y = pointToPixel[3 * i + 1], layer = pointToPixel[3 * i + 2];
+    if ( x >= uint32_t( W ) || y >= uint32_t( H ) || layer > 1 ) {
+      setError( "attribute_images: point %llu maps to (%u, %u, layer %u), outside the %dx%d canvas", (unsigned long long)i, x, y, layer, W, H );
+      return TMC2_E_INVALID;
+    }
+    if ( layer ) hasD1[size_t( y ) * W + x] = 1;
+  }
+  std::vector<uint8_t>  c4( 4 * M );
+  std::vector<uint32_t> pp( M );
+  for ( uint64_t i = 0; i < M; ++i ) {
+    const uint32_t x = pointToPixel[3 * i], y = pointToPixel[3 * i + 1], layer = pointToPixel[3 * i + 2];
+    c4[4 * i] = rgb[3 * i], c4[4 * i + 1] = rgb[3 * i + 1], c4[4 * i + 2] = rgb[3 * i + 2], c4[4 * i + 3] = 0;
+    pp[i]     = packPixel( int( x ), int( y ), int( layer ), !layer && hasD1[size_t( y ) * W + x] );
+  }
+  ApiScope         scope( ctx );
+  hipStream_t      s = ctx->stream;
+  DevBuf<uint8_t>  d_rgb, d_occVideo, d_attr;
+  DevBuf<uint32_t> d_pp;
+  TMC2_TRY( d_rgb.alloc( std::max<size_t>( 4 * M, 4 ) ) );
+  TMC2_TRY( d_pp.alloc( std::max<size_t>( M, 1 ) ) );
+  TMC2_TRY( d_occVideo.alloc( video ) );
+  TMC2_TRY( d_attr.alloc( 6 * area ) );
+  if ( M ) {
+    TMC2_HIP( hipMemcpyAsync( d_rgb.p, c4.data(), 4 * M, hipMemcpyHostToDevice, s ) );
+    TMC2_HIP( hipMemcpyAsync( d_pp.p, pp.data(), 4 * M, hipMemcpyHostToDevice, s ) );
+  }
+  TMC2_HIP( hipMemcpyAsync( d_occVideo.p, occVideo, video, hipMemcpyHostToDevice, s ) );
+  TMC2_TRY( attributeImagesDevice( ctx, d_rgb.p, d_pp.p, uint32_t( M ), d_occVideo.p, W, H, occPrecision, d_attr.p ) );
+  TMC2_HIP( hipMemcpyAsync( out, d_attr.p, 6 * area, hipMemcpyDeviceToHost, s ) );
+  TMC2_HIP( hipStreamSynchronize( s ) );
+  return TMC2_OK;
+}
 
 int tmc2_transfer_colors( tmc2_ctx* ctx, const int16_t* srcXyz, const uint8_t* srcRgb, uint64_t n, const int16_t* tgtXyz,
                           uint64_t m, uint8_t* tgtRgb ) {
diff --git a/mpeg-pcc-tmc2_amd/csrc/images.hip b/mpeg-pcc-tmc2_amd/csrc/images.hip
--- a/mpeg-pcc-tmc2_amd/csrc/images.hip
+++ b/mpeg-pcc-tmc2_amd/csrc/images.hip
@@ -161,15 +161,21 @@
 }
 
 __global__ __launch_bounds__( 256 ) void groupDilateKernel( const uint8_t* __restrict__ occVideo, int W, int H, int Wv,
-                                                             int p, uint16_t* __restrict__ geo ) {
-  const size_t c = size_t( blockIdx.x ) * blockDim.x + threadIdx.x;
-  if ( c >= size_t( W ) * H ) return;
-  const int x = int( c % W ), y = int( c / W );
-  if ( occVideo[size_t( y / p ) * Wv + x / p ] ) return;
-  const uint32_t a = geo[c], b = geo[size_t( W ) * H + c];
-  const uint16_t avg = uint16_t( ( a + b + 1 ) >> 1 );
-  geo[c]                   = avg;
-  geo[size_t( W ) * H + c] = avg;
+                                                             int p, uint2* __restrict__ geo ) {
+  const size_t c = size_t( blockIdx.x ) * blockDim.x + threadIdx.x, plane4 = size_t( W ) * H / 4;
+  if ( c >= plane4 ) return;
+  const int      x   = int( c % ( W / 4 ) ) * 4, y = int( c / ( W / 4 ) );
+  const uint8_t* row = occVideo + size_t( y / p ) * Wv;
+  const uint32_t k0 = row[x / p] ? 0xFFFFu : 0u, k1 = row[( x + 1 ) / p] ? 0xFFFF0000u : 0u;
+  const uint32_t k2 = row[( x + 2 ) / p] ? 0xFFFFu : 0u, k3 = row[( x + 3 ) / p] ? 0xFFFF0000u : 0u;
+  const uint32_t keepX = k0 | k1, keepY = k2 | k3;
+  if ( ( keepX & keepY ) == 0xFFFFFFFFu ) return;
+  uint2       a = geo[c], b = geo[plane4 + c];
+  const uint2 avg = make_uint2( ( a.x | b.x ) - ( ( ( a.x ^ b.x ) >> 1 ) & 0x7FFF7FFFu ), ( a.y | b.y ) - ( ( ( a.y ^ b.y ) >> 1 ) & 0x7FFF7FFFu ) );
+  a.x = ( a.x & keepX ) | ( avg.x & ~keepX ), a.y = ( a.y & keepY ) | ( avg.y & ~keepY );
+  b.x = ( b.x & keepX ) | ( avg.x & ~keepX ), b.y = ( b.y & keepY ) | ( avg.y & ~keepY );
+  geo[c]          = a;
+  geo[plane4 + c] = b;
 }
 
 }
@@ -317,8 +323,8 @@
   hipLaunchKernelGGL( dilateBlockKernel, dim3( Wb * Hb, 2 ), blk, 0, s, f->d_occMap.p, W, H, f->d_geo.p, d_empty.p );
   hipLaunchKernelGGL( carryFirstColumnKernel, dim3( 2 ), dim3( 16 ), 0, s, d_empty.p, W, H, f->d_geo.p, (uint8_t*)nullptr );
   hipLaunchKernelGGL( carryRowsKernel, dim3( ( H + 63 ) / 64, 2 ), dim3( 64 ), 0, s, d_empty.p, W, H, f->d_geo.p );
-  hipLaunchKernelGGL( groupDilateKernel, dim3( uint32_t( ( area + 255 ) / 256 ) ), blk, 0, s, f->d_occVideo.p, W, H, Wv,
-                      occPrecision, f->d_geo.p );
+  hipLaunchKernelGGL( groupDilateKernel, dim3( uint32_t( ( area / 4 + 255 ) / 256 ) ), blk, 0, s, f->d_occVideo.p, W, H, Wv,
+                      occPrecision, reinterpret_cast<uint2*>( f->d_geo.p ) );
   stage.end();
   TMC2_HIP( hipStreamSynchronize( s ) );
   TMC2_HIP( hipGetLastError() );
diff --git a/mpeg-pcc-tmc2_amd/tmc2_amd/lib.py b/mpeg-pcc-tmc2_amd/tmc2_amd/lib.py
--- a/mpeg-pcc-tmc2_amd/tmc2_amd/lib.py
+++ b/mpeg-pcc-tmc2_amd/tmc2_amd/lib.py
@@ -292,6 +292,19 @@
             raise Tmc2Error("transfer_colors: %d source points, %d source colours" % (len(a), len(b)))
         out = np.zeros((len(c), 3), np.uint8)
         _check(self.L.tmc2_transfer_colors(self.h, _ptr(a), _ptr(b), len(a), _ptr(c), len(c), _ptr(out)))
+        return out
+
+    def attribute_images(self, rgb, point_to_pixel, occ_video, W, H, occ_precision=4):
+        a = np.ascontiguousarray(rgb, np.uint8).reshape(-1, 3)
+        b = np.ascontiguousarray(point_to_pixel, np.uint32).reshape(-1, 3)
+        o = np.ascontiguousarray(occ_video, np.uint8)
+        if len(a) != len(b):
+            raise Tmc2Error("attribute_images: %d colours, %d pixel positions" % (len(a), len(b)))
+        W, H, p = int(W), int(H), int(occ_precision)
+        if W <= 0 or H <= 0 or p <= 0 or o.size != (W // p) * (H // p):
+            raise Tmc2Error("attribute_images: occupancy video of %d bytes for a %dx%d canvas at precision %d" % (o.size, W, H, p))
+        out = np.zeros((2, 3, H, W), np.uint8)
+        _check(self.L.tmc2_attribute_images(self.h, _ptr(a), _ptr(b), len(a), _ptr(o), W, H, p, _ptr(out)))
         return out
 
     def convert_points_to_voxels(self, xyz, vox_dim, bits3d):
@@ -1039,6 +1052,7 @@
 int tmc2_frame_get_geometry_images(tmc2_frame*, uint8_t*, uint8_t*, uint32_t*, uint16_t*, uint16_t*)
 int tmc2_encoder_generate_attribute_images(tmc2_frame*)
 int tmc2_transfer_colors(tmc2_ctx*, const int16_t*, const uint8_t*, uint64_t, const int16_t*, uint64_t, uint8_t*)
+int tmc2_attribute_images(tmc2_ctx*, const uint8_t*, const uint32_t*, uint64_t, const uint8_t*, int, int, int, uint8_t*)
 int64_t tmc2_frame_recon_count(tmc2_frame*)
 int tmc2_frame_get_reconstruction(tmc2_frame*, int16_t*, uint8_t*, uint32_t*)
 int tmc2_frame_get_attribute_images(tmc2_frame*, uint8_t*)
```

Measured after the change: 200.3 (median of 6 runs). +1.2%, better.
